# dryman/HashMergeJoin

Hardware: AMD Instinct MI355X
Metric: probe-side tuples/s + achieved HBM GB/s, |R|=|S|=2^28 u64 keys (higher is better)
Workload: dtype u64

## Files before the change

hashmergejoin_amd/__init__.py:

```python
from ._lib import (HMJ_BUILD_ANTI, HMJ_BUILD_OUTER, HMJ_BUILD_SEMI, HMJ_CHECKSUM, HMJ_COLS_HASHED, HMJ_COLS_NO_ROW, HMJ_COLS_PACKED, HMJ_FIRST_WINS, HMJ_FULL_OUTER, HMJ_GROUP_COUNT, HMJ_GROUP_MAX, HMJ_GROUP_MIN, HMJ_GROUP_ROW_MAP, HMJ_GROUP_SUM, HMJ_JOIN_ANTI, HMJ_JOIN_INNER, HMJ_JOIN_PROBE_OUTER, HMJ_JOIN_SEMI, HMJ_KIND_BUILD_SIDE, HMJ_KIND_PROBE_SIDE, HMJ_MATERIALIZE, HMJ_ORDERED, HMJ_PATH_CHUNKED_BUILD, HMJ_PATH_DENSE_BUILD,
                   HMJ_PATH_EXACT, HMJ_PATH_GLOBAL_TABLE, HMJ_PATH_HOST_PIPELINE, HMJ_PATH_HOT_KEY_HINT, HMJ_PATH_LOOKBACK_TIMEOUT, HMJ_PATH_ORDER_BY_KEY, HMJ_PATH_ORDER_BY_RANK_SORT, HMJ_PATH_ORDER_DEFERRED, HMJ_PATH_ORDERED_EXPANSION, HMJ_PATH_LDS_TABLE,
                   HMJ_PATH_KEY_RANGES, HMJ_PATH_PREPARED, HMJ_PATH_PRESORTED, HMJ_PATH_RANK_RUNS, HMJ_PATH_SORT_MSD, HMJ_PATH_SLAB, HMJ_PATH_SLAB_ONE_PASS, HMJ_PATH_SLAB_PROBE, HMJ_PATH_SORTED_FK, HMJ_PATH_SORTED_FK_HALF, HMJ_PATH_SORTED_FK_WIDE, HMJ_PATH_SORTED_WRITE, HMJ_PATH_SPLIT, HMJ_PATH_UNIQ_WRITE, HMJ_PATH_WINDOW,
                   HMJ_KEY_FIXED, HMJ_KEY_LARGE_STRING, HMJ_MAX_KEY_COLS, HMJ_MAX_TAKE_COLS, HMJ_NULL_EQUAL, HMJ_STR_NO_ROW, HMJ_SUM_PROBE, HMJ_TAKE_NO_ROW, BuildJoinOpts, ColsJoinOpts, ColsKindOpts, ColsRel, ColsResult, ExchangeKindOpts, GroupOpts, GroupResult, HmjError, JoinOpts, JoinResult, KeyCol, KindCounts, MixedCol, MixedOpts, MixedRel, StrJoinOpts, StrKindOpts, StrRel, StrResult, TakeDst, TakeOpts, TakeSrc, TakeStrDst, TakeStrOpts, TakeStrSrc, Timing, Validity,
                   lib_path, load_library)
from .join import Executor, HashMergeJoin, cols_key64, expected_groups, mixed_key64, pack_strings, pack_validity, plan, unpack_strings, unpack_validity

__all__ = ["Executor", "HashMergeJoin", "plan", "HmjError", "JoinResult", "Timing", "load_library",
           "lib_path", "HMJ_MATERIALIZE", "HMJ_ORDERED", "HMJ_FIRST_WINS", "HMJ_CHECKSUM",
           "HMJ_SUM_PROBE", "JoinOpts", "HMJ_JOIN_INNER", "HMJ_JOIN_SEMI", "HMJ_JOIN_ANTI", "HMJ_JOIN_PROBE_OUTER",
           "BuildJoinOpts", "HMJ_BUILD_SEMI", "HMJ_BUILD_ANTI", "HMJ_BUILD_OUTER", "HMJ_FULL_OUTER",
           "ExchangeKindOpts", "KindCounts", "HMJ_KIND_PROBE_SIDE", "HMJ_KIND_BUILD_SIDE",
           "pack_strings", "StrRel", "StrJoinOpts", "StrResult", "StrKindOpts", "HMJ_STR_NO_ROW",
           "KeyCol", "ColsRel", "ColsJoinOpts", "ColsResult", "HMJ_COLS_PACKED", "HMJ_COLS_HASHED", "HMJ_MAX_KEY_COLS",
           "cols_key64", "ColsKindOpts", "HMJ_COLS_NO_ROW", "Validity", "pack_validity",
           "TakeSrc", "TakeDst", "TakeOpts", "HMJ_TAKE_NO_ROW", "HMJ_MAX_TAKE_COLS", "unpack_validity",
           "TakeStrSrc", "TakeStrDst", "TakeStrOpts", "unpack_strings",
           "MixedCol", "MixedRel", "MixedOpts", "HMJ_KEY_FIXED", "HMJ_KEY_LARGE_STRING", "mixed_key64",
           "HMJ_NULL_EQUAL",
           "GroupOpts", "GroupResult", "HMJ_GROUP_COUNT", "HMJ_GROUP_SUM", "HMJ_GROUP_MIN", "HMJ_GROUP_MAX", "HMJ_GROUP_ROW_MAP",
           "expected_groups"]
```

hashmergejoin_amd/_lib.py:

```python
import ctypes as C
import os

HMJ_MATERIALIZE = 0x01
HMJ_ORDERED = 0x02
HMJ_FIRST_WINS = 0x04
HMJ_CHECKSUM = 0x08
HMJ_SUM_PROBE = 0x10
HMJ_NULL_EQUAL = 0x20
HMJ_E_RCCL, HMJ_E_PEER, HMJ_E_TIMEOUT = -6, -7, -8
HMJ_PATH_SLAB, HMJ_PATH_EXACT, HMJ_PATH_UNIQ_WRITE, HMJ_PATH_SPLIT, HMJ_PATH_WINDOW = 0x1, 0x2, 0x4, 0x8, 0x10
HMJ_PATH_ORDER_DEFERRED, HMJ_PATH_ORDER_BY_KEY, HMJ_PATH_PREPARED, HMJ_PATH_CHUNKED_BUILD = 0x20, 0x40, 0x80, 0x100
HMJ_PATH_HOT_KEY_HINT = 0x200
HMJ_PATH_SLAB_PROBE = 0x400
HMJ_PATH_SORTED_WRITE = 0x800
HMJ_PATH_SORTED_FK = 0x1000
HMJ_PATH_DENSE_BUILD = 0x2000
HMJ_PATH_GLOBAL_TABLE = 0x100000
HMJ_PATH_ORDER_BY_RANK_SORT = 0x200000
HMJ_PATH_ORDERED_EXPANSION = 0x400000
HMJ_PATH_LDS_TABLE = 0x800000
HMJ_PATH_RANK_RUNS = 0x1000000
HMJ_PATH_RANK_LOOKUP_IN_PASS = 0x2000000
HMJ_PATH_SORT_MSD = 0x4000000
HMJ_PATH_KEY_RANGES = 0x8000000
HMJ_PATH_SLAB_ONE_PASS = 0x80000
HMJ_PATH_HOST_PIPELINE = 0x4000
HMJ_PATH_SORTED_FK_HALF = 0x8000
HMJ_PATH_LOOKBACK_TIMEOUT = 0x10000
HMJ_PATH_SORTED_FK_WIDE = 0x20000
HMJ_PATH_PRESORTED = 0x40000

_HERE = os.path.dirname(os.path.abspath(__file__))
_U64P = C.POINTER(C.c_uint64)


class HmjError(RuntimeError):
    def __init__(self, code, msg):
        super().__init__("hmj error %d: %s" % (code, msg))
        self.code = code


class JoinResult(C.Structure):
    _fields_ = [("n_matches", C.c_uint64), ("sum_r", C.c_uint64), ("sum_s", C.c_uint64),
                ("xor_fold", C.c_uint64), ("mix_sum", C.c_uint64), ("sum_probe_all", C.c_uint64),
                ("key", C.c_void_p), ("rval", C.c_void_p), ("sval", C.c_void_p)]

    def checks(self):
        return {k: int(getattr(self, k)) for k in ("n_matches", "sum_r", "sum_s", "xor_fold", "mix_sum")}


HMJ_JOIN_INNER, HMJ_JOIN_SEMI, HMJ_JOIN_ANTI, HMJ_JOIN_PROBE_OUTER = 0, 1, 2, 3


class JoinOpts(C.Structure):
    _fields_ = [("struct_size", C.c_uint32), ("kind", C.c_uint32), ("outer_fill", C.c_uint64),
                ("n_probe_matched", C.c_uint64), ("n_probe_unmatched", C.c_uint64)]


HMJ_BUILD_SEMI, HMJ_BUILD_ANTI, HMJ_BUILD_OUTER, HMJ_FULL_OUTER = 1, 2, 3, 4


class BuildJoinOpts(C.Structure):
    _fields_ = [("struct_size", C.c_uint32), ("kind", C.c_uint32), ("build_fill", C.c_uint64), ("probe_fill", C.c_uint64),
# ... 165 lines not shown
                ("ms_out_scan", C.c_float), ("ms_probe_write", C.c_float), ("ms_order", C.c_float),
                ("radix_bits", C.c_int), ("radix_passes", C.c_int),
                ("n_scatter_launches", C.c_int), ("n_split_retries", C.c_int),
                ("bytes_scatter", C.c_uint64), ("bytes_hist", C.c_uint64),
                ("bytes_probe_count", C.c_uint64), ("bytes_probe_write", C.c_uint64),
                ("path", C.c_uint32), ("key_prefix_bits", C.c_int32), ("key_window_low", C.c_int32),
                ("n_probe_items", C.c_uint32), ("ms_scatter_pass0", C.c_float), ("ms_scatter_pass1", C.c_float)]

    def as_dict(self):
        return {n: getattr(self, n) for n, _ in self._fields_}


class PlanDesc(C.Structure):
    _fields_ = [("struct_size", C.c_uint32), ("path", C.c_uint32), ("radix_bits", C.c_int32), ("radix_passes", C.c_int32),
                ("pass_bits", C.c_int32 * 4), ("key_prefix_bits", C.c_int32), ("key_window_low", C.c_int32),
                ("n_partitions", C.c_uint32), ("probe_items", C.c_uint32), ("attempts", C.c_uint32), ("refused", C.c_uint32),
                ("cooling", C.c_uint32), ("workload", C.c_uint64)]

    def as_dict(self):
        d = {n: getattr(self, n) for n, _ in self._fields_}
        d["pass_bits"] = list(self.pass_bits)
        return d


HMJ_REFUSED_GTABLE_SHAPE, HMJ_REFUSED_GTABLE_COOLING, HMJ_REFUSED_GTABLE_GAVE_UP = 0x1, 0x2, 0x4
HMJ_REFUSED_RANK_SORT_MODEL, HMJ_REFUSED_RANK_SORT_COOLING, HMJ_REFUSED_RANK_SORT_GAVE_UP = 0x8, 0x10, 0x20
HMJ_REFUSED_SLAB_SHAPE, HMJ_REFUSED_SLAB_COOLING, HMJ_REFUSED_SLAB_SORTED_INPUT, HMJ_REFUSED_SLAB_OVERFLOW = 0x40, 0x80, 0x100, 0x200
HMJ_REFUSED_FAST_WRITE_COOLING, HMJ_REFUSED_FAST_WRITE_GAVE_UP = 0x400, 0x800
HMJ_REFUSED_SLAB_PROBE_COOLING, HMJ_REFUSED_SLAB_PROBE_OVERFLOW = 0x1000, 0x2000
HMJ_REFUSED_PREFIX_VIOLATED, HMJ_REFUSED_EXPANSION_GAVE_UP = 0x4000, 0x8000
HMJ_COOL_UNIQ_WRITE, HMJ_COOL_SORTED_WRITE, HMJ_COOL_GTABLE, HMJ_COOL_GTABLE_WRITE = 0x1, 0x2, 0x4, 0x8
HMJ_COOL_RANK_SORT, HMJ_COOL_RANK_SORT_SLAB, HMJ_COOL_EXPANSION, HMJ_COOL_SORT_SLAB = 0x10, 0x20, 0x40, 0x80
HMJ_COOL_SLAB, HMJ_COOL_SLAB_PROBE, HMJ_COOL_ONE_PASS_WRITE, HMJ_COOL_EXACT_PREFIX = 0x100, 0x200, 0x400, 0x800
HMJ_COOL_RANK_RUNS = 0x1000


class PlaceInfo(C.Structure):
    _fields_ = [("name", C.c_char * 16), ("bytes", C.c_uint64), ("fill_TBps", C.c_float), ("candidates", C.c_int),
                ("ms_search", C.c_float), ("searched", C.c_int), ("aborted", C.c_int), ("budget_ms", C.c_float),
                ("cand_ms_alloc", C.c_float * 4), ("cand_ms_fill", C.c_float * 4), ("cand_TBps", C.c_float * 4)]


def lib_path():
    return os.environ.get("HMJ_LIB") or os.path.join(_HERE, "libhmj_hip.so")


class ExchangeInfo(C.Structure):
    _fields_ = [("n_ranks", C.c_int), ("owner_mode", C.c_int), ("rounds_build", C.c_uint32), ("rounds_probe", C.c_uint32),
                ("recv_build", C.c_uint64), ("recv_probe", C.c_uint64), ("ms_split", C.c_float),
                ("ms_exchange_build", C.c_float), ("ms_exchange_probe", C.c_float), ("ms_local", C.c_float),
                ("ms_total", C.c_float), ("digit_bits", C.c_int32), ("digit_low", C.c_int32), ("n_subjoins", C.c_uint32),
                ("fallback", C.c_uint32), ("sample_max_share", C.c_float), ("ms_kernels", C.c_float),
                ("ms_exposed", C.c_float)]

    def as_dict(self):
        return {n: getattr(self, n) for n, _ in self._fields_}


HMJ_MAX_RANKS, HMJ_MAX_ROUNDS = 16, 16


class DigitPlan(C.Structure):
    _fields_ = [("usable", C.c_int32), ("digit_bits", C.c_int32), ("digit_low", C.c_int32), ("n_rounds", C.c_uint32),
                ("owner_first", C.c_uint32 * (HMJ_MAX_RANKS + 1)),
                ("round_first", (C.c_uint32 * (HMJ_MAX_ROUNDS + 1)) * HMJ_MAX_RANKS), ("max_share", C.c_float)]


# ... 151 lines not shown
```

hashmergejoin_amd/csrc/api.hip:

```cpp
#include <hip/hip_runtime.h>
#include <sys/mman.h>

#include <algorithm>
#include <cstdio>
#include <cstdlib>
#include <chrono>
#include <cmath>
#include <cstring>
#include <mutex>
#include <string>
#include <thread>
#include <vector>

#include "hmj_ctx.h"

using hmj::u32;
using hmj::u64;
using namespace hmj_host;

namespace hmj_host {

constexpr int kMaxEvents = 1024;

int fail(hmj_ctx* c, int code, const char* what, hipError_t e) {
// ... 29 lines not shown
  acc->ms_scatter_pass[0] += t.ms_scatter_pass[0];
  acc->ms_scatter_pass[1] += t.ms_scatter_pass[1];
  if (t.radix_passes) {
    acc->radix_bits = t.radix_bits;
    acc->radix_passes = t.radix_passes;
    acc->key_prefix_bits = t.key_prefix_bits;
    acc->key_window_low = t.key_window_low;
  }
  acc->n_probe_items += t.n_probe_items;
}

static int ilog2_u64(uint64_t v) { return v ? 63 - __builtin_clzll(v) : 0; }
uint64_t workload_signature(uint64_t n_build, uint64_t n_probe, uint32_t flags, int kind) {
  const uint32_t mode = ((flags & HMJ_ORDERED) ? 4u : 0u) | ((flags & (HMJ_MATERIALIZE | HMJ_ORDERED)) ? 2u : 0u) |
                        ((flags & HMJ_FIRST_WINS) ? 1u : 0u);
  return ((uint64_t)(kind & 31) << 20) | ((uint64_t)mode << 16) | ((uint64_t)ilog2_u64(n_build) << 8) | (uint64_t)ilog2_u64(n_probe);
}
WorkloadMemo* memo_for(hmj_ctx* c, uint64_t sig) {
  auto it = c->memos.find(sig);
  if (it == c->memos.end()) {
    if (c->memos.size() >= 1024) c->memos.clear();
    it = c->memos.emplace(sig, c->memo_init).first;
  }
  c->wm = &it->second;
  c->wm_sig = sig;
  return c->wm;
}
uint32_t WorkloadMemo::cooling() const {
  return (uniq_cooldown ? HMJ_COOL_UNIQ_WRITE : 0u) | (sorted_cooldown ? HMJ_COOL_SORTED_WRITE : 0u) | (gtable_cooldown ? HMJ_COOL_GTABLE : 0u) |
         (gtable_write_cooldown ? HMJ_COOL_GTABLE_WRITE : 0u) | (gtable_sort_cooldown ? HMJ_COOL_RANK_SORT : 0u) |
         (gtable_sort_slab_cooldown ? HMJ_COOL_RANK_SORT_SLAB : 0u) | (expand_cooldown ? HMJ_COOL_EXPANSION : 0u) |
         (sort_slab_cooldown ? HMJ_COOL_SORT_SLAB : 0u) | (slab_cooldown ? HMJ_COOL_SLAB : 0u) | (slab_probe_cooldown ? HMJ_COOL_SLAB_PROBE : 0u) |
         (one_pass_write_cooldown ? HMJ_COOL_ONE_PASS_WRITE : 0u) | (exact_prefix_joins ? HMJ_COOL_EXACT_PREFIX : 0u) |
         (rank_runs_cooldown ? HMJ_COOL_RANK_RUNS : 0u) | (sort_msd_cooldown ? HMJ_COOL_SORT_MSD : 0u);
}

int wait_arrival(hmj_ctx* c, hipEvent_t ev) {
  if (c->arrive_wait) return c->arrive_wait(c, ev);
  HIP_TRY(hipStreamWaitEvent(c->stream, ev, 0));
  return HMJ_OK;
}

int ensure_dev(hmj_ctx* c, DevBuf& b, size_t bytes) {
  if (bytes <= b.cap) return HMJ_OK;
  if (c && (&b == &c->rbuf[0] || &b == &c->rbuf[1] || &b == &c->r_off || &b == &c->slab_br || &b == &c->cnt_br))
    c->prep.valid = false;
  if (b.p) {
    hipError_t e = hipFree(b.p);
    b.p = nullptr;
    b.cap = 0;
    if (e != hipSuccess) return fail(c, HMJ_E_HIP, "hipFree", e);
  }
  size_t want = bytes + (bytes >> 4) + 256;
#ifdef HMJ_DEV
  if (const char* e = getenv("HMJ_ALLOC_PAD_KB")) want += (size_t)atoll(e) << 10;
  if (const char* e = getenv("HMJ_ALLOC_ROUND_MB")) {
    const size_t g = (size_t)atoll(e) << 20;
    if (g) want = (want + g - 1) / g * g;
  }
#endif
  const auto t_alloc0 = std::chrono::steady_clock::now();
  hipError_t e = hipMalloc(&b.p, want);
  if (e != hipSuccess) {
    b.p = nullptr;
    (void)hipGetLastError();
    return fail(c, HMJ_E_OOM, "hipMalloc", e);
  }
// ... 430 lines not shown
  a.r_off = (const u32*)c->r_off.p;
  a.S = Sp;
  a.s_off = (const u32*)c->s_off.p;
  a.P = P;
  a.Q = Q;
  a.accum = (u64*)c->accum.p;
  return a;
}
static hmj::ProbeArgs slab_probe_args(hmj_ctx* c, const hmj::SlabGeom* build_slabs, const void* Rp, const DevBuf& s_slab,
                                      const DevBuf& s_cnt, u32 s_cap, u32 P, u32 Q) {
  hmj::ProbeArgs a;
  std::memset(&a, 0, sizeof(a));
  if (build_slabs) {
    a.R = c->slab_br.p;
    a.r_cnt = (const u32*)c->cnt_br.p;
    a.r_cap = build_slabs->CB;
    a.r_cnt_n = c->cnt_br.cap / 4;
    a.r_rows = c->slab_br.cap / 16;
  } else {
    a.R = Rp;
    a.r_off = (const u32*)c->r_off.p;
  }
  a.S = s_slab.p;
  a.s_cnt = (const u32*)s_cnt.p;
  a.s_cap = s_cap;
  a.s_cnt_n = s_cnt.cap / 4;
  a.s_rows = s_slab.cap / 16;
  a.P = P;
  a.Q = Q;
  a.accum = (u64*)c->accum.p;
  return a;
}

static int slab_pass_a(hmj_ctx* c, const void* in, u32 n, int rel, int low, int bits, const hmj::SlabGeom& g, bool arriving) {
  u64* acc = (u64*)c->accum.p;
  const u64 a_rows = c->slab_a.cap / 16, a_cnt = c->cnt_a.cap / 4;
  const int sp = span_begin(c, K_SCATTER, rel, 0);
  if (arriving) {
    u32 w_done = 0;
    for (size_t i = 0; i < c->arrive_ev.size(); i++) {
      RC_TRY(wait_arrival(c, c->arrive_ev[i]));
      const bool last = i + 1 == c->arrive_ev.size();
      const u32 w_end = last ? g.WA : (u32)std::min<u64>(g.WA, c->arrive_rows[i] / g.rpw);
      if (w_end > w_done) {
        HIP_TRY(hmj::launch_slab_a(in, n, low, bits, g, c->slab_a.p, a_rows, (u32*)c->cnt_a.p, a_cnt, acc, c->stream, w_done, w_end));
        w_done = w_end;
      }
    }
  } else {
    HIP_TRY(hmj::launch_slab_a(in, n, low, bits, g, c->slab_a.p, a_rows, (u32*)c->cnt_a.p, a_cnt, acc, c->stream));
  }
  span_end(c, sp);
  c->timing.bytes_scatter += 32ull * n;
  return HMJ_OK;
}
static int slab_passes(hmj_ctx* c, const void* in, u32 n, int rel, int low, int ba, int bb, const hmj::SlabGeom& g, DevBuf& sb,
                       DevBuf& cb, bool arriving) {
  RC_TRY(slab_pass_a(c, in, n, rel, low, ba, g, arriving));
  const int sp = span_begin(c, K_SCATTER, rel, 1);
  HIP_TRY(hmj::launch_slab_b(c->slab_a.p, (const u32*)c->cnt_a.p, ba, low + ba, bb, g, sb.p, sb.cap / 16, (u32*)cb.p, cb.cap / 4,
                             (u64*)c->accum.p, c->stream));
  span_end(c, sp);
  c->timing.bytes_scatter += 32ull * n;
  return HMJ_OK;
}

static int clear_matched(hmj_ctx* c, size_t slots, u32** matched) {
  const size_t bytes = (slots / 32 + 1) * 4;
  RC_TRY(ensure_dev(c, c->matched, bytes));
  *matched = (u32*)c->matched.p;
  HIP_TRY(hipMemsetAsync(c->matched.p, 0, bytes, c->stream));
  return HMJ_OK;
}

int order_rows(hmj_ctx* c, const u32* vstart, const u32* in_base32, const u64* in_base64, u32 P, u32 Q, int low,
               u64 n, bool by_key_only, bool many_per_key, const u64** rk, const u64** rr, const u64** rs, int* retry_code) {
  const size_t bytes = (size_t)n * 8;
  RC_TRY(ensure_dev(c, c->ord_key, bytes));
  RC_TRY(ensure_dev(c, c->ord_rval, bytes));
  RC_TRY(ensure_dev(c, c->ord_sval, bytes));
  const bool can_sort = n <= 0xFFFFFFFFull;
  if (by_key_only && !can_sort) {
    *retry_code = kRetryNoWinOrdered;
    return HMJ_OK;
  }
  int sp = span_begin(c, K_ORDER, -1);
  HIP_TRY(hmj::launch_order((const u64*)c->part_out_off.p, vstart, in_base32, in_base64, P, Q, low,
                            (const u64*)c->out_key.p, (const u64*)c->out_rval.p, (const u64*)c->out_sval.p,
                            (u64*)c->ord_key.p, (u64*)c->ord_rval.p, (u64*)c->ord_sval.p, (u64*)c->accum.p,
                            can_sort ? 65536u : 0u, many_per_key, c->num_cus * 4, c->stream));
  span_end(c, sp);
  u64* h = (u64*)c->h_accum.p;
  HIP_TRY(hipMemcpyAsync(&h[hmj::ACC_ERR], (u64*)c->accum.p + hmj::ACC_ERR, 8, hipMemcpyDeviceToHost, c->stream));
  HIP_TRY(hipStreamSynchronize(c->stream));
  if (h[hmj::ACC_ERR] & hmj::ERR_ORDER_FAIL)
    return fail(c, HMJ_E_UNSUPPORTED, "HMJ_ORDERED: one partition's result exceeds 2^31-1 rows and the whole result 2^32-1 rows");
// ... 521 lines not shown
static int run_slab_join(hmj_ctx* c, const JoinCall& j, const JoinPlan& p) {
  const bool materialize = j.materialize(), first = j.first(), extra = j.extra();
  const u32 nb = j.nb, np = j.np, np_plan = p.np_plan, P = p.P;
  const int* pass_bits = p.pass_bits;
  hmj::SlabGeom gr, gs;
  if (p.allow_slab && c->slab_mode && c->wm->slab_cooldown == 0 && !c->prepare_only && !(c->timing.path & HMJ_PATH_SLAB) &&
      !((!materialize || p.fast_write) && p.Q == 1 && p.probe_fits && p.passes == 2 && pass_bits[0] <= hmj::SLAB_MAX_BITS &&
        pass_bits[1] <= hmj::SLAB_MAX_BITS && p.dense_scale <= 2.5))
    c->plan.refused |= HMJ_REFUSED_SLAB_SHAPE;
  if (!(p.allow_slab && c->slab_mode && c->wm->slab_cooldown == 0 && (!materialize || p.fast_write) && p.Q == 1 &&
        p.probe_fits &&
        p.passes == 2 && pass_bits[0] <= hmj::SLAB_MAX_BITS && pass_bits[1] <= hmj::SLAB_MAX_BITS &&
        slab_sizes_ok(c, nb, np_plan, materialize || np_plan < nb) &&
        p.dense_scale <= 2.5 &&
        hmj::slab_geometry(nb, pass_bits[0], pass_bits[1], &gr, 0, 1.0, p.dense_scale) &&
        hmj::slab_geometry(np_plan, pass_bits[0], pass_bits[1], &gs, 0,
                           (nb && np_plan > nb) ? (double)np_plan / (double)nb : 1.0, p.dense_scale)))
    return kPlanNotTaken;
  const bool reuse = c->prep.valid && c->prep.slab && c->prep.ptr == j.R && c->prep.n == nb &&
                     c->prep.low == p.low && c->prep.B == p.B;
  c->prep.valid = false;
  c->timing.path |= HMJ_PATH_SLAB | (reuse ? HMJ_PATH_PREPARED : 0u);
  c->timing.n_probe_items = P;
  const int ba = pass_bits[0], bb = pass_bits[1];
  const u64 rows_a = gr.rows_a > gs.rows_a ? gr.rows_a : gs.rows_a;
  const u32 wa = gr.WA > gs.WA ? gr.WA : gs.WA;
  RC_TRY(ensure_dev(c, c->slab_a, rows_a * 16));
  RC_TRY(ensure_dev(c, c->cnt_a, ((size_t)wa << ba) * 4));
  RC_TRY(ensure_dev(c, c->slab_br, gr.rows_b * 16));
  RC_TRY(ensure_dev(c, c->slab_bs, gs.rows_b * 16));
  RC_TRY(ensure_dev(c, c->cnt_br, (size_t)P * gr.KB * 4));
  RC_TRY(ensure_dev(c, c->cnt_bs, (size_t)P * gs.KB * 4));
  if (!reuse) RC_TRY(slab_passes(c, j.R, nb, 0, p.low, ba, bb, gr, c->slab_br, c->cnt_br, false));
  if (!c->prepare_only) RC_TRY(slab_passes(c, j.S, np, 1, p.low, ba, bb, gs, c->slab_bs, c->cnt_bs, !c->arrive_ev.empty()));
  u64* hh;
  if (c->prepare_only) {
    RC_TRY(read_accum(c, &hh));
    if (hh[hmj::ACC_ERR] & hmj::ERR_SLAB) {
      c->wm->slab_cooldown = 8;
      return kRetryNoSlab;
    }
    c->prep.valid = true;
    c->prep.slab = true;
    c->prep.ptr = j.R;
    c->prep.n = nb;
    c->prep.low = p.low;
    c->prep.B = p.B;
    return HMJ_OK;
  }
  hmj::ProbeArgs sa = slab_probe_args(c, &gr, nullptr, c->slab_bs, c->cnt_bs, gs.CB, P, 1);
  if (p.fast_write)
    return unique_key_write(c, sa, true, nb, np, p.low, extra, p.verify_pfx ? p.prefix : 0, p.pfx_ref, j.ordered(), j.to_host,
                            p.fk_wide_plan, p.dense_scale, j.out);
#ifdef HMJ_DEV
  sa.debug = c->dev_ablate;
#endif
  int sp = span_begin(c, K_PROBE_COUNT, -1);
  if (first || extra) {
    sa.extra = (extra ? 1u : 0u) | (first ? 2u : 0u);
    HIP_TRY(hmj::launch_probe_count_ext(sa, nullptr, nullptr, true, c->num_cus, c->stream));
  } else {
    HIP_TRY(hmj::launch_probe_count_slab(sa, c->num_cus, c->stream));
  }
  span_end(c, sp);
  c->timing.bytes_probe_count = 16ull * ((u64)nb + np);
  RC_TRY(read_accum(c, &hh));
  if (hh[hmj::ACC_ERR] & hmj::ERR_SLAB) {
    c->wm->slab_cooldown = 8;
    return kRetryNoSlab;
  }
  result_sums(j.out, hh);
  return HMJ_OK;
}

static int partition_build_exact(hmj_ctx* c, const JoinCall& j, const JoinPlan& p, const void** Rp) {
  const bool reuse_exact = c->prep.valid && !c->prep.slab && c->prep.ptr == j.R && c->prep.n == j.nb &&
                           c->prep.low == p.low && c->prep.B == p.B;
  c->prep.valid = false;
  c->timing.path |= HMJ_PATH_EXACT | (reuse_exact ? HMJ_PATH_PREPARED : 0u);
  if (reuse_exact) {
    *Rp = c->prep.Rp;
  } else {
    RC_TRY(partition_relation(c, j.R, j.nb, c->rbuf, p.low, p.passes, p.pass_bits, 0, Rp, p.asc_r));
    const int s = span_begin(c, K_OFFSETS, -1);
    HIP_TRY(hmj::launch_part_offsets(*Rp, j.nb, p.low, p.B, (u32*)c->r_off.p, c->stream));
    span_end(c, s);
  }
  if (c->prepare_only) {
    HIP_TRY(hipStreamSynchronize(c->stream));
// ... 316 lines not shown
  RC_TRY(ensure_dev(c, c->s_off, ((size_t)p.P + 1) * 4));
  RC_TRY(ensure_dev(c, c->accum, 8 * sizeof(u64)));
  RC_TRY(ensure_host(c, c->h_accum, 8 * sizeof(u64)));
  if (j.materialize()) {
    RC_TRY(ensure_dev(c, c->part_count, (size_t)p.items * 8));
    RC_TRY(ensure_dev(c, c->part_out_off, ((size_t)p.items + 1) * 8));
  }
  HIP_TRY(hipMemsetAsync(c->accum.p, 0, 8 * sizeof(u64), c->stream));
  int rc = run_slab_join(c, j, p);
  if (rc != kPlanNotTaken) return rc;
  const void* Rp;
  RC_TRY(partition_build_exact(c, j, p, &Rp));
  if (c->prepare_only) return HMJ_OK;
  for (hipEvent_t ev : c->arrive_ev) RC_TRY(wait_arrival(c, ev));
  rc = run_probe_slab_join(c, j, p, Rp);
  if (rc != kPlanNotTaken) return rc;
  rc = run_one_pass_slab_join(c, j, p, Rp);
  if (rc != kPlanNotTaken) return rc;
  return run_partitioned_join(c, j, p, Rp);
}

int join_device_impl(hmj_ctx* c, const void* R, uint64_t n_build, const void* S, uint64_t n_probe,
                     uint32_t flags, hmj_result* out, bool to_host, bool allow_auto_prefix,
                     bool allow_slab, bool allow_fast_write, bool allow_win_ordered, bool prefix_unsafe,
                     bool allow_slab_probe) {
  if (!out) return fail(c, HMJ_E_ARG, "out is NULL");
  std::memset(out, 0, sizeof(*out));
  RC_TRY(check_rel(c, R, n_build, "build_aos is NULL"));
  RC_TRY(check_rel(c, S, n_probe, "probe_aos is NULL"));
  if (flags & HMJ_ORDERED) flags |= HMJ_MATERIALIZE;
  if (!c->prepare_only && c->prep.valid && !c->prep.slab && c->prep.ptr == R && c->prep.n == (u32)n_build) allow_slab = false;
  const bool materialize = flags & HMJ_MATERIALIZE;
  if (c->wm->slab_cooldown > 0 && allow_slab) c->wm->slab_cooldown--;
  if (c->wm->slab_probe_cooldown > 0 && allow_slab_probe) c->wm->slab_probe_cooldown--;
  if (c->wm->one_pass_write_cooldown > 0 && materialize && allow_slab_probe) c->wm->one_pass_write_cooldown--;
  JoinPlan p;
  RC_TRY(plan_join(c, R, n_build, S, n_probe, flags, allow_auto_prefix, allow_slab, allow_fast_write, allow_win_ordered,
                   prefix_unsafe, allow_slab_probe, &p));
  const JoinCall j{R, S, (u32)n_build, (u32)n_probe, flags, out, to_host};
  return execute_join(c, j, p);
}

int try_global_table(hmj_ctx* c, const void* R, uint64_t n_build, const void* S, uint64_t n_probe, uint32_t flags,
                     hmj_result* out, bool to_host, bool* done) {
  *done = false;
  const bool materialize = (flags & HMJ_MATERIALIZE) != 0;
  c->plan.refused |= HMJ_REFUSED_GTABLE_SHAPE;
  if (!c->gtable_mode || (flags & HMJ_ORDERED) || c->prepare_only || c->force_bits >= 0 ||
      !c->arrive_ev.empty() || n_build == 0 || n_probe > 0xFFFFFFFFull || n_probe < c->gtable_min_probe ||
      (n_build > (materialize && !(c->one_pass_slab && c->slab_mode && n_probe >= (1ull << 22) && n_probe >= 8 * n_build) ? 2 : 1) * c->gtable_max_rows && !(n_build <= 8 * c->gtable_max_rows && n_build + n_probe <= 16 * c->gtable_max_rows)) ||
      n_probe < (uint64_t)c->gtable_min_fanout * n_build ||
      (c->prep.valid && c->prep.ptr == R && c->prep.n == (u32)n_build))
    return HMJ_OK;
  c->plan.refused &= ~HMJ_REFUSED_GTABLE_SHAPE;
  if (materialize && c->wm->gtable_write_cooldown > 0) {
    c->wm->gtable_write_cooldown--;
    c->plan.refused |= HMJ_REFUSED_GTABLE_COOLING;
    return HMJ_OK;
  }
  if (c->wm->gtable_cooldown > 0) {
    c->wm->gtable_cooldown--;
    c->plan.refused |= HMJ_REFUSED_GTABLE_COOLING;
    return HMJ_OK;
  }
  if (!out) return fail(c, HMJ_E_ARG, "out is NULL");
  RC_TRY(check_rel(c, R, n_build, "build_aos is NULL"));
// ... 875 lines not shown
    const u64 unmatched = k.kind == HMJ_JOIN_SEMI ? n_probe - out->n_matches : filled;
    counts->n_probe_matched = n_probe - unmatched;
    counts->n_probe_unmatched = unmatched;
  } else {
    const u64 b_unmatched = k.kind == HMJ_BUILD_SEMI ? n_build - swept : swept;
    counts->n_build_matched = n_build - b_unmatched;
    counts->n_build_unmatched = b_unmatched;
    if (k.kind == HMJ_FULL_OUTER) {
      counts->n_probe_matched = n_probe - filled;
      counts->n_probe_unmatched = filled;
    }
  }
  return HMJ_OK;
}

}

extern "C" {

int hmj_create(hmj_ctx** out, int device_id) {
  if (!out) return HMJ_E_ARG;
  *out = nullptr;
  int ndev = 0;
  if (hipGetDeviceCount(&ndev) != hipSuccess || ndev <= 0) {
    (void)hipGetLastError();
    return HMJ_E_NODEV;
  }
  if (device_id < 0 && hipGetDevice(&device_id) != hipSuccess) return HMJ_E_NODEV;
  if (device_id >= ndev) return HMJ_E_ARG;
  if (hipSetDevice(device_id) != hipSuccess) return HMJ_E_NODEV;
  hmj_ctx* c = new hmj_ctx();
  c->device = device_id;
  if (const char* e = getenv("HMJ_SLAB")) c->slab_mode = atoi(e);
  if (const char* e = getenv("HMJ_ONE_PASS_SLAB")) c->one_pass_slab = atoi(e) != 0;
  if (const char* e = getenv("HMJ_GTABLE")) c->gtable_mode = atoi(e) != 0;
  if (const char* e = getenv("HMJ_RANK_RUNS")) c->rank_runs_mode = atoi(e) != 0;
  if (const char* e = getenv("HMJ_RANK_RUNS_MAX_CUT")) c->rank_runs_max_cut = atoi(e) < 0 ? 0 : atoi(e) > 16 ? 16 : atoi(e);
  if (const char* e = getenv("HMJ_RANK_RUNS_MAX_GROUP")) c->rank_runs_max_group = atoi(e) < 0 ? 0 : atoi(e) > 4 ? 4 : atoi(e);
  if (const char* e = getenv("HMJ_PROMOTE_TO_ORDERED")) c->promote_to_ordered = atoi(e) != 0;
  if (const char* e = getenv("HMJ_KEY_RANGES")) c->key_ranges = atoi(e) != 0;
  if (const char* e = getenv("HMJ_KEY_RANGES_FORCE")) c->key_ranges_force = atoi(e) < 0 ? 0 : atoi(e) > 4 ? 4 : atoi(e);
  if (const char* e = getenv("HMJ_RANK_RUNS_WAVE")) c->rank_runs_wave = atoi(e) != 0;
  if (const char* e = getenv("HMJ_RANK_RUNS_MAX_LEVEL")) c->rank_runs_max_level = atoi(e) < 0 ? 0 : atoi(e) > 2 ? 2 : atoi(e);
  if (const char* e = getenv("HMJ_GTABLE_SORT")) c->gtable_sort_mode = atoi(e) != 0;
  if (const char* e = getenv("HMJ_EXPAND_FK_FANOUT")) c->expand_fk_fanout = atoi(e) > 0 ? (u32)atoi(e) : 0u;
  if (const char* e = getenv("HMJ_SORT_MSD")) c->sort_msd = atoi(e) != 0;
  if (const char* e = getenv("HMJ_SORT_MSD_MEAN")) c->sort_msd_mean = atof(e) >= 64.0 ? atof(e) : c->sort_msd_mean;
  if (const char* e = getenv("HMJ_SORT_MSD_MAX_BITS")) c->sort_msd_max_bits = atoi(e) < 2 ? 2 : atoi(e) > 18 ? 18 : atoi(e);
  if (const char* e = getenv("HMJ_SORT_MSD_MIN_LOG2")) {
    const int l = atoi(e);
    if (l >= 16 && l <= 32) c->sort_msd_min = 1ull << l;
  }
  if (const char* e = getenv("HMJ_SORT_SLAB_MIN_LOG2")) {
    const int l = atoi(e);
    if (l >= 12 && l <= 32) c->sort_slab_min = 1ull << l;
  }
  if (const char* e = getenv("HMJ_GTABLE_SORT_SLAB_MIN_LOG2")) {
    const int l = atoi(e);
    if (l >= 12 && l <= 32) c->gtable_sort_slab_min = 1ull << l;
  }
  if (const char* e = getenv("HMJ_GTABLE_SORT_FANOUT")) c->gtable_sort_fanout = atoi(e) > 0 ? (u32)atoi(e) : 1u;
  if (const char* e = getenv("HMJ_PLACE")) {
    c->place_tune = atoi(e) != 0;
    if (atoi(e) > 0) {
      c->place_tries = atoi(e);
      c->place_search_always = true;
// ... 862 lines not shown
```

hashmergejoin_amd/csrc/hmj_ctx.h:

```cpp
#pragma once
#include <hip/hip_runtime.h>

#include <string>
#include <unordered_map>
#include <vector>

#include "../../include/hmj.h"
#include "hmj_dev.h"
#include "hmj_launch.h"

struct hmj_comm;

namespace hmj_host {

struct DevBuf {
  void* p = nullptr;
  size_t cap = 0;
};
struct HostBuf {
  void* p = nullptr;
  size_t cap = 0;
  bool pinned = true;
};

// ... 31 lines not shown
  template <class F>
  void each_buf(F f) {
    for (DevBuf* b : {&rows, &sorted, &flags, &blk, &blk_off, &list, &runs, &acc, &start}) f(*b);
    each_result_buf(f);
  }
};

enum Kind {
  K_TOTAL = 0, K_H2D, K_D2H, K_HIST, K_SCAN, K_SCATTER, K_OFFSETS, K_PROBE_COUNT, K_OUT_SCAN,
  K_PROBE_WRITE, K_ORDER, K_NKINDS
};
struct Span {
  int kind, rel, e0, e1;
  int pass;
};

struct WorkloadMemo {
  int uniq_cooldown = 0;
  int sorted_cooldown = 0;
  bool sorted_chained = false;
  bool sorted_wide = true;
  bool sorted_fk = false;
  int sorted_fk_age = 0;
  int gtable_cooldown = 0;
  int gtable_write_cooldown = 0;
  int gtable_sort_cooldown = 0;
  int gtable_sort_slab_cooldown = 0;
  int rank_runs_cooldown = 0;
  int rank_lookup_cooldown = 0;
  int expand_cooldown = 0;
  int sort_slab_cooldown = 0;
  int sort_msd_cooldown = 0;
  int slab_cooldown = 0;
  int slab_probe_cooldown = 0;
  int one_pass_write_cooldown = 0;
  int exact_prefix_joins = 0;
  uint32_t cooling() const;
};

}

namespace hmj_host {
struct OrderedCostModel {
  double part_fixed_ms = 0.15;
  double part_ns = 0.030, part_ns_per_f = 0.00023;
  double part_bucket_ns = 0.043, part_bucket_ns_per_f = 0.0001;
  double part_epilogue_ns = 0.25;
  double comp_fixed_ms = 0.65;
  double comp_ns_chain = 0.060, comp_ns_exact = 0.072;
  double comp_ns_wide = 0.145;
  double comp_ns_beyond_l2 = 0.02;
  double runs_fixed_ms = 0.25, runs_ns = 0.0215, runs_ns_per_run = 7.5;
  double runs_ns_per_log2_build = 0.0023;
  double runs_wave_ns_per_run = 1.2, runs_wave_ns = 0.007;
  double runs_range_ns = 0.0;
};
}

struct hmj_ctx {
  using DevBuf = hmj_host::DevBuf;
  using HostBuf = hmj_host::HostBuf;
  using Span = hmj_host::Span;
  using WorkloadMemo = hmj_host::WorkloadMemo;
  using u32 = hmj::u32;
  using u64 = hmj::u64;
  int device = 0, num_cus = 256;
// ... 56 lines not shown
  bool gtable_mode = true;
  uint64_t gtable_max_rows = 1ull << 17;
  u32 gtable_min_fanout = 0;
  uint64_t gtable_min_probe = 1;
  int gtable_wg_per_cu = 8;
  u32 gtable_slots_per_row = 16;
  int gtable_max_log_cap = 18;
  bool ltable_mode = true;
  bool gtable_sort_mode = true;
  u32 gtable_sort_fanout = 128;
  bool rank_runs_mode = true;
  int rank_runs_max_cut = 10;
  int rank_runs_max_group = 3;
  int rank_runs_max_level = 2;
  uint64_t big_join_rows = 1ull << 29;
  bool promote_to_ordered = true;
  bool key_ranges = true;
  int key_ranges_force = 0;
  bool rank_runs_wave = true;
  bool build_sort_msd = true;
  bool gtable_sort_slab = true;
  u64 gtable_sort_slab_min = 1ull << 25;
  bool expand_mode = true;
  u32 fk_payload_buckets = 24;
  u32 expand_fk_fanout = 0;
  bool expand_allow_rebits = true;
  int expand_rebits = 0;
  bool sort_msd = true;
  double sort_msd_mean = 1200.0;
  int sort_msd_max_bits = 18;
  u64 sort_msd_min = 1ull << 22;
  bool sort_slab = true;
  u64 sort_slab_min = 1ull << 25;
  int slab_mode = 1;
  bool staged_upload = false;
  bool host_pipeline = true;
  hipStream_t copy_stream = nullptr;
  std::vector<hipEvent_t> copy_ev;
  bool split_mode = true;
  bool window_mode = true;
  u32 slab_min_rows = 1u << 21;
  u32 slab_probe_kb = 0;
  bool one_pass_slab = true;
  int scatter_variant = 1;
  bool profiling = false;
  bool trace = false;
#ifdef HMJ_DEV
  u32 dev_ablate = 0;
#endif
  std::vector<hipEvent_t> events;
  std::vector<Span> spans;
  int ev_used = 0;
  hmj_timing timing;
  std::string last_error;
  hmj_comm* comm = nullptr;
  std::vector<u64> arrive_rows;
  std::vector<hipEvent_t> arrive_ev;
  bool sample_build_only = false;
  int (*arrive_wait)(hmj_ctx*, hipEvent_t) = nullptr;
};


namespace hmj_host {
int fail(hmj_ctx* c, int code, const char* what, hipError_t e = hipSuccess);
#define HIP_TRY(expr)                                                        \
  do {                                                                       \
// ... 39 lines not shown
```

hashmergejoin_amd/csrc/hmj_dev.h:

```cpp
#pragma once
#include <hip/hip_runtime.h>
#include <stdint.h>

namespace hmj {

typedef unsigned long long u64;
typedef unsigned int u32;
typedef unsigned short u16;

struct __attribute__((aligned(16))) Tup {
  u64 key;
  u64 val;
};

constexpr int kWave = 64;
#ifndef HMJ_SCAN_DPP
#define HMJ_SCAN_DPP 1
#endif

#ifndef HMJ_STREAM_POLICY
#define HMJ_STREAM_POLICY 2
#endif
typedef u64 u64x2_t __attribute__((ext_vector_type(2)));
__device__ __forceinline__ void store_stream(Tup* p, const Tup& v) {
#if HMJ_STREAM_POLICY >= 1
  u64x2_t x = {v.key, v.val};
  __builtin_nontemporal_store(x, reinterpret_cast<u64x2_t*>(p));
#else
  *p = v;
#endif
}
__device__ __forceinline__ Tup load_stream(const Tup* p) {
#if HMJ_STREAM_POLICY >= 2
  const u64x2_t x = __builtin_nontemporal_load(reinterpret_cast<const u64x2_t*>(p));
  Tup t;
  t.key = x.x;
  t.val = x.y;
  return t;
#else
  return *p;
#endif
}

constexpr u64 GT_EMPTY = ~0ull;
constexpr int GT_MAXWALK = 64;
__device__ __forceinline__ u32 gt_hash(u64 key, int shift) {
  u64 h = key * 0x9E3779B97F4A7C15ull;
  h ^= h >> 32;
  h *= 0xD6E8FEB86659FD93ull;
  return (u32)(h >> shift);
}

#ifndef HMJ_RANK_PASS_CHUNK_ROWS
#define HMJ_RANK_PASS_CHUNK_ROWS 64
#endif
constexpr int RANK_PASS_CHUNK_ROWS = HMJ_RANK_PASS_CHUNK_ROWS;
__device__ __forceinline__ u64 rank_run_bucket(u64 off, int pre, u64 mult) { return ((off >> pre) * mult) >> 32; }

template <int ROWS, typename Table, typename OnSlot>
__device__ __forceinline__ void gt_walk(Table tab, u32 mask, u32 (&slot)[ROWS], bool (&live)[ROWS], OnSlot on_slot) {
  bool any_live = false;
#pragma unroll
  for (int r = 0; r < ROWS; r++) any_live |= live[r];
  while (any_live) {
    Tup e[ROWS];
#pragma unroll
    for (int r = 0; r < ROWS; r++)
      if (live[r]) e[r] = tab[slot[r]];
    any_live = false;
#pragma unroll
    for (int r = 0; r < ROWS; r++) {
// ... 3 lines not shown
        } else {
          slot[r] = (slot[r] + 1) & mask;
          any_live = true;
        }
      }
    }
  }
}

constexpr int RP_THREADS = 512;
constexpr int RP_WAVES = RP_THREADS / kWave;
constexpr int RP_ITEMS = 8;
constexpr int RP_TILE = RP_THREADS * RP_ITEMS;
constexpr int RP_MAX_BITS = 9;
constexpr int RP_MAXD = 1 << RP_MAX_BITS;
constexpr int RP_MAX_BLOCKS = 2048;

constexpr int PB_THREADS = 1024;
constexpr int PB_CAP = 5120;
constexpr int PB_LOG_NB = 12;
constexpr int PB_TARGET_AVG = 4096;
constexpr int PB_PLAN_SLACK = 256;

constexpr int SLAB_KB = 4;
constexpr int SLAB_MAX_BITS = 9;

enum { ACC_N = 0, ACC_SUM_R, ACC_SUM_S, ACC_XOR, ACC_MIX, ACC_SUM_P, ACC_ERR, ACC_PAD };
constexpr u64 ERR_SLAB = 2;
constexpr u64 ERR_ORDER_DEFER = 16;
constexpr u64 ERR_ORDER_FAIL = 32;
constexpr u64 ERR_SORTED = 64;
constexpr u64 ERR_FASTPATH = 8;
constexpr u64 ERR_GTABLE = 128;
constexpr u64 ERR_PREFIX = 4;

__device__ __forceinline__ u64 mix64(u64 x) {
  x ^= x >> 30;
  x *= 0xBF58476D1CE4E5B9ull;
  x ^= x >> 27;
  x *= 0x94D049BB133111EBull;
  x ^= x >> 31;
  return x;
}

__device__ __forceinline__ u64 tmix(u64 key, u64 rval, u64 sval) {
  u64 t = mix64(key);
  t = mix64(t ^ rval);
  t = mix64(t + sval);
  return t;
}

__device__ __forceinline__ int lane_id() {
  return __builtin_amdgcn_mbcnt_hi(~0u, __builtin_amdgcn_mbcnt_lo(~0u, 0u));
}

__device__ __forceinline__ u32 popc_below(u64 m) {
  return __builtin_amdgcn_mbcnt_hi((u32)(m >> 32), __builtin_amdgcn_mbcnt_lo((u32)m, 0u));
}

__device__ __forceinline__ u32 wave_incl_scan_u32(u32 v, int ) {
#if HMJ_SCAN_DPP
  v += (u32)__builtin_amdgcn_update_dpp(0, (int)v, 0x111, 0xF, 0xF, false);
  v += (u32)__builtin_amdgcn_update_dpp(0, (int)v, 0x112, 0xF, 0xF, false);
  v += (u32)__builtin_amdgcn_update_dpp(0, (int)v, 0x114, 0xF, 0xF, false);
  v += (u32)__builtin_amdgcn_update_dpp(0, (int)v, 0x118, 0xF, 0xF, false);
  v += (u32)__builtin_amdgcn_update_dpp(0, (int)v, 0x142, 0xA, 0xF, false);
// ... 73 lines not shown
```

hashmergejoin_amd/csrc/hmj_launch.h:

```cpp
#pragma once
#include <hip/hip_runtime.h>
#include <stddef.h>
#include <stdint.h>

#include <atomic>

namespace hmj {
typedef unsigned long long u64;
typedef unsigned int u32;

struct SmemAttrOnce {
  std::atomic<unsigned long long> devices{0};
};
inline hipError_t ensure_max_smem(SmemAttrOnce& once, const void* kernel, size_t bytes) {
  int dev = 0;
  hipError_t e = hipGetDevice(&dev);
  if (e != hipSuccess) return e;
  const unsigned long long bit = 1ull << (dev & 63);
  if (dev < 64 && (once.devices.load(std::memory_order_acquire) & bit)) return hipSuccess;
  e = hipFuncSetAttribute(kernel, hipFuncAttributeMaxDynamicSharedMemorySize, (int)bytes);
  if (e != hipSuccess) return e;
  if (dev < 64) once.devices.fetch_or(bit, std::memory_order_release);
  return hipSuccess;
}

constexpr int kMaxRanks = 16;
struct OwnerFn {
  u32 mode;
  u32 G;
  u64 spl[kMaxRanks - 1];
};
int radix_tile_rows(int bits, int variant);
void radix_pass_geometry(u32 n, int tile, u32* nblk, u32* rows_per_block);
size_t radix_scatter_smem_bytes();
hipError_t launch_radix_hist(const void* in, u32 n, int tile, int shift, int bits, u32* hist,
                             u32 nblk, u32 rows_per_block, hipStream_t st, const OwnerFn* own = nullptr);
hipError_t launch_owner_scatter(const void* in, void* out, u32 n, int bits, const OwnerFn& own,
                                const u32* hist_scanned, const u32* totals, u32 nblk, u32 rows_per_block,
                                u64* offsets_out, hipStream_t st);
hipError_t launch_radix_rowscan(u32* hist, u32 nblk, int bits, u32* totals, hipStream_t st);
hipError_t launch_radix_scatter(const void* in, void* out, u32 n, int variant, int shift, int bits,
                                const u32* hist_scanned, const u32* totals, u32 nblk,
                                u32 rows_per_block, u64* offsets_out, hipStream_t st);
struct SlabGeom {
  u32 WA, rpw, CA, CB, KB;
  u64 rows_a, rows_b;
};
bool slab_geometry(u32 n, int bits_a, int bits_b, SlabGeom* g, u32 kb = 0, double fan = 1.0, double density = 1.0);
bool slab_geometry_one_pass(u32 n, int bits, double keys_per_digit, u32 max_workers, SlabGeom* g, double density = 1.0);
u32 slab_capacity(double mean, double fan);
hipError_t launch_slab_a(const void* in, u32 n, int shift, int bits, const SlabGeom& g, void* slab_a, u64 slab_a_rows,
                         u32* cnt_a, u64 cnt_a_n, u64* accum, hipStream_t st, u32 w_begin = 0, u32 w_end = 0xFFFFFFFFu);
hipError_t launch_slab_b(const void* slab_a, const u32* cnt_a, int bits_a, int shift, int bits,
                         const SlabGeom& g, void* slab_b, u64 slab_b_rows, u32* cnt_b, u64 cnt_b_n, u64* accum, hipStream_t st);
hipError_t launch_key_sample(const void* R, u32 nb, const void* S, u32 np, u64* out, hipStream_t st);
hipError_t launch_key_exact(const void* R, u32 nb, const void* S, u32 np, u64 ref, u64* out, int num_cus, hipStream_t st,
                            bool ref_is_first_key = false);
hipError_t launch_check_partitioned(const void* a, u32 n, int low, int bits, u32* flag, int num_cus, hipStream_t st);
hipError_t launch_part_offsets(const void* a, u32 n, int low, int bits, u32* off, hipStream_t st);

struct ProbeArgs {
  const void* R;
  const u32* r_off;
  const void* S;
  const u32* s_off;
  u32 P;
  u32 Q;
  u64* part_count;
  const u64* part_out_off;
  u64* out_key;
  u64* out_rval;
  u64* out_sval;
  u64 out_cap;
  u64* accum;
  const u32* item_list;
  const u32* n_item_list;
  const u32* r_cnt;
  const u32* s_cnt;
  u32 r_cap, s_cap;
  u32 s_wa, s_ppi;
  u64 r_cnt_n, s_cnt_n;
  u64 r_rows, s_rows;
  const u64* item_base;
  const u32* r_end;
  const u32* s_end;
  u32 extra;
  u32 pfx_shift;
  u64 pfx_val;
  u32* matched;
  u32 debug;
};
hipError_t launch_probe(const ProbeArgs& a, int mode, bool first_wins, bool extra, int grid,
                        hipStream_t st);
int probe_default_grid(int num_cus);
hipError_t launch_probe_kind(const ProbeArgs& a, int mode, int kind, bool first_wins, u64 fill, int grid, hipStream_t st);
hipError_t launch_probe_build_kind(const ProbeArgs& a, int mode, int kind, u64 fill, u32* bmark, int grid, hipStream_t st);
hipError_t launch_build_sweep(const ProbeArgs& a, const u32* r_off, u32 P, const u32* vstart, u64* sweep_n, int mode,
                              bool set, u64 fill, int num_cus, hipStream_t st);
hipError_t launch_probe_count_ext(const ProbeArgs& a, u32* irregular, u32* n_irregular, bool slab,
                                  int num_cus, hipStream_t st);
hipError_t launch_probe_count_slab(const ProbeArgs& a, int num_cus, hipStream_t st);
hipError_t launch_probe_write_sorted(const ProbeArgs& a, bool slab, bool fk, int shape, u64* lookback, bool chained, int key_low,
                                     int num_cus, hipStream_t st);
hipError_t launch_probe_write_uniq(const ProbeArgs& a, bool slab, int num_cus, hipStream_t st);
hipError_t launch_slab_np(const u32* cnt, u32 P, u64* out, hipStream_t st);
hipError_t launch_probe_count_fast(const ProbeArgs& a, u32* irregular, u32* n_irregular, bool big,
                                   bool per_partition_counts, int num_cus, hipStream_t st);
hipError_t launch_scan_u64(const u64* in, u64* out_excl, u32 n, hipStream_t st);
hipError_t launch_probe_expand_ordered(const ProbeArgs& a, int key_low, int num_cus, hipStream_t st);
hipError_t launch_order(const u64* part_out_off, const u32* vstart, const u32* in_base32, const u64* in_base64, u32 P, u32 Q,
                        int low, const u64* akey, const u64* arval, const u64* asval, u64* bkey, u64* brval,
                        u64* bsval, u64* accum, u32 defer_rows, bool many_per_key, int grid, hipStream_t st);
hipError_t launch_compact(const u64* part_out_off, const u32* in_base32, const u64* in_base64, u32 P, const u64* akey,
                          const u64* arval, const u64* asval, u64* bkey, u64* brval, u64* bsval, int grid, hipStream_t st);
hipError_t launch_rekey(void* pairs, u64 n, const u64* col, hipStream_t st);

hipError_t launch_gtable_build(const void* R, u32 nb, void* tab, int log_cap, u64* accum, bool first, int num_cus,
                               hipStream_t st);
hipError_t launch_gtable_probe(const void* S, u32 np, const void* tab, int log_cap, const void* R, u64* accum, bool first,
                               bool extra, int num_cus, int wg_per_cu, hipStream_t st);
hipError_t launch_gtable_write(const void* S, u32 np, const void* tab, int log_cap, const void* R, u64* accum, u64* out_key,
                               u64* out_rval, u64* out_sval, bool first, bool extra, int num_cus, int wg_per_cu, hipStream_t st);

hipError_t launch_ltable_probe(const void* R, u32 nb, const void* S, u32 np, u64* accum, bool first, bool extra, int num_cus, hipStream_t st);
int ltable_max_rows();
hipError_t launch_sval_range(const void* S, u32 np, u64* out2 , int num_cus, hipStream_t st,
                             u32 every = 1 );
hipError_t launch_gtable_emit(const void* S, u32 np, const void* tab, int log_cap, u64 svmin, int range_bits, u64* accum,
                              void* pairs, bool extra, bool wide, int num_cus, int wg_per_cu, hipStream_t st);
hipError_t launch_gtable_swap(const void* in, void* out, u64 n, int num_cus, hipStream_t st);
hipError_t launch_gtable_emit_ranks(const void* S, u32 np, const void* tab, int log_cap, u64* accum, void* pairs, bool extra, int num_cus,
                                    int wg_per_cu, hipStream_t st);
int rank_sort_max_run(int level = 0);
hipError_t launch_sort_runs_write(const void* slabs, const u32* cnt, u32 cap, u32 P, const u64* out_off, void* out, u64* accum, int level,
// ... 36 lines not shown
```

hashmergejoin_amd/csrc/probe.hip:

```cpp
#include "hmj_dev.h"
#include "hmj_launch.h"
#include <type_traits>

namespace hmj {

constexpr u32 PB_NB = 1u << PB_LOG_NB;
constexpr u32 NIL = 0xFFFFu;
static_assert(PB_CAP < 0xFFFF, "chain links are 16-bit");

struct ProbeSmem {
  u64 key[PB_CAP];
  u64 val[PB_CAP];
  u32 head[PB_NB];
  u32 aux[PB_CAP];
  u16 next[PB_CAP];
  u32 scratch[PB_THREADS / kWave + 1];
  u64 pcount;
  u64 red[8];
  u64 obase;
  u32 wtot[PB_THREADS / kWave];
  u32 nslot;
};
constexpr u32 PB_BATCH = 2 * PB_THREADS;
static_assert(PB_BATCH <= PB_CAP, "a batch must fit an empty table");
// ... 860 lines not shown
};

template <int LOG_NB>
__device__ __forceinline__ u32 fast_hash(u64 k) {
  u32 x = (u32)k ^ ((u32)(k >> 32) * 0x85EBCA6Bu);
  x *= 0x9E3779B1u;
  return x >> (32 - LOG_NB);
}

template <int THREADS, int ROWS = FP_ROWS>
__device__ __forceinline__ void fp_load(Tup (&t)[ROWS], const Tup* __restrict__ base, u32 n,
                                        int tid) {
#pragma unroll
  for (int k = 0; k < ROWS; k++) {
    u32 i = k * THREADS + tid;
    t[k] = base[i < n ? i : n - 1];
  }
}

static_assert(SLAB_KB == 4, "fp_load_slab / fp_load_pieces / slab_np_kernel unroll exactly four pieces per partition");
template <int THREADS, int ROWS = FP_ROWS>
__device__ __forceinline__ void fp_load_slab(Tup (&t)[ROWS], const Tup* __restrict__ base, u32 cap,
                                             u32 p1, u32 p2, u32 p3, u32 n, int tid) {
#pragma unroll
  for (int k = 0; k < ROWS; k++) {
    u32 i = k * THREADS + tid;
    i = i < n ? i : n - 1;
    const u32 j = (i >= p1) + (i >= p2) + (i >= p3);
    const u32 pre = j == 0 ? 0u : (j == 1 ? p1 : (j == 2 ? p2 : p3));
    t[k] = base[(u64)j * cap + (i - pre)];
  }
}

template <int THREADS>
__device__ __forceinline__ void fp_load_pieces(Tup (&t)[FP_ROWS], const Tup* __restrict__ base, u32 cap, u32 cnt_mine, int tid) {
  constexpr int QT = THREADS / 4;
  const u32 g = (u32)tid / QT, l = (u32)tid % QT;
  const Tup* __restrict__ piece = base + (u64)g * cap;
  const u32 last = cnt_mine ? cnt_mine - 1 : 0;
#pragma unroll
  for (int k = 0; k < FP_ROWS; k++) {
    const u32 r = l + (u32)k * QT;
    t[k] = piece[r < last ? r : last];
  }
}

template <int THREADS, int LOG_NB, bool PCOUNT, bool SLAB, int OUT>
__global__ __launch_bounds__(THREADS, 4) void probe_count_fast_kernel(
    ProbeArgs a, u32* __restrict__ irregular, u32* __restrict__ n_irregular) {
  typedef FastSmem<THREADS, LOG_NB> Smem;
  constexpr u32 CAP = Smem::CAP, NB = 1u << LOG_NB;
  constexpr bool PIECES = SLAB && OUT == 0 && !PCOUNT && HMJ_PROBE_PIECES;
  constexpr u32 QT = THREADS / 4, PIECE_CAP = FP_ROWS * QT;
  extern __shared__ __attribute__((aligned(16))) unsigned char smem_raw[];
  Smem& sm = *reinterpret_cast<Smem*>(smem_raw);
  const Tup* __restrict__ R = static_cast<const Tup*>(a.R);
  const Tup* __restrict__ S = static_cast<const Tup*>(a.S);
  const u32* __restrict__ r_off = a.r_off;
  const u32* __restrict__ s_off = a.s_off;
  const u32* __restrict__ r_end = (SLAB || a.r_end == nullptr) ? a.r_off + 1 : a.r_end;
  const u32* __restrict__ s_end = (SLAB || a.s_end == nullptr) ? a.s_off + 1 : a.s_end;
  const u32 P = a.P;
  const int tid = threadIdx.x;
  u64 acc_n = 0, acc_r = 0, acc_s = 0, acc_x = 0, acc_m = 0, acc_p = 0;
  bool pfx_bad = false, giveup = false;
  for (u32 i = tid; i < NB; i += THREADS) sm.head[i] = 0;
  if (tid < 2) sm.itemcnt[tid] = 0;
  u32 epoch = 0;
  u32 prev_p = 0xFFFFFFFFu, parity = 0;

  u32 p = blockIdx.x;
  u32 rb = 0, nb = 0, sb = 0, np = 0;
  bool regular = false;
  Tup br[FP_ROWS], pr[FP_ROWS], pq[FP_ROWS];
  u32 r1 = 0, r2 = 0, r3 = 0, s1 = 0, s2 = 0, s3 = 0, r1n = 0, r2n = 0, r3n = 0, s1n = 0, s2n = 0, s3n = 0;
  u32 rm = 0, sm_ = 0, rmn = 0, smn = 0;
  const u32 my_piece = (u32)tid / QT;
  bool slab_bad = false;
  if (p < P) {
    if (SLAB) {
      const u32* rc = a.r_cnt + (u64)p * SLAB_KB;
      const u32* sc = a.s_cnt + (u64)p * SLAB_KB;
      r1 = rc[0]; r2 = r1 + rc[1]; r3 = r2 + rc[2]; nb = r3 + rc[3];
      s1 = sc[0]; s2 = s1 + sc[1]; s3 = s2 + sc[2]; np = s3 + sc[3];
      if (nb > CAP || np > CAP) slab_bad = true;
      if (PIECES) {
        rm = my_piece == 0 ? rc[0] : my_piece == 1 ? rc[1] : my_piece == 2 ? rc[2] : rc[3];
        sm_ = my_piece == 0 ? sc[0] : my_piece == 1 ? sc[1] : my_piece == 2 ? sc[2] : sc[3];
        if (rc[0] > PIECE_CAP || rc[1] > PIECE_CAP || rc[2] > PIECE_CAP || rc[3] > PIECE_CAP || sc[0] > PIECE_CAP ||
            sc[1] > PIECE_CAP || sc[2] > PIECE_CAP || sc[3] > PIECE_CAP) {
          slab_bad = true;
          nb = CAP + 1;
        }
      }
    } else {
      rb = r_off[p]; nb = r_end[p] - rb;
      sb = s_off[p]; np = s_end[p] - sb;
    }
    regular = nb && np && nb <= CAP && np <= CAP;
    if (regular) {
      if (PIECES) {
        fp_load_pieces<THREADS>(br, R + (u64)p * SLAB_KB * a.r_cap, a.r_cap, rm, tid);
        fp_load_pieces<THREADS>(pr, S + (u64)p * SLAB_KB * a.s_cap, a.s_cap, sm_, tid);
      } else if (SLAB) {
        fp_load_slab<THREADS>(br, R + (u64)p * SLAB_KB * a.r_cap, a.r_cap, r1, r2, r3, nb, tid);
        if (OUT == 0) fp_load_slab<THREADS>(pr, S + (u64)p * SLAB_KB * a.s_cap, a.s_cap, s1, s2, s3, np, tid);
      } else {
        fp_load<THREADS>(br, R + rb, nb, tid);
        if (OUT == 0) fp_load<THREADS>(pr, S + sb, np, tid);
      }
    }
  }
  const Tup* __restrict__ dummy = reinterpret_cast<const Tup*>(a.accum);
  auto load_build = [&](Tup (&t)[FP_ROWS], bool ok, u32 pp, u32 rb_, u32 nb_, u32 q1, u32 q2, u32 q3, u32 mine) {
    if (PIECES)
      fp_load_pieces<THREADS>(t, ok ? R + (u64)pp * SLAB_KB * a.r_cap : dummy, ok ? a.r_cap : 0u, ok ? mine : 1u, tid);
    else if (SLAB)
      fp_load_slab<THREADS>(t, ok ? R + (u64)pp * SLAB_KB * a.r_cap : dummy, ok ? a.r_cap : 0u, ok ? q1 : 1u, ok ? q2 : 1u,
                            ok ? q3 : 1u, ok ? nb_ : 1u, tid);
    else
      fp_load<THREADS>(t, ok ? R + rb_ : dummy, ok ? nb_ : 1u, tid);
  };
  auto load_probe = [&](Tup (&t)[FP_ROWS], bool ok, u32 pp, u32 sb_, u32 np_, u32 q1, u32 q2, u32 q3, u32 mine) {
    if (PIECES)
      fp_load_pieces<THREADS>(t, ok ? S + (u64)pp * SLAB_KB * a.s_cap : dummy, ok ? a.s_cap : 0u, ok ? mine : 1u, tid);
    else if (SLAB)
      fp_load_slab<THREADS>(t, ok ? S + (u64)pp * SLAB_KB * a.s_cap : dummy, ok ? a.s_cap : 0u, ok ? q1 : 1u, ok ? q2 : 1u,
                            ok ? q3 : 1u, ok ? np_ : 1u, tid);
    else
      fp_load<THREADS>(t, ok ? S + sb_ : dummy, ok ? np_ : 1u, tid);
  };
  const int tid_outer = tid;
  while (p < P) {
    int tid = tid_outer;
    if constexpr (OUT != 0) asm volatile("" : "+v"(tid));
    u64 out_base = (u64)sb;
    if constexpr (OUT == 1 && SLAB) {
      const u64* ibp = a.item_base + p;
      asm volatile("s_load_dwordx2 %0, %1, 0x0\n\ts_waitcnt lgkmcnt(0)" : "=s"(out_base) : "s"(ibp) : "memory");
    }
    const u32 pn = __builtin_amdgcn_readfirstlane(p + gridDim.x);
    u32 rb2 = 0, nb2 = 0, sb2 = 0, np2 = 0;
    bool regular2 = false;
    if (pn < P) {
      if (SLAB) {
        const u32* rc = a.r_cnt + (u64)pn * SLAB_KB;
        const u32* sc = a.s_cnt + (u64)pn * SLAB_KB;
        r1n = rc[0]; r2n = r1n + rc[1]; r3n = r2n + rc[2]; nb2 = r3n + rc[3];
        s1n = sc[0]; s2n = s1n + sc[1]; s3n = s2n + sc[2]; np2 = s3n + sc[3];
        if (nb2 > CAP || np2 > CAP) slab_bad = true;
        if (PIECES) {
          rmn = my_piece == 0 ? rc[0] : my_piece == 1 ? rc[1] : my_piece == 2 ? rc[2] : rc[3];
          smn = my_piece == 0 ? sc[0] : my_piece == 1 ? sc[1] : my_piece == 2 ? sc[2] : sc[3];
          if (rc[0] > PIECE_CAP || rc[1] > PIECE_CAP || rc[2] > PIECE_CAP || rc[3] > PIECE_CAP || sc[0] > PIECE_CAP ||
              sc[1] > PIECE_CAP || sc[2] > PIECE_CAP || sc[3] > PIECE_CAP) {
            slab_bad = true;
            nb2 = CAP + 1;
          }
        }
      } else {
        rb2 = r_off[pn]; nb2 = r_end[pn] - rb2;
        sb2 = s_off[pn]; np2 = s_end[pn] - sb2;
      }
      regular2 = nb2 && np2 && nb2 <= CAP && np2 <= CAP;
    }
    if (OUT == 0) {
      load_probe(pq, regular2, pn, sb2, np2, s1n, s2n, s3n, smn);
    } else if (regular) {
      if (SLAB)
        fp_load_slab<THREADS>(pr, S + (u64)p * SLAB_KB * a.s_cap, a.s_cap, s1, s2, s3, np, tid);
      else
        fp_load<THREADS>(pr, S + sb, np, tid);
    }
    if (regular) {
      lds_barrier();
      if (PCOUNT && prev_p != 0xFFFFFFFFu && tid == 0) {
        a.part_count[prev_p] = sm.itemcnt[parity ^ 1];
        sm.itemcnt[parity ^ 1] = 0;
      }
      if (PCOUNT) prev_p = 0xFFFFFFFFu;
      epoch++;
      if (epoch == 0x10000u) {
        for (u32 i = tid; i < NB; i += THREADS) sm.head[i] = 0;
        epoch = 1;
        lds_barrier();
      }
      const u32 tag = epoch << 16;
      if (!HMJ_ABLATE(1u)) {
        u32 old[FP_ROWS];
#pragma unroll
        for (int k = 0; k < FP_ROWS; k++) {
          const u32 i = k * THREADS + tid;
          old[k] = tag | NIL;
          if (PIECES ? ((u32)tid % QT + (u32)k * QT < rm) : (i < nb)) {
            if (a.pfx_shift && (br[k].key >> a.pfx_shift) != a.pfx_val) pfx_bad = true;
            sm.key[i] = br[k].key;
            sm.val[i] = br[k].val;
            old[k] = atomicExch(&sm.head[fast_hash<LOG_NB>(br[k].key)], tag | i);
          }
        }
#pragma unroll
        for (int k = 0; k < FP_ROWS; k++) {
          const u32 i = k * THREADS + tid;
          if (PIECES ? ((u32)tid % QT + (u32)k * QT < rm) : (i < nb)) sm.next[i] = ((old[k] >> 16) == epoch) ? (u16)old[k] : (u16)NIL;
        }
      } else {
#pragma unroll
        for (int k = 0; k < FP_ROWS; k++) acc_r += br[k].key;
      }
      load_build(br, regular2, pn, rb2, nb2, r1n, r2n, r3n, rmn);
      lds_barrier();
      const u64 n_before = acc_n;
      if (!HMJ_ABLATE(1u)) {
        u32 cur[FP_ROWS];
        u32 cnt[FP_ROWS], first[FP_ROWS];
#pragma unroll
        for (int k = 0; k < FP_ROWS; k++) {
          const u32 j = k * THREADS + tid;
          cur[k] = NIL;
          cnt[k] = 0;
          first[k] = OUT == 2 ? NIL : 0;
          if (PIECES ? ((u32)tid % QT + (u32)k * QT < sm_) : (j < np)) {
            if (a.pfx_shift && (pr[k].key >> a.pfx_shift) != a.pfx_val) pfx_bad = true;
            if (OUT >= 1 && (a.extra & 1u)) acc_p += pr[k].val;
            const u32 hv = sm.head[fast_hash<LOG_NB>(pr[k].key)];
            cur[k] = ((hv >> 16) == epoch) ? (hv & 0xFFFFu) : NIL;
          }
        }
        for (; !HMJ_ABLATE(2u);) {
          bool any = false;
#pragma unroll
          for (int k = 0; k < FP_ROWS; k++) any |= (cur[k] != NIL);
          if (!__any(any)) break;
#pragma unroll
          for (int k = 0; k < FP_ROWS; k++) {
            if (cur[k] != NIL) {
              const u32 i = cur[k];
              const u64 kk = sm.key[i], vv = sm.val[i];
              cur[k] = sm.next[i];
              if (kk == pr[k].key) {
                if (OUT == 2 && (a.extra & 2u)) {
                  first[k] = i < first[k] ? i : first[k];
                } else {
                  acc_n++;
                  acc_r += vv;
                  acc_s += pr[k].val;
                  if (OUT == 1) {
                    if (cnt[k] == 0) first[k] = i;
                    cnt[k]++;
                  }
                  if (OUT >= 1 && (a.extra & 1u)) {
                    const u64 m = tmix(kk, vv, pr[k].val);
                    acc_x ^= m;
                    acc_m += m;
                  }
                }
              }
            }
          }
        }
        if (OUT == 2 && (a.extra & 2u)) {
#pragma unroll
          for (int k = 0; k < FP_ROWS; k++) {
            if (first[k] != NIL) {
              const u64 vv = sm.val[first[k]];
              acc_n++;
              acc_r += vv;
              acc_s += pr[k].val;
              if (a.extra & 1u) {
                const u64 m = tmix(pr[k].key, vv, pr[k].val);
                acc_x ^= m;
                acc_m += m;
              }
            }
          }
        }
        if (OUT == 1) {
          u64 packed = 0;
          bool cx = false;
#pragma unroll
          for (int k = 0; k < FP_ROWS; k++) {
            cx |= cnt[k] > 1;
            packed |= (u64)(cnt[k] ? 1u : 0u) << (12 * k);
          }
          const int lane = tid & 63, wv = tid >> 6;
          const bool wave_dup = __any(cx);
          u64 incl = packed;
#pragma unroll
          for (int o = 1; o < kWave; o <<= 1) {
            u64 t = __shfl_up(incl, o, kWave);
            if (lane >= o) incl += t;
          }
          if (lane == 63) {
            sm.wscan[wv] = incl;
            sm.wdup[wv] = wave_dup ? 1u : 0u;
          }
          lds_barrier();
          u64 pre = 0, tot = 0;
          u32 dup = 0;
#pragma unroll
          for (int q = 0; q < THREADS / kWave; q++) {
            const u64 ws = sm.wscan[q];
            dup |= sm.wdup[q];
            if (q < wv) pre += ws;
            tot += ws;
          }
          const u64 ex = pre + incl - packed;
          if (dup) {
            giveup = true;
          } else {
            u64 o = out_base;
            u32 total = 0;
#pragma unroll
            for (int k = 0; k < FP_ROWS; k++) {
              if (cnt[k]) {
                const u64 d = o + ((ex >> (12 * k)) & 0xFFFu);
                a.out_key[d] = pr[k].key;
                a.out_rval[d] = sm.val[first[k]];
                a.out_sval[d] = pr[k].val;
              }
              const u32 tk = (u32)((tot >> (12 * k)) & 0xFFFu);
              o += tk;
              total += tk;
            }
            if (tid == 0) a.part_count[p] = total;
          }
        }
      } else {
#pragma unroll
        for (int k = 0; k < FP_ROWS; k++) acc_r += pr[k].key;
      }
      if (PCOUNT) {
        const u32 mine = (u32)(acc_n - n_before);
        const u32 ws = (u32)wave_sum_u64(mine);
        if ((tid & 63) == 0 && ws) atomicAdd(&sm.itemcnt[parity], ws);
        prev_p = p;
        parity ^= 1;
      }
    } else {
      if ((PCOUNT || OUT == 1) && tid == 0 && !(nb && np)) a.part_count[p] = 0;
      if (OUT == 1 && nb && np) giveup = true;
      if (OUT >= 1 && (a.extra & 1u) && !nb) {
        if (SLAB) {
          const Tup* base = S + (u64)p * SLAB_KB * a.s_cap;
          for (u32 j = tid; j < np; j += THREADS) {
            const u32 pc = (j >= s1) + (j >= s2) + (j >= s3);
            const u32 pre = pc == 0 ? 0 : pc == 1 ? s1 : pc == 2 ? s2 : s3;
            acc_p += base[(u64)pc * a.s_cap + (j - pre)].val;
          }
        } else {
          for (u32 j = tid; j < np; j += THREADS) acc_p += S[sb + j].val;
        }
      }
      if (OUT != 1 && !SLAB && tid == 0 && nb && np) irregular[atomicAdd(n_irregular, 1u)] = p;
      load_build(br, regular2, pn, rb2, nb2, r1n, r2n, r3n, rmn);
    }
    if (OUT == 0) {
#pragma unroll
      for (int k = 0; k < FP_ROWS; k++) pr[k] = pq[k];
    }
    p = pn; rb = rb2; nb = nb2; sb = sb2; np = np2; regular = regular2;
    r1 = r1n; r2 = r2n; r3 = r3n; s1 = s1n; s2 = s2n; s3 = s3n;
    rm = rmn; sm_ = smn;
  }
  if (SLAB && slab_bad && tid == 0) atomicOr(&a.accum[ACC_ERR], ERR_SLAB);
  if (OUT == 1 && __any(giveup) && (tid & 63) == 0) atomicOr(&a.accum[ACC_ERR], ERR_FASTPATH);
  if (__any(pfx_bad) && (tid & 63) == 0) atomicOr(&a.accum[ACC_ERR], ERR_PREFIX);
  lds_barrier();
  if (PCOUNT && prev_p != 0xFFFFFFFFu && tid == 0) a.part_count[prev_p] = sm.itemcnt[parity ^ 1];
  if (tid < 8) sm.red[tid] = 0;
  lds_barrier();
  const u64 v[6] = {acc_n, acc_r, acc_s, acc_x, acc_m, acc_p};
  block_accumulate(sm.red, a.accum, v, 1u << ACC_XOR);
}

constexpr int SW_LOGB = 12, SW_NB = 1 << SW_LOGB, SW_MAXBUCKET = 32;
constexpr u64 LB_AGG = 1ull << 62, LB_PFX = 2ull << 62, LB_MASK = (1ull << 62) - 1;
constexpr u32 LB_SPIN_LIMIT = 1u << 22;

template <int THREADS>
struct SortedSmem {
  static constexpr int CAP = THREADS * FP_ROWS, CAPB = CAP, LOGB = SW_LOGB;
  u64 key[CAP];
  u64 val[CAP];
  u64 sval[CAP];
  u32 cnt[SW_NB];
  u16 bstart[SW_NB + 2];
  u16 perm[CAP];
  u32 mbits[2][CAP / 32];
  u32 scratch[THREADS / kWave + 1];
  u32 tick[2];
  u32 flag;
  u64 obase;
  u64 red[8];
};

constexpr int SWF_LOGB = 11, SWF_CAPB = 4608, SWF_MAXDUP = 1024;
constexpr int SWF_HALF_THREADS = 512, SWF_HALF_ROWS = 6, SWF_HALF_CAPB = 2048, SWF_HALF_LOGB = 10;
constexpr int SWF_WIDE_ROWS = 6, SWF_WIDE_CAPB = 2560;
template <int THREADS, int ROWS = FP_ROWS, int CAPB_ = SWF_CAPB, int LOGB_ = SWF_LOGB>
// ... 1094 lines not shown
      vr_beg[v] = rb + b;
      vr_end[v] = rb + e;
    }
    if (ns == 1) {
      vs_beg[v] = sb;
      vs_end[v] = sb + np;
    } else {
      const u32 step = (np + ns - 1) / ns;
      const u32 b = qs * step, e = (b + step < np) ? b + step : np;
      vs_beg[v] = sb + (b < np ? b : np);
      vs_end[v] = sb + e;
    }
  }
}
hipError_t launch_split_parts(const u32* r_off, const u32* s_off, u32 P, u32 thr_rows, u32 slice_rows, u32 build_thr,
                              u32 build_slice, u32 cap_v, u32* vstart, u32* vr_beg, u32* vr_end, u32* vs_beg,
                              u32* vs_end, u32* nv_out, hipStream_t st) {
  hipLaunchKernelGGL(split_count_kernel, dim3(1), dim3(1024), 0, st, r_off, s_off, P, thr_rows, slice_rows, build_thr,
                     build_slice, cap_v, vstart, nv_out);
  hipLaunchKernelGGL(split_fill_kernel, dim3((cap_v + 255) / 256), dim3(256), 0, st, r_off, s_off, P, thr_rows,
                     slice_rows, build_thr, build_slice, cap_v, vstart, vr_beg, vr_end, vs_beg, vs_end);
  return hipGetLastError();
}

template <int MODE, bool FIRST, bool EXTRA>
static hipError_t launch_probe_t(const ProbeArgs& a, int grid, hipStream_t st) {
  static SmemAttrOnce attr_once;
  if (hipError_t e = ensure_max_smem(attr_once, reinterpret_cast<const void*>(probe_kernel<MODE, FIRST, EXTRA>), (size_t)sizeof(ProbeSmem)); e != hipSuccess) return e;
  hipLaunchKernelGGL((probe_kernel<MODE, FIRST, EXTRA>), dim3(grid), dim3(PB_THREADS),
                     sizeof(ProbeSmem), st, a);
  return hipGetLastError();
}

template <int THREADS, int LOG_NB, bool PCOUNT, bool SLAB = false, int OUT = 0>
static hipError_t launch_fast_t(const ProbeArgs& a, u32* irregular, u32* n_irregular, int grid,
                                hipStream_t st) {
  typedef FastSmem<THREADS, LOG_NB> Smem;
  static SmemAttrOnce attr_once;
  if (hipError_t e = ensure_max_smem(attr_once, reinterpret_cast<const void*>(probe_count_fast_kernel<THREADS, LOG_NB, PCOUNT, SLAB, OUT>), (size_t)sizeof(Smem)); e != hipSuccess) return e;
  if ((u32)grid > a.P) grid = (int)a.P;
  if (grid < 1) grid = 1;
  hipLaunchKernelGGL((probe_count_fast_kernel<THREADS, LOG_NB, PCOUNT, SLAB, OUT>), dim3(grid), dim3(THREADS),
                     sizeof(Smem), st, a, irregular, n_irregular);
  return hipGetLastError();
}

hipError_t launch_probe_count_fast(const ProbeArgs& a, u32* irregular, u32* n_irregular, bool big,
                                   bool per_partition_counts, int num_cus, hipStream_t st) {
  if (per_partition_counts) {
    if (big) return launch_fast_t<1024, BIG_LOG_NB, true>(a, irregular, n_irregular, num_cus * 4, st);
    return launch_fast_t<512, 11, true>(a, irregular, n_irregular, num_cus * 3 * 4, st);
  }
  if (big) return launch_fast_t<1024, BIG_LOG_NB, false>(a, irregular, n_irregular, num_cus * 4, st);
  return launch_fast_t<512, 11, false>(a, irregular, n_irregular, num_cus * 3 * 4, st);
}

static bool slab_operands_ok(const ProbeArgs& a) {
  const u64 pieces = (u64)a.P * SLAB_KB;
  return a.r_cnt && a.s_cnt && a.r_cnt_n >= pieces && a.s_cnt_n >= pieces && a.r_rows >= pieces * a.r_cap &&
         a.s_rows >= pieces * a.s_cap;
}

hipError_t launch_probe_write_uniq(const ProbeArgs& a, bool slab, int num_cus, hipStream_t st) {
  if (slab && !slab_operands_ok(a)) return hipErrorInvalidValue;
  if (slab) return launch_fast_t<1024, BIG_LOG_NB, false, true, 1>(a, nullptr, nullptr, num_cus * 4, st);
  return launch_fast_t<1024, BIG_LOG_NB, false, false, 1>(a, nullptr, nullptr, num_cus * 4, st);
}

template <bool SLAB, bool FK, bool EXTRA, bool PB = false>
static hipError_t launch_sorted_t(const ProbeArgs& a, u64* lookback, bool chained, int key_low, int grid, hipStream_t st) {
  typedef typename std::conditional<FK, SortedFkSmem<1024>, SortedSmem<1024>>::type Smem;
  static_assert(sizeof(Smem) <= 160 * 1024, "one workgroup's LDS");
  if constexpr (FK && !PB) {
    if (a.extra & 4u) return launch_sorted_t<SLAB, FK, EXTRA, true>(a, lookback, chained, key_low, grid, st);
  }
// ... 35 lines not shown
  if (slab && !slab_operands_ok(a)) return hipErrorInvalidValue;
  int grid = (fk && shape == 1) ? 2 * num_cus : num_cus;
  if ((u32)grid > a.P) grid = (int)a.P;
  if (grid < 1) grid = 1;
  if (fk && shape == 1)
    return launch_sorted_shape<SWF_HALF_THREADS, SWF_HALF_ROWS, SWF_HALF_CAPB, SWF_HALF_LOGB>(a, slab, lookback, chained, key_low, grid, st);
  if (fk && shape == 2)
    return launch_sorted_shape<1024, SWF_WIDE_ROWS, SWF_WIDE_CAPB, SWF_LOGB>(a, slab, lookback, chained, key_low, grid, st);
  if (slab) return fk ? launch_sorted_x<true, true>(a, lookback, chained, key_low, grid, st)
                      : launch_sorted_x<true, false>(a, lookback, chained, key_low, grid, st);
  return fk ? launch_sorted_x<false, true>(a, lookback, chained, key_low, grid, st)
            : launch_sorted_x<false, false>(a, lookback, chained, key_low, grid, st);
}

__global__ void slab_np_kernel(const u32* __restrict__ cnt, u32 P, u64* __restrict__ out) {
  u32 p = blockIdx.x * blockDim.x + threadIdx.x;
  if (p < P) {
    const u32* q = cnt + (u64)p * SLAB_KB;
    out[p] = (u64)q[0] + q[1] + q[2] + q[3];
  }
}
hipError_t launch_slab_np(const u32* cnt, u32 P, u64* out, hipStream_t st) {
  hipLaunchKernelGGL(slab_np_kernel, dim3((P + 255) / 256), dim3(256), 0, st, cnt, P, out);
  return hipGetLastError();
}

hipError_t launch_probe_count_ext(const ProbeArgs& a, u32* irregular, u32* n_irregular, bool slab,
                                  int num_cus, hipStream_t st) {
  if (slab && !slab_operands_ok(a)) return hipErrorInvalidValue;
  if (slab) return launch_fast_t<1024, BIG_LOG_NB, false, true, 2>(a, nullptr, nullptr, num_cus * 4, st);
  return launch_fast_t<1024, BIG_LOG_NB, false, false, 2>(a, irregular, n_irregular, num_cus * 4, st);
}

hipError_t launch_probe_count_slab(const ProbeArgs& a, int num_cus, hipStream_t st) {
  if (!slab_operands_ok(a)) return hipErrorInvalidValue;
  return launch_fast_t<1024, BIG_LOG_NB, false, true>(a, nullptr, nullptr, num_cus * 4, st);
}

hipError_t launch_probe(const ProbeArgs& a, int mode, bool first_wins, bool extra, int grid,
                        hipStream_t st) {
  if (!a.item_list && (u64)grid > (u64)a.P * a.Q) grid = (int)((u64)a.P * a.Q);
  if (grid < 1) grid = 1;
  if (a.s_ppi) {
    if (!a.s_cnt || (mode != 0 && mode != 3) || (mode == 3 && (!a.out_key || !a.out_rval || !a.out_sval || a.out_cap == 0)) || (first_wins && !a.matched) || a.s_wa == 0 || (u64)a.P * a.s_wa * a.s_cap > 0xFFFFFFFFull || (u64)a.Q * a.s_ppi < a.s_wa || (u64)(a.Q - 1) * a.s_ppi >= a.s_wa ||
        a.s_cnt_n < (u64)a.P * a.s_wa || a.s_rows < (u64)a.P * a.s_wa * a.s_cap)
      return hipErrorInvalidValue;
  } else if (a.s_cnt && (a.s_cnt_n < (u64)a.P * a.Q || a.s_rows < (u64)a.P * a.Q * a.s_cap || (u64)a.P * a.Q * a.s_cap > 0xFFFFFFFFull))
    return hipErrorInvalidValue;
#define HMJ_DISPATCH(M)                                                          \
  if (first_wins)                                                                \
    return extra ? launch_probe_t<M, true, true>(a, grid, st)                    \
                 : launch_probe_t<M, true, false>(a, grid, st);                  \
  else                                                                           \
    return extra ? launch_probe_t<M, false, true>(a, grid, st)                   \
                 : launch_probe_t<M, false, false>(a, grid, st);
  if (mode == 3 && !a.s_ppi) return hipErrorInvalidValue;
  if (mode == 0) {
    HMJ_DISPATCH(0)
  } else if (mode == 3) {
    HMJ_DISPATCH(3)
  } else if (mode == 1) {
    HMJ_DISPATCH(1)
  } else {
    if (first_wins) return launch_probe_t<2, true, false>(a, grid, st);
    return launch_probe_t<2, false, false>(a, grid, st);
  }
#undef HMJ_DISPATCH
}
// ... 427 lines not shown
```

hashmergejoin_amd/csrc/radix.hip:

```cpp
#include <cstdlib>
#include <cstring>

#include <type_traits>

#include "hmj_dev.h"
#include "hmj_launch.h"

namespace hmj {

template <int OWN>
__device__ __forceinline__ u32 owner_digit(u64 key, int shift, u32 mask, const OwnerFn& f) {
  if (OWN == 1) return (u32)__umul64hi(mix64(key), (u64)f.G);
  if (OWN == 2) {
    u32 d = 0;
#pragma unroll
    for (int i = 0; i < kMaxRanks - 1; i++) d += ((u32)i + 1 < f.G && key >= f.spl[i]) ? 1u : 0u;
    return d;
  }
  return (u32)(key >> shift) & mask;
}

template <int OWN>
__global__ __launch_bounds__(RP_THREADS) void radix_hist_kernel(const Tup* __restrict__ in, u32 n,
                                                                int shift, u32 mask,
// ... 177 lines not shown
    for (int h = 0; h < 2; h++) {
      Tup v[RP_ITEMS / 2];
#pragma unroll
      for (int r = 0; r < RP_ITEMS / 2; r++) {
        const u32 i = (h * (RP_ITEMS / 2) + r) * RP_THREADS + tid;
        if (FULL || i < tile_n) v[r] = sm.stage[i];
      }
      if (h == 0) {
#pragma unroll
        for (int r = 0; r < RP_ITEMS / 2; r++) {
          Tup z;
          z.key = 0;
          z.val = 0;
          sm.stage[r * RP_THREADS + tid] = z;
        }
      }
#pragma unroll
      for (int r = 0; r < RP_ITEMS / 2; r++) {
        const u32 i = (h * (RP_ITEMS / 2) + r) * RP_THREADS + tid;
        if (FULL || i < tile_n) {
          const u32 d = OWN ? owner_digit<OWN>(v[r].key, shift, mask, own) : digit_of<HI>(v[r].key, shift, mask);
          store_stream(&out[sm.delta[d] + i], v[r]);
        }
      }
    }
    for (int i = tid; i < RP_WAVES * RP_MAXD / 2; i += RP_THREADS)
      reinterpret_cast<u32*>(&sm.wcnt[0][0])[i] = 0;
    lds_barrier();
  }
}

constexpr int WC_ITEMS = 4;
constexpr int WC_LINE = 8;

#ifndef HMJ_WC_PLAN1
#define HMJ_WC_PLAN1 0
#endif
#ifndef HMJ_WC_FULLTILE
#define HMJ_WC_FULLTILE 1
#endif
#ifndef HMJ_WC_NOBAR5
#define HMJ_WC_NOBAR5 1
#endif
#ifdef HMJ_STAMPS
__device__ unsigned long long g_wc_stamps[32];
struct WcStamps {
  u32 acc[14];
  u64 last;
  int base;
  __device__ __forceinline__ void begin() {
    asm volatile("s_waitcnt vmcnt(0)" ::: "memory");
    last = __builtin_amdgcn_s_memtime();
  }
  __device__ __forceinline__ void mark(int i) {
    const u64 now = __builtin_amdgcn_s_memtime();
    acc[i] += (u32)(now - last);
    last = now;
  }
  __device__ __forceinline__ void flush() {
    if ((threadIdx.x & 63) == 0)
      for (int i = 0; i < 14; i++) atomicAdd(&g_wc_stamps[base + i], (unsigned long long)acc[i]);
  }
};
#define WC_STAMP_ARG , WcStamps& stamps
#define WC_STAMP_PASS , stamps
#define WC_MARK(i) stamps.mark(i)
#define WC_VMWAIT() asm volatile("s_waitcnt vmcnt(0)" ::: "memory")
#else
#define WC_STAMP_ARG
#define WC_STAMP_PASS
#define WC_MARK(i)
#define WC_VMWAIT()
#endif

template <int THREADS, int MAXD>
struct WcSmem {
  static constexpr int TILE = THREADS * WC_ITEMS;
  static constexpr int WAVES = THREADS / kWave;
  static constexpr int ZROWS = WAVES * MAXD * 8 / 16;
  static constexpr int MAXLINES = TILE / WC_LINE + 2 * MAXD;
  static_assert(ZROWS <= TILE && ZROWS % THREADS == 0, "lane masks must alias whole row slabs");
  static_assert(MAXD <= THREADS && MAXD * WC_LINE == TILE, "one digit per thread; carry == tile slots");
  union {
    Tup stage[TILE];
    u64 lanemask[WAVES][MAXD];
  };
  Tup carry[MAXD][WC_LINE];
  u16 wcnt[WAVES][MAXD];
  u32 tile_off[MAXD];
  u32 cflush[MAXD];
  static constexpr bool HAS_CF_TILE = MAXD <= 256;
  u32 cf_tile[HAS_CF_TILE ? MAXD : 1];
  u32 plan[MAXD];
  u32 pend[MAXD];
  u32 line_off[MAXD];
  u16 line_tab[MAXLINES];
  u32 total_lines;
  u32 scratch[WAVES + 1];
};

struct NoLimit {
  __device__ __forceinline__ u32 operator()(u32) const { return 0xFFFFFFFFu; }
};
template <int THREADS, int MAXD, bool HI, bool ALLVALID, bool LIMIT, typename Prefetch, typename Limit>
__device__ __forceinline__ void wc_tile(WcSmem<THREADS, MAXD>& sm, Tup (&t)[WC_ITEMS], u32 tile_n,
                                        Tup* __restrict__ out, int shift, u32 mask, u32 D,
                                        Prefetch&& prefetch, const Limit& limit, bool* ovf WC_STAMP_ARG) {
  typedef WcSmem<THREADS, MAXD> Smem;
  constexpr int WAVES = Smem::WAVES;
  const int tid = threadIdx.x, lane = tid & 63, w = tid >> 6;
  u16* wc = &sm.wcnt[w][0];
  u64* lm = &sm.lanemask[w][0];
  const u64 lanebit = 1ull << lane;
  const u32 wbase = (u32)w * (WC_ITEMS * 64) + lane;

  u32 dr[WC_ITEMS];
#ifdef HMJ_STAMPS
  stamps.last = __builtin_amdgcn_s_memtime();
  WC_VMWAIT();
  WC_MARK(0);
  stamps.acc[11]++;
#endif
#pragma unroll
  for (int r = 0; r < WC_ITEMS; r++) {
    u32 d = 0, rank = 0;
    if (ALLVALID || wbase + r * 64 < tile_n) {
      d = digit_of<HI>(t[r].key, shift, mask);
      __hip_atomic_fetch_or(&lm[d], lanebit, __ATOMIC_RELAXED, __HIP_MEMORY_SCOPE_WORKGROUP);
      const u64 m = __hip_atomic_load(&lm[d], __ATOMIC_RELAXED, __HIP_MEMORY_SCOPE_WORKGROUP);
      const u32 old = __hip_atomic_load(&wc[d], __ATOMIC_RELAXED, __HIP_MEMORY_SCOPE_WORKGROUP);
      const u32 below = popc_below(m);
      if (below == 0) {
        __hip_atomic_store(&lm[d], 0ull, __ATOMIC_RELAXED, __HIP_MEMORY_SCOPE_WORKGROUP);
        __hip_atomic_store(&wc[d], (u16)(old + (u32)__popcll(m)), __ATOMIC_RELAXED,
                           __HIP_MEMORY_SCOPE_WORKGROUP);
      }
      rank = old + below;
    }
    dr[r] = (d << 16) | rank;
  }
  WC_MARK(1);
  lds_barrier();
  WC_MARK(2);

#if HMJ_WC_PLAN1
  if (w == 0) {
    constexpr int DPL = MAXD / kWave;
    u32 cnt[DPL], nl[DPL], pd[DPL], cf[DPL], fl[DPL];
#pragma unroll
    for (int j = 0; j < DPL; j++) {
      const u32 d = (u32)j * kWave + lane;
      cnt[j] = nl[j] = pd[j] = cf[j] = fl[j] = 0;
      if (d < D) {
        u32 c[WAVES];
#pragma unroll
        for (int k = 0; k < WAVES; k++) c[k] = sm.wcnt[k][d];
        u32 run = 0;
#pragma unroll
        for (int k = 0; k < WAVES; k++) {
          sm.wcnt[k][d] = (u16)run;
          run += c[k];
        }
        cnt[j] = run;
        pd[j] = sm.pend[d];
        cf[j] = sm.cflush[d];
        u32 avail = pd[j] + run;
        if (LIMIT && cf[j] + avail > limit(d)) {
          *ovf = true;
          avail = 0;
          pd[j] = 0;
        }
        const u32 tail = (cf[j] + avail) & (WC_LINE - 1);
        fl[j] = (tail >= avail) ? 0u : avail - tail;
        nl[j] = fl[j] ? (((cf[j] & (WC_LINE - 1)) + fl[j] + WC_LINE - 1) >> 3) : 0u;
        sm.pend[d] = avail - fl[j];
        sm.cflush[d] = cf[j] + fl[j];
      }
    }
    u32 running = 0;
#pragma unroll
    for (int j = 0; j < DPL; j++) {
      const u32 d = (u32)j * kWave + lane;
      const u32 v = (nl[j] << 16) | cnt[j];
      const u32 incl = wave_incl_scan_u32(v, lane);
      const u32 sc = running + incl - v;
      running += (u32)__builtin_amdgcn_readlane((int)incl, 63);
      if (d < D) {
        const u32 loff = sc >> 16;
        sm.tile_off[d] = sc & 0xFFFFu;
        if constexpr (Smem::HAS_CF_TILE) sm.cf_tile[d] = cf[j];
        sm.plan[d] = (fl[j] << 8) | pd[j];
        sm.line_off[d] = loff;
        for (u32 l = 0; l < nl[j]; l++) sm.line_tab[loff + l] = (u16)d;
      }
    }
    if (lane == 0) sm.total_lines = running >> 16;
  }
#else
  {
    u32 cnt = 0, nl = 0, pd = 0, cf = 0, fl = 0;
    if ((u32)tid < D) {
#pragma unroll
      for (int k = 0; k < WAVES; k++) {
        u32 c = sm.wcnt[k][tid];
        sm.wcnt[k][tid] = (u16)cnt;
        cnt += c;
      }
      pd = sm.pend[tid];
      cf = sm.cflush[tid];
      u32 avail = pd + cnt;
      if (LIMIT && cf + avail > limit((u32)tid)) {
        *ovf = true;
        avail = 0;
        pd = 0;
      }
      const u32 tail = (cf + avail) & (WC_LINE - 1);
      fl = (tail >= avail) ? 0u : avail - tail;
      nl = fl ? (((cf & (WC_LINE - 1)) + fl + WC_LINE - 1) >> 3) : 0u;
      sm.pend[tid] = avail - fl;
      sm.cflush[tid] = cf + fl;
    }
    u32 tot;
    const u32 sc = block_excl_scan_u32<THREADS, false>((nl << 16) | cnt, sm.scratch, &tot);
    if ((u32)tid < D) {
      const u32 loff = sc >> 16;
      sm.tile_off[tid] = sc & 0xFFFFu;
      if constexpr (Smem::HAS_CF_TILE) sm.cf_tile[tid] = cf;
      sm.plan[tid] = (fl << 8) | pd;
      sm.line_off[tid] = loff;
      for (u32 l = 0; l < nl; l++) sm.line_tab[loff + l] = (u16)tid;
    }
    if (tid == 0) sm.total_lines = tot >> 16;
  }
#endif
  WC_MARK(3);
  lds_barrier();
  WC_MARK(4);

#pragma unroll
  for (int r = 0; r < WC_ITEMS; r++) {
    if (ALLVALID || wbase + r * 64 < tile_n) {
      const u32 d = dr[r] >> 16;
      sm.stage[sm.tile_off[d] + sm.wcnt[w][d] + (dr[r] & 0xFFFFu)] = t[r];
    }
  }
  WC_MARK(5);
  prefetch();
  WC_MARK(12);
  lds_barrier();
  WC_MARK(6);

  {
    const u32 TL = sm.total_lines, k = (u32)tid & (WC_LINE - 1);
    for (u32 L = (u32)tid >> 3; L < TL; L += THREADS / WC_LINE) {
      const u32 d = sm.line_tab[L];
      const u32 pl = sm.plan[d], fl = pl >> 8, pd = pl & 0xFFu;
      u32 cfd;
      if constexpr (Smem::HAS_CF_TILE) cfd = sm.cf_tile[d];
      else cfd = sm.cflush[d] - fl;
      const u32 grow = (cfd & ~(u32)(WC_LINE - 1)) + (L - sm.line_off[d]) * WC_LINE + k;
      const u32 j = grow - cfd;
      if (j < fl) store_stream(&out[grow], (j < pd) ? sm.carry[d][j] : sm.stage[sm.tile_off[d] + j - pd]);
    }
  }
  u64 keep_k[WC_ITEMS], keep_v[WC_ITEMS];
  u32 has = 0;
#pragma unroll
  for (int q = 0; q < WC_ITEMS; q++) {
    const u32 s = q * THREADS + tid, d = s >> 3, k = s & (WC_LINE - 1);
    u32 idx = 0;
    if (d < D && k < sm.pend[d]) {
      const u32 pl = sm.plan[d], fl = pl >> 8, pd = pl & 0xFFu;
      if (fl != 0 || k >= pd) {
        idx = sm.tile_off[d] + (fl ? fl - pd + k : k - pd);
        has |= 1u << q;
      }
    }
    const Tup kv = sm.stage[idx];
    keep_k[q] = kv.key;
    keep_v[q] = kv.val;
  }
  WC_MARK(7);
  lds_barrier();
  WC_MARK(8);
#pragma unroll
  for (int q = 0; q < WC_ITEMS; q++) {
    const u32 s = q * THREADS + tid;
    if (has & (1u << q)) {
      Tup kv;
      kv.key = keep_k[q];
      kv.val = keep_v[q];
      sm.carry[s >> 3][s & (WC_LINE - 1)] = kv;
    }
  }
#if HMJ_WC_NOBAR5
  {
    constexpr int ZR = MAXD * 8 / 16;
    Tup z;
    z.key = 0;
    z.val = 0;
#pragma unroll
    for (int r = 0; r < ZR / kWave; r++) sm.stage[w * ZR + r * kWave + lane] = z;
    u32* wz = reinterpret_cast<u32*>(&sm.wcnt[w][0]);
#pragma unroll
    for (int r = 0; r < MAXD / 2 / kWave; r++) wz[r * kWave + lane] = 0;
  }
  WC_MARK(9);
  WC_MARK(10);
#else
#pragma unroll
  for (int r = 0; r < WC_ITEMS; r++) {
    if (r * THREADS < Smem::ZROWS) {
      Tup z;
      z.key = 0;
      z.val = 0;
      sm.stage[r * THREADS + tid] = z;
    }
  }
  for (int i = tid; i < WAVES * MAXD / 2; i += THREADS) reinterpret_cast<u32*>(&sm.wcnt[0][0])[i] = 0;
  WC_MARK(9);
  lds_barrier();
  WC_MARK(10);
#endif
}

template <int THREADS, int MAXD>
__device__ __forceinline__ void wc_flush_carry(WcSmem<THREADS, MAXD>& sm, Tup* __restrict__ out, u32 D) {
  const int tid = threadIdx.x;
  lds_barrier();
#pragma unroll
  for (int q = 0; q < WC_ITEMS; q++) {
    const u32 s = q * THREADS + tid, d = s >> 3, k = s & (WC_LINE - 1);
    if (d < D && k < sm.pend[d]) store_stream(&out[sm.cflush[d] + k], sm.carry[d][k]);
  }
}

template <int THREADS, int MAXD>
__device__ __forceinline__ void wc_clear(WcSmem<THREADS, MAXD>& sm) {
  constexpr int WAVES = WcSmem<THREADS, MAXD>::WAVES;
  const int tid = threadIdx.x;
  for (int i = tid; i < WAVES * MAXD / 2; i += THREADS) reinterpret_cast<u32*>(&sm.wcnt[0][0])[i] = 0;
  for (int i = tid; i < WAVES * MAXD; i += THREADS) (&sm.lanemask[0][0])[i] = 0;
}

template <int THREADS, int MAXD, bool HI, bool FULL>
__global__ __launch_bounds__(THREADS, (THREADS * (MAXD <= 256 ? 2 : 1)) / 256) void radix_scatter_wc_kernel(
    const Tup* __restrict__ in, Tup* __restrict__ out, u32 n, u32 n_full, int shift, int bits,
    u32 rows_per_block, u32 worker_base, const u32* __restrict__ hist_scanned,
    const u32* __restrict__ totals, u32 nblk, u64* __restrict__ offsets_out) {
  typedef WcSmem<THREADS, MAXD> Smem;
  constexpr int TILE = Smem::TILE;
  extern __shared__ __attribute__((aligned(16))) unsigned char smem_raw[];
  Smem& sm = *reinterpret_cast<Smem*>(smem_raw);
  const u32 D = 1u << bits, mask = D - 1;
  const int tid = threadIdx.x, lane = tid & 63, w = tid >> 6;
  const u32 worker = worker_base + blockIdx.x;

  {
    u32 t = ((u32)tid < D) ? totals[tid] : 0, tot;
    u32 base = block_excl_scan_u32<THREADS>(t, sm.scratch, &tot);
    if ((u32)tid < D) {
      sm.cflush[tid] = base + hist_scanned[(u64)tid * nblk + worker];
      sm.pend[tid] = 0;
      if (offsets_out && worker == 0) {
        offsets_out[tid] = base;
        if ((u32)tid == D - 1) offsets_out[D] = n;
      }
    }
    wc_clear(sm);
  }
  __syncthreads();

// ... 10 lines not shown
  const u32 wbase = (u32)w * (WC_ITEMS * 64) + lane;

  Tup t[WC_ITEMS];
#pragma unroll
  for (int r = 0; r < WC_ITEMS; r++)
    if (FULL || begin + wbase + r * 64 < end) t[r] = load_stream(&in[begin + wbase + r * 64]);

  bool ovf = false;
#ifdef HMJ_STAMPS
  WcStamps stamps = {};
#endif
  for (u64 tile = begin; tile < end; tile += TILE) {
    const u32 tile_n = FULL ? (u32)TILE : (u32)(end - tile);
    wc_tile<THREADS, MAXD, HI, FULL, false>(
        sm, t, tile_n, out, shift, mask, D,
        [&]() {
          if (FULL && tile + TILE < end) {
            const Tup* src = in + tile + TILE;
#pragma unroll
            for (int r = 0; r < WC_ITEMS; r++) t[r] = load_stream(&src[wbase + r * 64]);
          }
        },
        NoLimit(), &ovf WC_STAMP_PASS);
  }
  wc_flush_carry(sm, out, D);
#ifdef HMJ_STAMPS
  stamps.flush();
#endif
}

struct NoXform {
  static constexpr bool kStrided = false;
};
template <int THREADS, int MAXD, bool HI, typename Xform>
__device__ __forceinline__ void slab_a_body(const Tup* __restrict__ in, u32 n, int shift, int bits, u32 rows_per_worker,
                                            Tup* __restrict__ slab, u32 CA, u32 WA, u32* __restrict__ cnt_out,
                                            u64* __restrict__ accum, u32 worker_base, Xform& xf) {
  typedef WcSmem<THREADS, MAXD> Smem;
  constexpr int TILE = Smem::TILE;
  extern __shared__ __attribute__((aligned(16))) unsigned char smem_raw[];
  Smem& sm = *reinterpret_cast<Smem*>(smem_raw);
  const u32 D = 1u << bits, mask = D - 1;
  const int tid = threadIdx.x, lane = tid & 63, w = tid >> 6;
  const u32 worker = worker_base + blockIdx.x;
  const auto limit = [=](u32 d) { return (d * WA + worker) * CA + CA; };
  if ((u32)tid < D) {
    sm.cflush[tid] = ((u32)tid * WA + worker) * CA;
    sm.pend[tid] = 0;
  }
  wc_clear(sm);
  __syncthreads();
  const u64 begin = (u64)worker * rows_per_worker;
  u64 end = begin + rows_per_worker;
  if (end > n) end = n;
  const u32 wbase = (u32)w * (WC_ITEMS * 64) + lane;
  bool ovf = false;
#ifdef HMJ_STAMPS
  WcStamps stamps = {};
#endif
  if constexpr (Xform::kStrided) {
    constexpr u32 CH = RANK_PASS_CHUNK_ROWS, IPC = CH / 64, CPT = TILE / CH;
    static_assert(WC_ITEMS % IPC == 0 && IPC >= 1, "a wave's rows of a tile are whole chunks");
    const u64 n_chunks = ((u64)n + CH - 1) / CH, whole_chunks = n / CH;
    const u32 tail = n % CH;
    const u32 slot = (u32)(((u64)worker * xf.slot_mult) % WA);
    const u64 my_whole = whole_chunks > slot ? (whole_chunks - slot + WA - 1) / WA : 0;
    auto chunk_of = [&](u64 k, u32 c) { return (k * CPT + c) * WA + slot; };
    auto rows_of = [&](u64 k) {
      const u64 first = k * CPT;
      const u32 nv = my_whole > first ? (u32)((my_whole - first < CPT) ? my_whole - first : CPT) : 0u;
      return nv * CH + ((nv < CPT && tail && chunk_of(k, nv) == whole_chunks) ? tail : 0u);
    };
    if (chunk_of(0, 0) < n_chunks) {
      Tup t[WC_ITEMS];
      auto load_tile = [&](u64 k) {
#pragma unroll
        for (int r = 0; r < WC_ITEMS; r++) {
          const u64 q = chunk_of(k, (u32)w * (WC_ITEMS / IPC) + r / IPC) * CH + (r % IPC) * 64 + lane;
          t[r] = load_stream(&in[q < n ? q : n - 1]);
        }
      };
      load_tile(0);
      for (u64 k = 0; chunk_of(k, 0) < n_chunks; k++) {
        const u32 tile_n = rows_of(k);
        auto prefetch = [&]() {
          if (chunk_of(k + 1, 0) < n_chunks) load_tile(k + 1);
        };
        xf(t, tile_n, wbase);
        if (HMJ_WC_FULLTILE && tile_n == (u32)TILE)
          wc_tile<THREADS, MAXD, HI, true, true>(sm, t, tile_n, slab, shift, mask, D, prefetch, limit, &ovf WC_STAMP_PASS);
        else
          wc_tile<THREADS, MAXD, HI, false, true>(sm, t, tile_n, slab, shift, mask, D, prefetch, limit, &ovf WC_STAMP_PASS);
      }
      wc_flush_carry(sm, slab, D);
    }
  } else if (begin < end) {
    Tup t[WC_ITEMS];
    {
      const u32 tn = (u32)((end - begin < TILE) ? end - begin : TILE);
#pragma unroll
      for (int r = 0; r < WC_ITEMS; r++) {
        const u32 q = wbase + r * 64;
        t[r] = load_stream(&in[begin + (q < tn ? q : tn - 1)]);
      }
    }
    for (u64 tile = begin; tile < end; tile += TILE) {
      const u32 tile_n = (u32)((end - tile < TILE) ? end - tile : TILE);
      auto prefetch = [&]() {
        if (tile + TILE < end) {
          const u64 nt = tile + TILE;
          const u32 tn = (u32)((end - nt < TILE) ? end - nt : TILE);
          const Tup* src = in + nt;
#pragma unroll
          for (int r = 0; r < WC_ITEMS; r++) {
            const u32 q = wbase + r * 64;
            t[r] = load_stream(&src[q < tn ? q : tn - 1]);
          }
        }
      };
      if constexpr (!std::is_same<Xform, NoXform>::value) xf(t, tile_n, wbase);
      if (HMJ_WC_FULLTILE && tile_n == (u32)TILE)
        wc_tile<THREADS, MAXD, HI, true, true>(sm, t, tile_n, slab, shift, mask, D, prefetch, limit, &ovf WC_STAMP_PASS);
      else
        wc_tile<THREADS, MAXD, HI, false, true>(sm, t, tile_n, slab, shift, mask, D, prefetch, limit, &ovf WC_STAMP_PASS);
    }
    wc_flush_carry(sm, slab, D);
  }
  if ((u32)tid < D) cnt_out[(u32)tid * WA + worker] = sm.cflush[tid] + sm.pend[tid] - ((u32)tid * WA + worker) * CA;
  if (ovf) atomicOr(&accum[ACC_ERR], ERR_SLAB);
#ifdef HMJ_STAMPS
  stamps.flush();
#endif
}

#ifndef HMJ_B_ADDR
#define HMJ_B_ADDR 2
#endif
#ifndef HMJ_B_NT
#define HMJ_B_NT 0
#endif
#ifdef HMJ_DEV
__device__ u32 g_b_ablate;
static bool g_b_addr_alt = false;
#endif
constexpr int SLAB_MAXSEG = 512;

template <int THREADS, int MAXD, bool HI, int ADDR>
__global__ __launch_bounds__(THREADS, (THREADS * (MAXD <= 256 ? 2 : 1)) / 256) void radix_slab_b_kernel(
    const Tup* __restrict__ slab_a, const u32* __restrict__ cnt_a, u32 CA, u32 WA, int bits_a, int shift,
    int bits, Tup* __restrict__ slab_b, u32 CB, u32* __restrict__ cnt_b, u64* __restrict__ accum, u32 KB) {
  typedef WcSmem<THREADS, MAXD> Smem;
  constexpr int TILE = Smem::TILE;
  static_assert(SLAB_MAXSEG <= THREADS, "one A-slab count per thread in the prologue scan");
  extern __shared__ __attribute__((aligned(16))) unsigned char smem_raw[];
  Smem& sm = *reinterpret_cast<Smem*>(smem_raw);
  u32* pre = reinterpret_cast<u32*>(smem_raw + sizeof(Smem));
  const u32 D = 1u << bits, mask = D - 1;
  const int tid = threadIdx.x, lane = tid & 63, w = tid >> 6;
  const u32 dA = blockIdx.x / KB, k = blockIdx.x % KB;
  const auto limit = [=](u32 d) { return (((d << bits_a) | dA) * KB + k) * CB + CB; };
  const u32 w0 = (u32)((u64)k * WA / KB), w1 = (u32)((u64)(k + 1) * WA / KB), ns = w1 - w0;
  {
    const u32 c = ((u32)tid < ns) ? cnt_a[dA * WA + w0 + tid] : 0;
    u32 tot;
    const u32 ex = block_excl_scan_u32<THREADS>(c, sm.scratch, &tot);
    if ((u32)tid < ns) pre[tid] = ex;
    if (tid == 0) pre[ns] = tot;
    if ((u32)tid < D) {
      sm.cflush[tid] = ((((u32)tid << bits_a) | dA) * KB + k) * CB;
      sm.pend[tid] = 0;
    }
    wc_clear(sm);
  }
  __syncthreads();
  const u32 total = pre[ns];
#ifdef HMJ_DEV
  const u32 abl = g_b_ablate;
#else
  constexpr u32 abl = 0;
#endif
  const u32 wbase = (u32)w * (WC_ITEMS * 64) + lane;
  (void)wbase;
  const Tup* __restrict__ bucket = slab_a + (u64)(dA * WA + w0) * CA;
  bool ovf = false;
#ifdef HMJ_STAMPS
  WcStamps stamps = {};
  stamps.base = 16;
#endif
  if (total) {
    Tup t[WC_ITEMS];
    if constexpr (ADDR != 0) {
    u32 d_s0 = 0, d_b0 = 0, d_b1 = 0, d_b2 = 0, d_b3 = 0;
    const float slabs_per_row = (float)ns / (float)total;
    auto plan1 = [&](u32 tile_begin) {
      u32 q0 = tile_begin + (u32)w * (WC_ITEMS * 64) + (u32)(lane & 3) * 64;
      q0 = q0 < total ? q0 : total - 1;
      u32 g = (u32)((float)q0 * slabs_per_row);
      g = g < ns ? g : ns - 1;
      u32 lo = g >= 3 ? g - 3 : 0;
      u32 pw[8];
#pragma unroll
      for (int i = 0; i < 8; i++) pw[i] = pre[lo + i < ns ? lo + i : ns];
      u32 j = 0;
#pragma unroll
      for (int i = 1; i < 8; i++) j += pw[i] <= q0 ? 1u : 0u;
      const bool bracketed = pw[0] <= q0 && pw[7] > q0;
      lo += j;
      if (__any(!bracketed)) {
        u32 hi = ns;
        lo = 0;
#pragma unroll
        for (int it = 0; it < 9; it++) {
          const u32 mid = (lo + hi) >> 1;
          const bool le = pre[mid] <= q0, act = hi - lo > 1;
          lo = (act && le) ? mid : lo;
          hi = (act && !le) ? mid : hi;
        }
      }
      d_s0 = lo;
      d_b0 = pre[lo];
      d_b1 = pre[lo + 1 < ns ? lo + 1 : ns];
      d_b2 = pre[lo + 2 < ns ? lo + 2 : ns];
      d_b3 = pre[lo + 3 < ns ? lo + 3 : ns];
// ... 114 lines not shown
#pragma unroll
        for (int r = 0; r < WC_ITEMS; r++) {
          u32 q = wq0 + lane + r * 64;
          q = q < total ? q : total - 1;
          u32 sx = u_s0;
          while (sx + 1 < ns && pre[sx + 1] <= q) sx++;
          off[r] = (u64)sx * CA + (q - pre[sx]);
        }
      }
#pragma unroll
      for (int r = 0; r < WC_ITEMS; r++) t[r] = HMJ_B_NT ? load_stream(&bucket[off[r]]) : bucket[off[r]];
    };
    auto plan = [&](u32 tb) {
      if constexpr (ADDR == 2) plan2(tb); else plan1(tb);
    };
    auto issue = [&](u32 tb) {
      if constexpr (ADDR == 2) issue2(tb); else issue1(tb);
    };
    if (abl != 4) plan(0);
    issue(0);
    if ((u32)TILE < total && abl != 4) plan(TILE);
    for (u32 tile = 0; tile < total; tile += TILE) {
      const u32 tile_n = (total - tile < (u32)TILE) ? total - tile : (u32)TILE;
      auto prefetch = [&]() {
        if (tile + TILE < total) {
          issue(tile + TILE);
#ifdef HMJ_STAMPS
          stamps.mark(13);
#endif
          if (tile + 2 * TILE < total && abl != 4) plan(tile + 2 * TILE);
        }
      };
#ifdef HMJ_DEV
      if (abl == 1 || abl == 4) {
#pragma unroll
        for (int r = 0; r < WC_ITEMS; r++)
          if (t[r].key == 0) t[r].key = (u64)(tile + (u32)tid + r * THREADS + blockIdx.x * 7919u + 1) * 0x9E3779B97F4A7C15ull;
      }
#endif
      if (HMJ_WC_FULLTILE && tile_n == (u32)TILE)
        wc_tile<THREADS, MAXD, HI, true, true>(sm, t, tile_n, slab_b, shift, mask, D, prefetch, limit, &ovf WC_STAMP_PASS);
      else
        wc_tile<THREADS, MAXD, HI, false, true>(sm, t, tile_n, slab_b, shift, mask, D, prefetch, limit, &ovf WC_STAMP_PASS);
    }
    } else {
    u32 seg = 0;
    auto load = [&](u32 tile_begin) {
      const u32 tn = (total - tile_begin < (u32)TILE) ? total - tile_begin : (u32)TILE;
      while (seg + 1 < ns && pre[seg + 1] <= tile_begin) seg++;
      u32 s = seg;
      u64 off[WC_ITEMS];
#pragma unroll
      for (int r = 0; r < WC_ITEMS; r++) {
        u32 q = wbase + r * 64;
        q = tile_begin + (q < tn ? q : tn - 1);
        while (s + 1 < ns && pre[s + 1] <= q) s++;
        off[r] = (u64)s * CA + (q - pre[s]);
      }
#pragma unroll
      for (int r = 0; r < WC_ITEMS; r++) t[r] = HMJ_B_NT ? load_stream(&bucket[off[r]]) : bucket[off[r]];
    };
    load(0);
    for (u32 tile = 0; tile < total; tile += TILE) {
      const u32 tile_n = (total - tile < (u32)TILE) ? total - tile : (u32)TILE;
      wc_tile<THREADS, MAXD, HI, false, true>(
          sm, t, tile_n, slab_b, shift, mask, D,
          [&]() {
            if (tile + TILE < total) load(tile + TILE);
          },
          limit, &ovf WC_STAMP_PASS);
// ... 98 lines not shown
    atomicMax(&rng[1], (unsigned long long)mx);
  }
  if (eq_r) atomicAdd(&same[0], eq_r);
  if (eq_s) atomicAdd(&same[1], eq_s);
  if (up_r) atomicAdd(&order[0], up_r);
  if (dn_r) atomicAdd(&order[1], dn_r);
  if (up_s) atomicAdd(&order[2], up_s);
  if (dn_s) atomicAdd(&order[3], dn_s);
  __syncthreads();
  {
    const u64 lo = rng[0], span = rng[1] - rng[0];
#pragma unroll
    for (int k = 0; k < 2; k++)
      if (myvalid[k] && span) atomicAdd(&bins[(u32)((mykey[k] - lo) / ((span >> 6) + 1)) & 63u], 1u);
  }
  __syncthreads();
  if (tid == 0) {
    out[0] = acc;
    out[1] = ref;
    out[2] = (u64)same[0] | ((u64)order[0] << 16) | ((u64)order[1] << 32);
    out[3] = (u64)same[1] | ((u64)order[2] << 16) | ((u64)order[3] << 32);
    out[4] = rng[0];
    out[5] = rng[1];
    u32 nonempty = 0, big = 0;
    for (int i = 0; i < 64; i++) {
      nonempty += bins[i] ? 1u : 0u;
      big = bins[i] > big ? bins[i] : big;
    }
    out[6] = nonempty;
    out[7] = big;
  }
}

template <int THREADS, int MAXD, bool HI>
__global__ __launch_bounds__(THREADS, (THREADS * (MAXD <= 256 ? 2 : 1)) / 256) void radix_slab_a_kernel(
    const Tup* __restrict__ in, u32 n, int shift, int bits, u32 rows_per_worker, Tup* __restrict__ slab,
    u32 CA, u32 WA, u32* __restrict__ cnt_out, u64* __restrict__ accum, u32 worker_base) {
  NoXform xf;
  slab_a_body<THREADS, MAXD, HI, NoXform>(in, n, shift, bits, rows_per_worker, slab, CA, WA, cnt_out, accum, worker_base, xf);
}

template <bool CUT>
struct RankXform {
  static constexpr bool kStrided = CUT;
  u32 slot_mult;
  const Tup* __restrict__ tab;
  u32 mask;
  int hshift;
  int tb, pre;
  u64 svmin, svrange, mult;
  u64 acc_s;
  u64 n_rows;
  bool miss;
  __device__ __forceinline__ void operator()(Tup (&t)[WC_ITEMS], u32 tile_n, u32 wbase) {
    u32 slot[WC_ITEMS];
    bool live[WC_ITEMS], want[WC_ITEMS];
    u32 found = 0;
#pragma unroll
    for (int r = 0; r < WC_ITEMS; r++) {
      want[r] = wbase + (u32)r * 64 < tile_n;
      slot[r] = gt_hash(t[r].key, hshift);
      if (want[r]) acc_s += t[r].val;
      if (want[r]) n_rows++;
      live[r] = want[r] && t[r].key != GT_EMPTY;
    }
    u64 rank[WC_ITEMS] = {};
    gt_walk<WC_ITEMS>(tab, mask, slot, live, [&](int r, const Tup& e) {
      const bool eq = e.key == t[r].key;
      if (eq) {
        rank[r] = e.val;
        found |= 1u << r;
      }
// ... 10 lines not shown
        t[r].key = rank[r];
      }
    }
  }
};
template <int THREADS, int MAXD, bool CUT>
__global__ __launch_bounds__(THREADS, (THREADS * (MAXD <= 256 ? 2 : 1)) / 256) void radix_slab_a_rank_kernel(
    const Tup* __restrict__ in, u32 n, int shift, int bits, u32 rows_per_worker, Tup* __restrict__ slab, u32 CA, u32 WA,
    u32* __restrict__ cnt_out, u64* __restrict__ accum, const Tup* __restrict__ tab, int log_cap, bool extra, int tb, u64 svmin, u64 svrange,
    int pre, u64 mult, u32 slot_mult) {
  RankXform<CUT> xf{slot_mult, tab, (1u << log_cap) - 1, 64 - log_cap, tb, pre, svmin, svrange, mult, 0ull, 0ull, false};
  slab_a_body<THREADS, MAXD, false, RankXform<CUT>>(in, n, shift, bits, rows_per_worker, slab, CA, WA, cnt_out, accum, 0u, xf);
  __shared__ u64 wsum[THREADS / kWave], wrows[THREADS / kWave];
  const int lane = threadIdx.x & 63, wv = threadIdx.x >> 6;
  const u64 ws = wave_sum_u64(xf.acc_s), wr = wave_sum_u64(xf.n_rows);
  const bool any_miss = __any(xf.miss);
  if (lane == 0) {
    wsum[wv] = ws;
    wrows[wv] = wr;
  }
  if (any_miss && lane == 0) atomicOr(reinterpret_cast<unsigned long long*>(&accum[ACC_ERR]), (unsigned long long)ERR_FASTPATH);
  __syncthreads();
  if (threadIdx.x == 0) {
    u64 tot = 0, rows = 0;
    for (int w = 0; w < THREADS / kWave; w++) {
      tot += wsum[w];
      rows += wrows[w];
    }
    if (tot) atomicAdd(reinterpret_cast<unsigned long long*>(&accum[ACC_SUM_S]), (unsigned long long)tot);
    if (extra && tot) atomicAdd(reinterpret_cast<unsigned long long*>(&accum[ACC_SUM_P]), (unsigned long long)tot);
    if (rows) atomicAdd(reinterpret_cast<unsigned long long*>(&accum[ACC_N]), (unsigned long long)rows);
  }
}
template <int THREADS, int MAXD, bool HI>
static hipError_t launch_slab_a_t(const void* in, u32 n, int shift, int bits, u32 rpw, void* slab, u32 CA,
                                  u32 WA, u32* cnt, u64* accum, hipStream_t st, u32 w_begin, u32 w_end) {
  typedef WcSmem<THREADS, MAXD> Smem;
  const size_t smem = sizeof(Smem);
  static_assert(sizeof(Smem) <= 160 * 1024, "slab pass A: LDS");
  static SmemAttrOnce attr_once;
  if (hipError_t e = ensure_max_smem(attr_once, reinterpret_cast<const void*>(radix_slab_a_kernel<THREADS, MAXD, HI>), (size_t)smem); e != hipSuccess) return e;
  if (w_end > WA) w_end = WA;
  if (w_begin >= w_end) return hipSuccess;
  hipLaunchKernelGGL((radix_slab_a_kernel<THREADS, MAXD, HI>), dim3(w_end - w_begin), dim3(THREADS), smem, st,
                     static_cast<const Tup*>(in), n, shift, bits, rpw, static_cast<Tup*>(slab), CA, WA, cnt,
                     accum, w_begin);
  return hipGetLastError();
}

template <int THREADS, int MAXD, bool HI>
static hipError_t launch_slab_b_t(const void* slab_a, const u32* cnt_a, u32 CA, u32 WA, int bits_a, int shift,
                                  int bits, void* slab_b, u32 CB, u32* cnt_b, u64* accum, hipStream_t st, u32 KB) {
  typedef WcSmem<THREADS, MAXD> Smem;
  const size_t smem = sizeof(Smem) + (SLAB_MAXSEG + 1) * sizeof(u32);
  static_assert(sizeof(Smem) + (SLAB_MAXSEG + 1) * sizeof(u32) <= 160 * 1024, "slab pass B: LDS");
#ifdef HMJ_DEV
  if (g_b_addr_alt) {
    constexpr int ALT = HMJ_B_ADDR == 2 ? 1 : 2;
    static SmemAttrOnce attr_alt;
    if (hipError_t e = ensure_max_smem(attr_alt, reinterpret_cast<const void*>(radix_slab_b_kernel<THREADS, MAXD, HI, ALT>), (size_t)smem); e != hipSuccess) return e;
    hipLaunchKernelGGL((radix_slab_b_kernel<THREADS, MAXD, HI, ALT>), dim3((1u << bits_a) * KB), dim3(THREADS), smem, st,
                       static_cast<const Tup*>(slab_a), cnt_a, CA, WA, bits_a, shift, bits,
                       static_cast<Tup*>(slab_b), CB, cnt_b, accum, KB);
    return hipGetLastError();
  }
#endif
  static SmemAttrOnce attr_once;
  if (hipError_t e = ensure_max_smem(attr_once, reinterpret_cast<const void*>(radix_slab_b_kernel<THREADS, MAXD, HI, HMJ_B_ADDR>), (size_t)smem); e != hipSuccess) return e;
  hipLaunchKernelGGL((radix_slab_b_kernel<THREADS, MAXD, HI, HMJ_B_ADDR>), dim3((1u << bits_a) * KB), dim3(THREADS), smem, st,
                     static_cast<const Tup*>(slab_a), cnt_a, CA, WA, bits_a, shift, bits,
                     static_cast<Tup*>(slab_b), CB, cnt_b, accum, KB);
  return hipGetLastError();
}

static u32 slab_cap(double mean, double fan) {
  double c = mean + 8.0 * __builtin_sqrt(fan * mean) + 24.0;
  return ((u32)c + 8) & ~7u;
}
u32 slab_capacity(double mean, double fan) { return slab_cap(mean, fan < 1.0 ? 1.0 : fan); }
bool slab_geometry(u32 n, int bits_a, int bits_b, SlabGeom* g, u32 kb, double fan, double density) {
  if (bits_a < 1 || bits_a > SLAB_MAX_BITS || bits_b < 1 || bits_b > SLAB_MAX_BITS) return false;
  const u32 tile = bits_a > 8 ? 4096 : 2048;
  u64 tiles = ((u64)n + tile - 1) / tile;
  u64 max_workers = 2048;
#ifdef HMJ_DEV
  if (const char* e = getenv("HMJ_SLAB_WORKERS")) max_workers = (u64)atoi(e) > 0 ? (u64)atoi(e) : max_workers;
#endif
  u64 tpw = (tiles + max_workers - 1) / max_workers;
  if (tpw == 0) tpw = 1;
  g->WA = (u32)((tiles + tpw - 1) / tpw);
  g->rpw = (u32)(tpw * tile);
  if (kb == 0) kb = SLAB_KB;
  g->KB = kb;
  if (g->WA < kb || (g->WA + kb - 1) / kb > (u32)SLAB_MAXSEG) return false;
  if (fan < 1.0) fan = 1.0;
  if (density < 1.0) density = 1.0;
  const double fan_a = 1.0 + 4.0 * (double)g->rpw * fan / (double)(n ? n : 1);
  g->CA = slab_cap(density * (double)g->rpw / (double)(1u << bits_a), fan_a < fan ? fan_a : fan);
  g->CB = slab_cap(density * (double)n / (double)(1u << bits_a) / (double)kb / (double)(1u << bits_b), fan);
  const u64 rows_a = (u64)(1u << bits_a) * g->WA * g->CA;
  const u64 rows_b = (u64)(1u << (bits_a + bits_b)) * kb * g->CB;
  g->rows_a = rows_a;
  g->rows_b = rows_b;
  return rows_a < 0xFFFFFFF0ull && rows_b < 0xFFFFFFF0ull;
}

bool slab_geometry_one_pass(u32 n, int bits, double keys_per_digit, u32 max_workers, SlabGeom* g, double density) {
  if (bits < 1 || bits > SLAB_MAX_BITS || max_workers == 0) return false;
  const u32 tile = bits > 8 ? 4096 : 2048;
  const u64 tiles = ((u64)n + tile - 1) / tile;
  u64 tpw = (tiles + max_workers - 1) / max_workers;
  if (tpw == 0) tpw = 1;
  g->WA = (u32)((tiles + tpw - 1) / tpw);
  g->rpw = (u32)(tpw * tile);
  g->KB = 0;
  g->CB = 0;
  g->rows_b = 0;
  if (density < 1.0) density = 1.0;
  const double mean = density * (double)g->rpw / (double)(1u << bits);
  if (keys_per_digit < 1.0) keys_per_digit = 1.0;
  g->CA = slab_cap(mean, 1.0 + mean / keys_per_digit);
  g->rows_a = (u64)(1u << bits) * g->WA * g->CA;
  return g->WA >= 1 && g->rows_a < 0xFFFFFFF0ull;
}

hipError_t launch_slab_a(const void* in, u32 n, int shift, int bits, const SlabGeom& g, void* slab_a, u64 slab_a_rows,
                         u32* cnt_a, u64 cnt_a_n, u64* accum, hipStream_t st, u32 w_begin, u32 w_end) {
  if (bits < 1 || bits > SLAB_MAX_BITS || g.WA == 0 || g.CA == 0 || (u64)g.WA * g.rpw < n) return hipErrorInvalidValue;
  if (slab_a_rows < ((u64)g.WA << bits) * g.CA || cnt_a_n < ((u64)g.WA << bits)) return hipErrorInvalidValue;
  if (((u64)g.WA << bits) * g.CA >= 0xFFFFFFF0ull) return hipErrorInvalidValue;
  const bool hi = shift >= 32;
#define HMJ_SLAB_A(T, M, H) launch_slab_a_t<T, M, H>(in, n, shift, bits, g.rpw, slab_a, g.CA, g.WA, cnt_a, accum, st, w_begin, w_end)
  if (bits > 8) return hi ? HMJ_SLAB_A(1024, 512, true) : HMJ_SLAB_A(1024, 512, false);
  return hi ? HMJ_SLAB_A(512, 256, true) : HMJ_SLAB_A(512, 256, false);
#undef HMJ_SLAB_A
}

hipError_t launch_slab_a_ranks(const void* in, u32 n, int shift, int bits, const SlabGeom& g, void* slab_a, u64 slab_a_rows, u32* cnt_a,
                               u64 cnt_a_n, u64* accum, const void* tab, int log_cap, bool extra, int tb, u64 svmin, u64 svrange, int pre,
                               u64 mult, hipStream_t st) {
  if (bits < 1 || bits > SLAB_MAX_BITS || g.WA == 0 || g.CA == 0 || (u64)g.WA * g.rpw < n || !tab || log_cap < 4 || log_cap > 30 || tb < 0 ||
      tb > 16 || pre < 0 || pre > 32 || shift < 0 || shift > 4 || (shift && tb))
    return hipErrorInvalidValue;
  if (slab_a_rows < ((u64)g.WA << bits) * g.CA || cnt_a_n < ((u64)g.WA << bits)) return hipErrorInvalidValue;
  if (((u64)g.WA << bits) * g.CA >= 0xFFFFFFF0ull) return hipErrorInvalidValue;
  u32 slot_mult = 1;
  if (tb > 0 && g.WA > 2) {
    auto gcd = [](u32 a, u32 b) {
      while (b) {
        const u32 t = a % b;
        a = b;
        b = t;
      }
      return a;
    };
    slot_mult = (u32)((double)g.WA * 0.6180339887498949);
    if (slot_mult < 1) slot_mult = 1;
    while (gcd(slot_mult, g.WA) != 1) slot_mult++;
  }
#define HMJ_SLAB_AR(T, M, C)                                                                                                          \
  {                                                                                                                                   \
    typedef WcSmem<T, M> Smem;                                                                                                        \
    static SmemAttrOnce once;                                                                                                         \
    if (hipError_t e = ensure_max_smem(once, reinterpret_cast<const void*>(radix_slab_a_rank_kernel<T, M, C>), sizeof(Smem)); e != hipSuccess) \
      return e;                                                                                                                       \
    hipLaunchKernelGGL((radix_slab_a_rank_kernel<T, M, C>), dim3(g.WA), dim3(T), sizeof(Smem), st, static_cast<const Tup*>(in), n, shift, bits, g.rpw, \
                       static_cast<Tup*>(slab_a), g.CA, g.WA, cnt_a, accum, static_cast<const Tup*>(tab), log_cap, extra, tb, svmin, svrange, pre, mult, \
                       slot_mult);                                                                                                    \
  }
  if (tb > 0) {
    if (bits > 8) HMJ_SLAB_AR(1024, 512, true) else HMJ_SLAB_AR(512, 256, true)
  } else {
    if (bits > 8) HMJ_SLAB_AR(1024, 512, false) else HMJ_SLAB_AR(512, 256, false)
  }
#undef HMJ_SLAB_AR
  return hipGetLastError();
}

hipError_t launch_slab_b(const void* slab_a, const u32* cnt_a, int bits_a, int shift, int bits,
                         const SlabGeom& g, void* slab_b, u64 slab_b_rows, u32* cnt_b, u64 cnt_b_n, u64* accum, hipStream_t st) {
  if (bits < 1 || bits > SLAB_MAX_BITS || bits_a < 1 || bits_a > SLAB_MAX_BITS || g.KB == 0 || g.WA < g.KB ||
      (g.WA + g.KB - 1) / g.KB > (u32)SLAB_MAXSEG)
    return hipErrorInvalidValue;
  const u64 pieces = ((u64)g.KB << (bits_a + bits));
  if (slab_b_rows < pieces * g.CB || cnt_b_n < pieces || pieces * g.CB >= 0xFFFFFFF0ull) return hipErrorInvalidValue;
  const bool hi = shift >= 32;
#define HMJ_SLAB_B(T, M, H) launch_slab_b_t<T, M, H>(slab_a, cnt_a, g.CA, g.WA, bits_a, shift, bits, slab_b, g.CB, cnt_b, accum, st, g.KB)
  if (bits > 8) return hi ? HMJ_SLAB_B(1024, 512, true) : HMJ_SLAB_B(1024, 512, false);
  return hi ? HMJ_SLAB_B(512, 256, true) : HMJ_SLAB_B(512, 256, false);
#undef HMJ_SLAB_B
}

__global__ __launch_bounds__(256) void key_exact_kernel(const Tup* __restrict__ R, u32 nb, const Tup* __restrict__ S, u32 np,
                                                        u64 ref, bool ref_is_first_key, u64* __restrict__ out) {
  if (ref_is_first_key) ref = nb ? R[0].key : (np ? S[0].key : 0);
  u64 x = 0, mn = ~0ull, mx = 0;
  const u64 stride = (u64)gridDim.x * blockDim.x;
  for (u64 i = (u64)blockIdx.x * blockDim.x + threadIdx.x; i < nb; i += stride) {
    const u64 k = R[i].key;
    x |= k ^ ref;
    mn = k < mn ? k : mn;
    mx = k > mx ? k : mx;
  }
  for (u64 i = (u64)blockIdx.x * blockDim.x + threadIdx.x; i < np; i += stride) x |= S[i].key ^ ref;
#pragma unroll
  for (int o = kWave / 2; o > 0; o >>= 1) {
    x |= __shfl_xor(x, o, kWave);
    const u64 a2 = __shfl_xor(mn, o, kWave), b2 = __shfl_xor(mx, o, kWave);
    mn = a2 < mn ? a2 : mn;
    mx = b2 > mx ? b2 : mx;
  }
  __shared__ u64 wx[4], wmn[4], wmx[4];
  if ((threadIdx.x & 63) == 0) {
    wx[threadIdx.x >> 6] = x;
    wmn[threadIdx.x >> 6] = mn;
    wmx[threadIdx.x >> 6] = mx;
  }
  __syncthreads();
  if (threadIdx.x == 0) {
// ... 231 lines not shown
```

include/hmj.h:

```cpp
#ifndef HMJ_H
#define HMJ_H

#include <stddef.h>
#include <stdint.h>

#ifdef __cplusplus
extern "C" {
#endif

typedef struct hmj_ctx hmj_ctx;

#define HMJ_OK 0
#define HMJ_E_ARG (-1)
#define HMJ_E_NODEV (-2)
#define HMJ_E_OOM (-3)
#define HMJ_E_HIP (-4)
#define HMJ_E_UNSUPPORTED (-5)

#define HMJ_E_RCCL (-6)
#define HMJ_E_PEER (-7)
#define HMJ_E_TIMEOUT (-8)

#define HMJ_MATERIALIZE 0x01u
#define HMJ_ORDERED 0x02u
// ... 36 lines not shown
  uint32_t path;
  int32_t key_prefix_bits;
  int32_t key_window_low;
  uint32_t n_probe_items;
  float ms_scatter_pass[2];
} hmj_timing;
#define HMJ_PATH_SLAB 0x001u
#define HMJ_PATH_EXACT 0x002u
#define HMJ_PATH_UNIQ_WRITE 0x004u
#define HMJ_PATH_SPLIT 0x008u
#define HMJ_PATH_WINDOW 0x010u
#define HMJ_PATH_ORDER_DEFERRED 0x020u
#define HMJ_PATH_ORDER_BY_KEY 0x040u
#define HMJ_PATH_PREPARED 0x080u
#define HMJ_PATH_CHUNKED_BUILD 0x100u
#define HMJ_PATH_HOT_KEY_HINT 0x200u
#define HMJ_PATH_SLAB_PROBE 0x400u
#define HMJ_PATH_SORTED_WRITE 0x800u
#define HMJ_PATH_SORTED_FK 0x1000u
#define HMJ_PATH_DENSE_BUILD 0x2000u
#define HMJ_PATH_SORTED_FK_HALF 0x8000u
#define HMJ_PATH_SORTED_FK_WIDE 0x20000u
#define HMJ_PATH_LOOKBACK_TIMEOUT 0x10000u
#define HMJ_PATH_PRESORTED 0x40000u
#define HMJ_PATH_SLAB_ONE_PASS 0x80000u
#define HMJ_PATH_ORDER_BY_RANK_SORT 0x200000u
#define HMJ_PATH_RANK_RUNS 0x1000000u
#define HMJ_PATH_RANK_LOOKUP_IN_PASS 0x2000000u
#define HMJ_PATH_SORT_MSD 0x4000000u
#define HMJ_PATH_KEY_RANGES 0x8000000u
#define HMJ_PATH_ORDERED_EXPANSION 0x400000u
#define HMJ_PATH_LDS_TABLE 0x800000u
#define HMJ_PATH_GLOBAL_TABLE 0x100000u
#define HMJ_PATH_HOST_PIPELINE 0x4000u

typedef struct {
  uint32_t struct_size;
  uint32_t path;
  int32_t radix_bits, radix_passes, pass_bits[4];
  int32_t key_prefix_bits, key_window_low;
  uint32_t n_partitions;
  uint32_t probe_items;
  uint32_t attempts;
  uint32_t refused;
  uint32_t cooling;
  uint64_t workload;
} hmj_plan_desc;
#define HMJ_REFUSED_GTABLE_SHAPE 0x0001u
#define HMJ_REFUSED_GTABLE_COOLING 0x0002u
#define HMJ_REFUSED_GTABLE_GAVE_UP 0x0004u
#define HMJ_REFUSED_RANK_SORT_MODEL 0x0008u
#define HMJ_REFUSED_RANK_SORT_COOLING 0x0010u
#define HMJ_REFUSED_RANK_SORT_GAVE_UP 0x0020u
#define HMJ_REFUSED_SLAB_SHAPE 0x0040u
#define HMJ_REFUSED_SLAB_COOLING 0x0080u
#define HMJ_REFUSED_SLAB_SORTED_INPUT 0x0100u
#define HMJ_REFUSED_SLAB_OVERFLOW 0x0200u
#define HMJ_REFUSED_FAST_WRITE_COOLING 0x0400u
#define HMJ_REFUSED_FAST_WRITE_GAVE_UP 0x0800u
#define HMJ_REFUSED_SLAB_PROBE_COOLING 0x1000u
#define HMJ_REFUSED_SLAB_PROBE_OVERFLOW 0x2000u
#define HMJ_REFUSED_PREFIX_VIOLATED 0x4000u
#define HMJ_REFUSED_EXPANSION_GAVE_UP 0x8000u
#define HMJ_COOL_UNIQ_WRITE 0x001u
#define HMJ_COOL_SORTED_WRITE 0x002u
#define HMJ_COOL_GTABLE 0x004u
#define HMJ_COOL_GTABLE_WRITE 0x008u
#define HMJ_COOL_RANK_SORT 0x010u
#define HMJ_COOL_RANK_SORT_SLAB 0x020u
#define HMJ_COOL_EXPANSION 0x040u
#define HMJ_COOL_SORT_SLAB 0x080u
#define HMJ_COOL_SLAB 0x100u
#define HMJ_COOL_SLAB_PROBE 0x200u
#define HMJ_COOL_ONE_PASS_WRITE 0x400u
#define HMJ_COOL_EXACT_PREFIX 0x800u
#define HMJ_COOL_RANK_RUNS 0x1000u
#define HMJ_COOL_SORT_MSD 0x2000u

int hmj_create(hmj_ctx** out, int device_id);
void hmj_destroy(hmj_ctx* ctx);
#define HMJ_STREAM_OWN ((void*)(intptr_t)-1)
int hmj_set_stream(hmj_ctx* ctx, void* hip_stream);
int hmj_reserve(hmj_ctx* ctx, uint64_t n_build, uint64_t n_probe, uint64_t max_matches,
                uint32_t flags);
int hmj_set_radix_bits(hmj_ctx* ctx, int total_bits);
int hmj_autotune_radix_bits(hmj_ctx* ctx, uint64_t n_build, uint64_t n_probe, int apply, int* best_bits,
                            double ms[3]);
int hmj_set_key_prefix_bits(hmj_ctx* ctx, int bits);
int hmj_plan(uint64_t n_build, int* total_bits, int* n_passes, int pass_bits[4]);
#define HMJ_ABI_VERSION 5
int hmj_abi_version(void);
#define HMJ_PLACE_MAX_CAND 4
typedef struct {
  char name[16];
  uint64_t bytes;
  float fill_TBps;
  int candidates;
  float ms_search;
  int searched;
  int aborted;
  float budget_ms;
  float cand_ms_alloc[HMJ_PLACE_MAX_CAND];
  float cand_ms_fill[HMJ_PLACE_MAX_CAND];
  float cand_TBps[HMJ_PLACE_MAX_CAND];
} hmj_place_info;
int hmj_placement_info(hmj_ctx* ctx, hmj_place_info* out, int max_entries);
int hmj_last_plan(hmj_ctx* ctx, hmj_plan_desc* out);
int hmj_forget_workloads(hmj_ctx* ctx);
int hmj_set_profiling(hmj_ctx* ctx, int enabled);
int hmj_last_timing(hmj_ctx* ctx, hmj_timing* out);
// ... 347 lines not shown
```

Measured before the change: 34.30 billion.

## Scatter bare probe keys through slab passes for count-only joins

```diff
diff --git a/hashmergejoin_amd/__init__.py b/hashmergejoin_amd/__init__.py
--- a/hashmergejoin_amd/__init__.py
+++ b/hashmergejoin_amd/__init__.py
@@ -1,6 +1,6 @@
-from ._lib import (HMJ_BUILD_ANTI, HMJ_BUILD_OUTER, HMJ_BUILD_SEMI, HMJ_CHECKSUM, HMJ_COLS_HASHED, HMJ_COLS_NO_ROW, HMJ_COLS_PACKED, HMJ_FIRST_WINS, HMJ_FULL_OUTER, HMJ_GROUP_COUNT, HMJ_GROUP_MAX, HMJ_GROUP_MIN, HMJ_GROUP_ROW_MAP, HMJ_GROUP_SUM, HMJ_JOIN_ANTI, HMJ_JOIN_INNER, HMJ_JOIN_PROBE_OUTER, HMJ_JOIN_SEMI, HMJ_KIND_BUILD_SIDE, HMJ_KIND_PROBE_SIDE, HMJ_MATERIALIZE, HMJ_ORDERED, HMJ_PATH_CHUNKED_BUILD, HMJ_PATH_DENSE_BUILD,
+from ._lib import (HMJ_BUILD_ANTI, HMJ_BUILD_OUTER, HMJ_BUILD_SEMI, HMJ_CHECKSUM, HMJ_COOL_PROBE_KEYS, HMJ_COLS_HASHED, HMJ_COLS_NO_ROW, HMJ_COLS_PACKED, HMJ_FIRST_WINS, HMJ_FULL_OUTER, HMJ_GROUP_COUNT, HMJ_GROUP_MAX, HMJ_GROUP_MIN, HMJ_GROUP_ROW_MAP, HMJ_GROUP_SUM, HMJ_JOIN_ANTI, HMJ_JOIN_INNER, HMJ_JOIN_PROBE_OUTER, HMJ_JOIN_SEMI, HMJ_KIND_BUILD_SIDE, HMJ_KIND_PROBE_SIDE, HMJ_MATERIALIZE, HMJ_ORDERED, HMJ_PATH_CHUNKED_BUILD, HMJ_PATH_DENSE_BUILD,
                    HMJ_PATH_EXACT, HMJ_PATH_GLOBAL_TABLE, HMJ_PATH_HOST_PIPELINE, HMJ_PATH_HOT_KEY_HINT, HMJ_PATH_LOOKBACK_TIMEOUT, HMJ_PATH_ORDER_BY_KEY, HMJ_PATH_ORDER_BY_RANK_SORT, HMJ_PATH_ORDER_DEFERRED, HMJ_PATH_ORDERED_EXPANSION, HMJ_PATH_LDS_TABLE,
-                   HMJ_PATH_KEY_RANGES, HMJ_PATH_PREPARED, HMJ_PATH_PRESORTED, HMJ_PATH_RANK_RUNS, HMJ_PATH_SORT_MSD, HMJ_PATH_SLAB, HMJ_PATH_SLAB_ONE_PASS, HMJ_PATH_SLAB_PROBE, HMJ_PATH_SORTED_FK, HMJ_PATH_SORTED_FK_HALF, HMJ_PATH_SORTED_FK_WIDE, HMJ_PATH_SORTED_WRITE, HMJ_PATH_SPLIT, HMJ_PATH_UNIQ_WRITE, HMJ_PATH_WINDOW,
+                   HMJ_PATH_KEY_RANGES, HMJ_PATH_PREPARED, HMJ_PATH_PRESORTED, HMJ_PATH_PROBE_KEYS, HMJ_PATH_RANK_LOOKUP_IN_PASS, HMJ_PATH_RANK_RUNS, HMJ_PATH_SORT_MSD, HMJ_PATH_SLAB, HMJ_PATH_SLAB_ONE_PASS, HMJ_PATH_SLAB_PROBE, HMJ_PATH_SORTED_FK, HMJ_PATH_SORTED_FK_HALF, HMJ_PATH_SORTED_FK_WIDE, HMJ_PATH_SORTED_WRITE, HMJ_PATH_SPLIT, HMJ_PATH_UNIQ_WRITE, HMJ_PATH_WINDOW,
                    HMJ_KEY_FIXED, HMJ_KEY_LARGE_STRING, HMJ_MAX_KEY_COLS, HMJ_MAX_TAKE_COLS, HMJ_NULL_EQUAL, HMJ_STR_NO_ROW, HMJ_SUM_PROBE, HMJ_TAKE_NO_ROW, BuildJoinOpts, ColsJoinOpts, ColsKindOpts, ColsRel, ColsResult, ExchangeKindOpts, GroupOpts, GroupResult, HmjError, JoinOpts, JoinResult, KeyCol, KindCounts, MixedCol, MixedOpts, MixedRel, StrJoinOpts, StrKindOpts, StrRel, StrResult, TakeDst, TakeOpts, TakeSrc, TakeStrDst, TakeStrOpts, TakeStrSrc, Timing, Validity,
                    lib_path, load_library)
 from .join import Executor, HashMergeJoin, cols_key64, expected_groups, mixed_key64, pack_strings, pack_validity, plan, unpack_strings, unpack_validity
@@ -18,4 +18,4 @@
            "MixedCol", "MixedRel", "MixedOpts", "HMJ_KEY_FIXED", "HMJ_KEY_LARGE_STRING", "mixed_key64",
            "HMJ_NULL_EQUAL",
            "GroupOpts", "GroupResult", "HMJ_GROUP_COUNT", "HMJ_GROUP_SUM", "HMJ_GROUP_MIN", "HMJ_GROUP_MAX", "HMJ_GROUP_ROW_MAP",
-           "expected_groups"]
+           "expected_groups", "HMJ_PATH_PROBE_KEYS", "HMJ_COOL_PROBE_KEYS", "HMJ_PATH_RANK_LOOKUP_IN_PASS"]
diff --git a/hashmergejoin_amd/_lib.py b/hashmergejoin_amd/_lib.py
--- a/hashmergejoin_amd/_lib.py
+++ b/hashmergejoin_amd/_lib.py
@@ -29,6 +29,7 @@
 HMJ_PATH_LOOKBACK_TIMEOUT = 0x10000
 HMJ_PATH_SORTED_FK_WIDE = 0x20000
 HMJ_PATH_PRESORTED = 0x40000
+HMJ_PATH_PROBE_KEYS = 0x10000000
 
 _HERE = os.path.dirname(os.path.abspath(__file__))
 _U64P = C.POINTER(C.c_uint64)
@@ -260,7 +261,7 @@
 HMJ_COOL_UNIQ_WRITE, HMJ_COOL_SORTED_WRITE, HMJ_COOL_GTABLE, HMJ_COOL_GTABLE_WRITE = 0x1, 0x2, 0x4, 0x8
 HMJ_COOL_RANK_SORT, HMJ_COOL_RANK_SORT_SLAB, HMJ_COOL_EXPANSION, HMJ_COOL_SORT_SLAB = 0x10, 0x20, 0x40, 0x80
 HMJ_COOL_SLAB, HMJ_COOL_SLAB_PROBE, HMJ_COOL_ONE_PASS_WRITE, HMJ_COOL_EXACT_PREFIX = 0x100, 0x200, 0x400, 0x800
-HMJ_COOL_RANK_RUNS = 0x1000
+HMJ_COOL_RANK_RUNS, HMJ_COOL_SORT_MSD, HMJ_COOL_PROBE_KEYS = 0x1000, 0x2000, 0x4000
 
 
 class PlaceInfo(C.Structure):
diff --git a/hashmergejoin_amd/csrc/api.hip b/hashmergejoin_amd/csrc/api.hip
--- a/hashmergejoin_amd/csrc/api.hip
+++ b/hashmergejoin_amd/csrc/api.hip
@@ -85,7 +85,8 @@
          (gtable_sort_slab_cooldown ? HMJ_COOL_RANK_SORT_SLAB : 0u) | (expand_cooldown ? HMJ_COOL_EXPANSION : 0u) |
          (sort_slab_cooldown ? HMJ_COOL_SORT_SLAB : 0u) | (slab_cooldown ? HMJ_COOL_SLAB : 0u) | (slab_probe_cooldown ? HMJ_COOL_SLAB_PROBE : 0u) |
          (one_pass_write_cooldown ? HMJ_COOL_ONE_PASS_WRITE : 0u) | (exact_prefix_joins ? HMJ_COOL_EXACT_PREFIX : 0u) |
-         (rank_runs_cooldown ? HMJ_COOL_RANK_RUNS : 0u) | (sort_msd_cooldown ? HMJ_COOL_SORT_MSD : 0u);
+         (rank_runs_cooldown ? HMJ_COOL_RANK_RUNS : 0u) | (sort_msd_cooldown ? HMJ_COOL_SORT_MSD : 0u) |
+         (probe_keys_cooldown ? HMJ_COOL_PROBE_KEYS : 0u);
 }
 
 int wait_arrival(hmj_ctx* c, hipEvent_t ev) {
@@ -582,9 +583,10 @@
   return a;
 }
 
-static int slab_pass_a(hmj_ctx* c, const void* in, u32 n, int rel, int low, int bits, const hmj::SlabGeom& g, bool arriving) {
+static int slab_pass_a(hmj_ctx* c, const void* in, u32 n, int rel, int low, int bits, const hmj::SlabGeom& g, bool arriving,
+                       u32 row_bytes = 16) {
   u64* acc = (u64*)c->accum.p;
-  const u64 a_rows = c->slab_a.cap / 16, a_cnt = c->cnt_a.cap / 4;
+  const u64 a_rows = c->slab_a.cap / row_bytes, a_cnt = c->cnt_a.cap / 4;
   const int sp = span_begin(c, K_SCATTER, rel, 0);
   if (arriving) {
     u32 w_done = 0;
@@ -593,25 +595,25 @@
       const bool last = i + 1 == c->arrive_ev.size();
       const u32 w_end = last ? g.WA : (u32)std::min<u64>(g.WA, c->arrive_rows[i] / g.rpw);
       if (w_end > w_done) {
-        HIP_TRY(hmj::launch_slab_a(in, n, low, bits, g, c->slab_a.p, a_rows, (u32*)c->cnt_a.p, a_cnt, acc, c->stream, w_done, w_end));
+        HIP_TRY(hmj::launch_slab_a(in, n, low, bits, g, c->slab_a.p, a_rows, (u32*)c->cnt_a.p, a_cnt, acc, c->stream, w_done, w_end, row_bytes));
         w_done = w_end;
       }
     }
   } else {
-    HIP_TRY(hmj::launch_slab_a(in, n, low, bits, g, c->slab_a.p, a_rows, (u32*)c->cnt_a.p, a_cnt, acc, c->stream));
+    HIP_TRY(hmj::launch_slab_a(in, n, low, bits, g, c->slab_a.p, a_rows, (u32*)c->cnt_a.p, a_cnt, acc, c->stream, 0, 0xFFFFFFFFu, row_bytes));
   }
   span_end(c, sp);
-  c->timing.bytes_scatter += 32ull * n;
+  c->timing.bytes_scatter += (16ull + row_bytes) * n;
   return HMJ_OK;
 }
 static int slab_passes(hmj_ctx* c, const void* in, u32 n, int rel, int low, int ba, int bb, const hmj::SlabGeom& g, DevBuf& sb,
-                       DevBuf& cb, bool arriving) {
-  RC_TRY(slab_pass_a(c, in, n, rel, low, ba, g, arriving));
+                       DevBuf& cb, bool arriving, u32 row_bytes = 16) {
+  RC_TRY(slab_pass_a(c, in, n, rel, low, ba, g, arriving, row_bytes));
   const int sp = span_begin(c, K_SCATTER, rel, 1);
-  HIP_TRY(hmj::launch_slab_b(c->slab_a.p, (const u32*)c->cnt_a.p, ba, low + ba, bb, g, sb.p, sb.cap / 16, (u32*)cb.p, cb.cap / 4,
-                             (u64*)c->accum.p, c->stream));
+  HIP_TRY(hmj::launch_slab_b(c->slab_a.p, (const u32*)c->cnt_a.p, ba, low + ba, bb, g, sb.p, sb.cap / row_bytes, (u32*)cb.p, cb.cap / 4,
+                             (u64*)c->accum.p, c->stream, row_bytes));
   span_end(c, sp);
-  c->timing.bytes_scatter += 32ull * n;
+  c->timing.bytes_scatter += 2ull * row_bytes * n;
   return HMJ_OK;
 }
 
@@ -1199,7 +1201,17 @@
   RC_TRY(ensure_dev(c, c->cnt_br, (size_t)P * gr.KB * 4));
   RC_TRY(ensure_dev(c, c->cnt_bs, (size_t)P * gs.KB * 4));
   if (!reuse) RC_TRY(slab_passes(c, j.R, nb, 0, p.low, ba, bb, gr, c->slab_br, c->cnt_br, false));
-  if (!c->prepare_only) RC_TRY(slab_passes(c, j.S, np, 1, p.low, ba, bb, gs, c->slab_bs, c->cnt_bs, !c->arrive_ev.empty()));
+  hmj::SlabGeom gk;
+  const bool keys = j.flags == 0 && c->join_kind == 0 && !c->prepare_only && !p.fast_write && c->probe_keys &&
+                    c->wm->probe_keys_cooldown == 0 &&
+                    hmj::slab_geometry(np_plan, ba, bb, &gk, 0, (nb && np_plan > nb) ? (double)np_plan / (double)nb : 1.0, p.dense_scale, 8) &&
+                    gk.KB == gs.KB && gk.rows_a * 8 <= c->slab_a.cap && ((u64)gk.WA << ba) * 4 <= c->cnt_a.cap &&
+                    gk.rows_b * 8 <= c->slab_bs.cap && (u64)gk.WA * gk.rpw >= np;
+  const bool arriving = !c->arrive_ev.empty();
+  const size_t spans_before = c->spans.size();
+  const u64 bytes_before = c->timing.bytes_scatter;
+  if (!c->prepare_only)
+    RC_TRY(slab_passes(c, j.S, np, 1, p.low, ba, bb, keys ? gk : gs, c->slab_bs, c->cnt_bs, arriving, keys ? 8 : 16));
   u64* hh;
   if (c->prepare_only) {
     RC_TRY(read_accum(c, &hh));
@@ -1222,6 +1234,31 @@
 #ifdef HMJ_DEV
   sa.debug = c->dev_ablate;
 #endif
+  if (keys) {
+    hmj::ProbeArgs ka = sa;
+    ka.s_cap = gk.CB;
+    ka.s_rows = c->slab_bs.cap / 8;
+    const int spk = span_begin(c, K_PROBE_COUNT, -1);
+    HIP_TRY(hmj::launch_probe_count_slab(ka, c->num_cus, c->stream, true));
+    span_end(c, spk);
+    RC_TRY(read_accum(c, &hh));
+    if (hh[hmj::ACC_ERR] & hmj::ERR_SLAB) {
+      c->wm->slab_cooldown = 8;
+      return kRetryNoSlab;
+    }
+    if (!(hh[hmj::ACC_ERR] & hmj::ERR_PROBE_KEYS)) {
+      c->timing.path |= HMJ_PATH_PROBE_KEYS;
+      c->timing.bytes_probe_count = 16ull * nb + 8ull * np;
+      result_sums(j.out, hh);
+      j.out->sum_s = hh[hmj::ACC_PAD];
+      return HMJ_OK;
+    }
+    c->wm->probe_keys_cooldown = 64;
+    c->spans.resize(spans_before);
+    c->timing.bytes_scatter = bytes_before;
+    HIP_TRY(hipMemsetAsync(c->accum.p, 0, 8 * sizeof(u64), c->stream));
+    RC_TRY(slab_passes(c, j.S, np, 1, p.low, ba, bb, gs, c->slab_bs, c->cnt_bs, arriving));
+  }
   int sp = span_begin(c, K_PROBE_COUNT, -1);
   if (first || extra) {
     sa.extra = (extra ? 1u : 0u) | (first ? 2u : 0u);
@@ -1604,6 +1641,7 @@
   if (!c->prepare_only && c->prep.valid && !c->prep.slab && c->prep.ptr == R && c->prep.n == (u32)n_build) allow_slab = false;
   const bool materialize = flags & HMJ_MATERIALIZE;
   if (c->wm->slab_cooldown > 0 && allow_slab) c->wm->slab_cooldown--;
+  if (c->wm->probe_keys_cooldown > 0 && allow_slab && flags == 0 && !c->prepare_only) c->wm->probe_keys_cooldown--;
   if (c->wm->slab_probe_cooldown > 0 && allow_slab_probe) c->wm->slab_probe_cooldown--;
   if (c->wm->one_pass_write_cooldown > 0 && materialize && allow_slab_probe) c->wm->one_pass_write_cooldown--;
   JoinPlan p;
@@ -2545,6 +2583,7 @@
   hmj_ctx* c = new hmj_ctx();
   c->device = device_id;
   if (const char* e = getenv("HMJ_SLAB")) c->slab_mode = atoi(e);
+  if (const char* e = getenv("HMJ_PROBE_KEYS")) c->probe_keys = atoi(e) != 0;
   if (const char* e = getenv("HMJ_ONE_PASS_SLAB")) c->one_pass_slab = atoi(e) != 0;
   if (const char* e = getenv("HMJ_GTABLE")) c->gtable_mode = atoi(e) != 0;
   if (const char* e = getenv("HMJ_RANK_RUNS")) c->rank_runs_mode = atoi(e) != 0;
diff --git a/hashmergejoin_amd/csrc/hmj_ctx.h b/hashmergejoin_amd/csrc/hmj_ctx.h
--- a/hashmergejoin_amd/csrc/hmj_ctx.h
+++ b/hashmergejoin_amd/csrc/hmj_ctx.h
@@ -87,6 +87,7 @@
   int sort_slab_cooldown = 0;
   int sort_msd_cooldown = 0;
   int slab_cooldown = 0;
+  int probe_keys_cooldown = 0;
   int slab_probe_cooldown = 0;
   int one_pass_write_cooldown = 0;
   int exact_prefix_joins = 0;
@@ -209,6 +210,7 @@
   u64 sort_msd_min = 1ull << 22;
   bool sort_slab = true;
   u64 sort_slab_min = 1ull << 25;
+  bool probe_keys = true;
   int slab_mode = 1;
   bool staged_upload = false;
   bool host_pipeline = true;
diff --git a/hashmergejoin_amd/csrc/hmj_dev.h b/hashmergejoin_amd/csrc/hmj_dev.h
--- a/hashmergejoin_amd/csrc/hmj_dev.h
+++ b/hashmergejoin_amd/csrc/hmj_dev.h
@@ -37,6 +37,20 @@
   t.key = x.x;
   t.val = x.y;
   return t;
+#else
+  return *p;
+#endif
+}
+__device__ __forceinline__ void store_stream(u64* p, u64 v) {
+#if HMJ_STREAM_POLICY >= 1
+  __builtin_nontemporal_store(v, p);
+#else
+  *p = v;
+#endif
+}
+__device__ __forceinline__ u64 load_stream(const u64* p) {
+#if HMJ_STREAM_POLICY >= 2
+  return __builtin_nontemporal_load(p);
 #else
   return *p;
 #endif
@@ -106,6 +120,7 @@
 constexpr u64 ERR_SORTED = 64;
 constexpr u64 ERR_FASTPATH = 8;
 constexpr u64 ERR_GTABLE = 128;
+constexpr u64 ERR_PROBE_KEYS = 256;
 constexpr u64 ERR_PREFIX = 4;
 
 __device__ __forceinline__ u64 mix64(u64 x) {
diff --git a/hashmergejoin_amd/csrc/hmj_launch.h b/hashmergejoin_amd/csrc/hmj_launch.h
--- a/hashmergejoin_amd/csrc/hmj_launch.h
+++ b/hashmergejoin_amd/csrc/hmj_launch.h
@@ -46,13 +46,16 @@
   u32 WA, rpw, CA, CB, KB;
   u64 rows_a, rows_b;
 };
-bool slab_geometry(u32 n, int bits_a, int bits_b, SlabGeom* g, u32 kb = 0, double fan = 1.0, double density = 1.0);
+bool slab_geometry(u32 n, int bits_a, int bits_b, SlabGeom* g, u32 kb = 0, double fan = 1.0, double density = 1.0,
+                   u32 row_bytes = 16);
 bool slab_geometry_one_pass(u32 n, int bits, double keys_per_digit, u32 max_workers, SlabGeom* g, double density = 1.0);
 u32 slab_capacity(double mean, double fan);
 hipError_t launch_slab_a(const void* in, u32 n, int shift, int bits, const SlabGeom& g, void* slab_a, u64 slab_a_rows,
-                         u32* cnt_a, u64 cnt_a_n, u64* accum, hipStream_t st, u32 w_begin = 0, u32 w_end = 0xFFFFFFFFu);
+                         u32* cnt_a, u64 cnt_a_n, u64* accum, hipStream_t st, u32 w_begin = 0, u32 w_end = 0xFFFFFFFFu,
+                         u32 row_bytes = 16);
 hipError_t launch_slab_b(const void* slab_a, const u32* cnt_a, int bits_a, int shift, int bits,
-                         const SlabGeom& g, void* slab_b, u64 slab_b_rows, u32* cnt_b, u64 cnt_b_n, u64* accum, hipStream_t st);
+                         const SlabGeom& g, void* slab_b, u64 slab_b_rows, u32* cnt_b, u64 cnt_b_n, u64* accum, hipStream_t st,
+                         u32 row_bytes = 16);
 hipError_t launch_key_sample(const void* R, u32 nb, const void* S, u32 np, u64* out, hipStream_t st);
 hipError_t launch_key_exact(const void* R, u32 nb, const void* S, u32 np, u64 ref, u64* out, int num_cus, hipStream_t st,
                             bool ref_is_first_key = false);
@@ -99,7 +102,7 @@
                               bool set, u64 fill, int num_cus, hipStream_t st);
 hipError_t launch_probe_count_ext(const ProbeArgs& a, u32* irregular, u32* n_irregular, bool slab,
                                   int num_cus, hipStream_t st);
-hipError_t launch_probe_count_slab(const ProbeArgs& a, int num_cus, hipStream_t st);
+hipError_t launch_probe_count_slab(const ProbeArgs& a, int num_cus, hipStream_t st, bool probe_keys = false);
 hipError_t launch_probe_write_sorted(const ProbeArgs& a, bool slab, bool fk, int shape, u64* lookback, bool chained, int key_low,
                                      int num_cus, hipStream_t st);
 hipError_t launch_probe_write_uniq(const ProbeArgs& a, bool slab, int num_cus, hipStream_t st);
diff --git a/hashmergejoin_amd/csrc/probe.hip b/hashmergejoin_amd/csrc/probe.hip
--- a/hashmergejoin_amd/csrc/probe.hip
+++ b/hashmergejoin_amd/csrc/probe.hip
@@ -916,11 +916,11 @@
   }
 }
 
-template <int THREADS>
-__device__ __forceinline__ void fp_load_pieces(Tup (&t)[FP_ROWS], const Tup* __restrict__ base, u32 cap, u32 cnt_mine, int tid) {
+template <int THREADS, typename Row>
+__device__ __forceinline__ void fp_load_pieces(Row (&t)[FP_ROWS], const Row* __restrict__ base, u32 cap, u32 cnt_mine, int tid) {
   constexpr int QT = THREADS / 4;
   const u32 g = (u32)tid / QT, l = (u32)tid % QT;
-  const Tup* __restrict__ piece = base + (u64)g * cap;
+  const Row* __restrict__ piece = base + (u64)g * cap;
   const u32 last = cnt_mine ? cnt_mine - 1 : 0;
 #pragma unroll
   for (int k = 0; k < FP_ROWS; k++) {
@@ -929,17 +929,24 @@
   }
 }
 
-template <int THREADS, int LOG_NB, bool PCOUNT, bool SLAB, int OUT>
+__device__ __forceinline__ u64 fp_key(const Tup& r) { return r.key; }
+__device__ __forceinline__ u64 fp_val(const Tup& r) { return r.val; }
+__device__ __forceinline__ u64 fp_key(u64 r) { return r; }
+__device__ __forceinline__ u64 fp_val(u64) { return 0ull; }
+
+template <int THREADS, int LOG_NB, bool PCOUNT, bool SLAB, int OUT, bool KEYS = false>
 __global__ __launch_bounds__(THREADS, 4) void probe_count_fast_kernel(
     ProbeArgs a, u32* __restrict__ irregular, u32* __restrict__ n_irregular) {
   typedef FastSmem<THREADS, LOG_NB> Smem;
+  typedef typename std::conditional<KEYS, u64, Tup>::type PRow;
   constexpr u32 CAP = Smem::CAP, NB = 1u << LOG_NB;
   constexpr bool PIECES = SLAB && OUT == 0 && !PCOUNT && HMJ_PROBE_PIECES;
+  static_assert(!KEYS || PIECES, "bare probe keys: the piece-wise count form only");
   constexpr u32 QT = THREADS / 4, PIECE_CAP = FP_ROWS * QT;
   extern __shared__ __attribute__((aligned(16))) unsigned char smem_raw[];
   Smem& sm = *reinterpret_cast<Smem*>(smem_raw);
   const Tup* __restrict__ R = static_cast<const Tup*>(a.R);
-  const Tup* __restrict__ S = static_cast<const Tup*>(a.S);
+  const PRow* __restrict__ S = static_cast<const PRow*>(a.S);
   const u32* __restrict__ r_off = a.r_off;
   const u32* __restrict__ s_off = a.s_off;
   const u32* __restrict__ r_end = (SLAB || a.r_end == nullptr) ? a.r_off + 1 : a.r_end;
@@ -947,7 +954,7 @@
   const u32 P = a.P;
   const int tid = threadIdx.x;
   u64 acc_n = 0, acc_r = 0, acc_s = 0, acc_x = 0, acc_m = 0, acc_p = 0;
-  bool pfx_bad = false, giveup = false;
+  bool pfx_bad = false, giveup = false, keys_bad = false;
   for (u32 i = tid; i < NB; i += THREADS) sm.head[i] = 0;
   if (tid < 2) sm.itemcnt[tid] = 0;
   u32 epoch = 0;
@@ -956,7 +963,8 @@
   u32 p = blockIdx.x;
   u32 rb = 0, nb = 0, sb = 0, np = 0;
   bool regular = false;
-  Tup br[FP_ROWS], pr[FP_ROWS], pq[FP_ROWS];
+  Tup br[FP_ROWS];
+  PRow pr[FP_ROWS], pq[FP_ROWS];
   u32 r1 = 0, r2 = 0, r3 = 0, s1 = 0, s2 = 0, s3 = 0, r1n = 0, r2n = 0, r3n = 0, s1n = 0, s2n = 0, s3n = 0;
   u32 rm = 0, sm_ = 0, rmn = 0, smn = 0;
   const u32 my_piece = (u32)tid / QT;
@@ -986,16 +994,19 @@
       if (PIECES) {
         fp_load_pieces<THREADS>(br, R + (u64)p * SLAB_KB * a.r_cap, a.r_cap, rm, tid);
         fp_load_pieces<THREADS>(pr, S + (u64)p * SLAB_KB * a.s_cap, a.s_cap, sm_, tid);
-      } else if (SLAB) {
-        fp_load_slab<THREADS>(br, R + (u64)p * SLAB_KB * a.r_cap, a.r_cap, r1, r2, r3, nb, tid);
-        if (OUT == 0) fp_load_slab<THREADS>(pr, S + (u64)p * SLAB_KB * a.s_cap, a.s_cap, s1, s2, s3, np, tid);
-      } else {
-        fp_load<THREADS>(br, R + rb, nb, tid);
-        if (OUT == 0) fp_load<THREADS>(pr, S + sb, np, tid);
+      } else if constexpr (!KEYS) {
+        if (SLAB) {
+          fp_load_slab<THREADS>(br, R + (u64)p * SLAB_KB * a.r_cap, a.r_cap, r1, r2, r3, nb, tid);
+          if (OUT == 0) fp_load_slab<THREADS>(pr, S + (u64)p * SLAB_KB * a.s_cap, a.s_cap, s1, s2, s3, np, tid);
+        } else {
+          fp_load<THREADS>(br, R + rb, nb, tid);
+          if (OUT == 0) fp_load<THREADS>(pr, S + sb, np, tid);
+        }
       }
     }
   }
   const Tup* __restrict__ dummy = reinterpret_cast<const Tup*>(a.accum);
+  const PRow* __restrict__ dummy_p = reinterpret_cast<const PRow*>(a.accum);
   auto load_build = [&](Tup (&t)[FP_ROWS], bool ok, u32 pp, u32 rb_, u32 nb_, u32 q1, u32 q2, u32 q3, u32 mine) {
     if (PIECES)
       fp_load_pieces<THREADS>(t, ok ? R + (u64)pp * SLAB_KB * a.r_cap : dummy, ok ? a.r_cap : 0u, ok ? mine : 1u, tid);
@@ -1005,14 +1016,16 @@
     else
       fp_load<THREADS>(t, ok ? R + rb_ : dummy, ok ? nb_ : 1u, tid);
   };
-  auto load_probe = [&](Tup (&t)[FP_ROWS], bool ok, u32 pp, u32 sb_, u32 np_, u32 q1, u32 q2, u32 q3, u32 mine) {
-    if (PIECES)
-      fp_load_pieces<THREADS>(t, ok ? S + (u64)pp * SLAB_KB * a.s_cap : dummy, ok ? a.s_cap : 0u, ok ? mine : 1u, tid);
-    else if (SLAB)
-      fp_load_slab<THREADS>(t, ok ? S + (u64)pp * SLAB_KB * a.s_cap : dummy, ok ? a.s_cap : 0u, ok ? q1 : 1u, ok ? q2 : 1u,
-                            ok ? q3 : 1u, ok ? np_ : 1u, tid);
-    else
-      fp_load<THREADS>(t, ok ? S + sb_ : dummy, ok ? np_ : 1u, tid);
+  auto load_probe = [&](PRow (&t)[FP_ROWS], bool ok, u32 pp, u32 sb_, u32 np_, u32 q1, u32 q2, u32 q3, u32 mine) {
+    if constexpr (PIECES) {
+      fp_load_pieces<THREADS>(t, ok ? S + (u64)pp * SLAB_KB * a.s_cap : dummy_p, ok ? a.s_cap : 0u, ok ? mine : 1u, tid);
+    } else {
+      if (SLAB)
+        fp_load_slab<THREADS>(t, ok ? S + (u64)pp * SLAB_KB * a.s_cap : dummy, ok ? a.s_cap : 0u, ok ? q1 : 1u, ok ? q2 : 1u,
+                              ok ? q3 : 1u, ok ? np_ : 1u, tid);
+      else
+        fp_load<THREADS>(t, ok ? S + sb_ : dummy, ok ? np_ : 1u, tid);
+    }
   };
   const int tid_outer = tid;
   while (p < P) {
@@ -1051,10 +1064,12 @@
     if (OUT == 0) {
       load_probe(pq, regular2, pn, sb2, np2, s1n, s2n, s3n, smn);
     } else if (regular) {
-      if (SLAB)
-        fp_load_slab<THREADS>(pr, S + (u64)p * SLAB_KB * a.s_cap, a.s_cap, s1, s2, s3, np, tid);
-      else
-        fp_load<THREADS>(pr, S + sb, np, tid);
+      if constexpr (!KEYS) {
+        if (SLAB)
+          fp_load_slab<THREADS>(pr, S + (u64)p * SLAB_KB * a.s_cap, a.s_cap, s1, s2, s3, np, tid);
+        else
+          fp_load<THREADS>(pr, S + sb, np, tid);
+      }
     }
     if (regular) {
       lds_barrier();
@@ -1098,6 +1113,7 @@
       if (!HMJ_ABLATE(1u)) {
         u32 cur[FP_ROWS];
         u32 cnt[FP_ROWS], first[FP_ROWS];
+        u32 live = 0;
 #pragma unroll
         for (int k = 0; k < FP_ROWS; k++) {
           const u32 j = k * THREADS + tid;
@@ -1105,9 +1121,10 @@
           cnt[k] = 0;
           first[k] = OUT == 2 ? NIL : 0;
           if (PIECES ? ((u32)tid % QT + (u32)k * QT < sm_) : (j < np)) {
-            if (a.pfx_shift && (pr[k].key >> a.pfx_shift) != a.pfx_val) pfx_bad = true;
-            if (OUT >= 1 && (a.extra & 1u)) acc_p += pr[k].val;
-            const u32 hv = sm.head[fast_hash<LOG_NB>(pr[k].key)];
+            if (KEYS) live |= 1u << k;
+            if (a.pfx_shift && (fp_key(pr[k]) >> a.pfx_shift) != a.pfx_val) pfx_bad = true;
+            if (OUT >= 1 && (a.extra & 1u)) acc_p += fp_val(pr[k]);
+            const u32 hv = sm.head[fast_hash<LOG_NB>(fp_key(pr[k]))];
             cur[k] = ((hv >> 16) == epoch) ? (hv & 0xFFFFu) : NIL;
           }
         }
@@ -1122,19 +1139,20 @@
               const u32 i = cur[k];
               const u64 kk = sm.key[i], vv = sm.val[i];
               cur[k] = sm.next[i];
-              if (kk == pr[k].key) {
+              if (kk == fp_key(pr[k])) {
                 if (OUT == 2 && (a.extra & 2u)) {
                   first[k] = i < first[k] ? i : first[k];
                 } else {
                   acc_n++;
                   acc_r += vv;
-                  acc_s += pr[k].val;
+                  acc_s += fp_val(pr[k]);
                   if (OUT == 1) {
                     if (cnt[k] == 0) first[k] = i;
                     cnt[k]++;
                   }
+                  if (KEYS) cnt[k]++;
                   if (OUT >= 1 && (a.extra & 1u)) {
-                    const u64 m = tmix(kk, vv, pr[k].val);
+                    const u64 m = tmix(kk, vv, fp_val(pr[k]));
                     acc_x ^= m;
                     acc_m += m;
                   }
@@ -1143,6 +1161,10 @@
             }
           }
         }
+        if (KEYS) {
+#pragma unroll
+          for (int k = 0; k < FP_ROWS; k++) keys_bad |= ((live >> k) & 1u) && cnt[k] != 1u;
+        }
         if (OUT == 2 && (a.extra & 2u)) {
 #pragma unroll
           for (int k = 0; k < FP_ROWS; k++) {
@@ -1150,9 +1172,9 @@
               const u64 vv = sm.val[first[k]];
               acc_n++;
               acc_r += vv;
-              acc_s += pr[k].val;
+              acc_s += fp_val(pr[k]);
               if (a.extra & 1u) {
-                const u64 m = tmix(pr[k].key, vv, pr[k].val);
+                const u64 m = tmix(fp_key(pr[k]), vv, fp_val(pr[k]));
                 acc_x ^= m;
                 acc_m += m;
               }
@@ -1199,9 +1221,9 @@
             for (int k = 0; k < FP_ROWS; k++) {
               if (cnt[k]) {
                 const u64 d = o + ((ex >> (12 * k)) & 0xFFFu);
-                a.out_key[d] = pr[k].key;
+                a.out_key[d] = fp_key(pr[k]);
                 a.out_rval[d] = sm.val[first[k]];
-                a.out_sval[d] = pr[k].val;
+                a.out_sval[d] = fp_val(pr[k]);
               }
               const u32 tk = (u32)((tot >> (12 * k)) & 0xFFFu);
               o += tk;
@@ -1212,7 +1234,7 @@
         }
       } else {
 #pragma unroll
-        for (int k = 0; k < FP_ROWS; k++) acc_r += pr[k].key;
+        for (int k = 0; k < FP_ROWS; k++) acc_r += fp_key(pr[k]);
       }
       if (PCOUNT) {
         const u32 mine = (u32)(acc_n - n_before);
@@ -1224,7 +1246,9 @@
     } else {
       if ((PCOUNT || OUT == 1) && tid == 0 && !(nb && np)) a.part_count[p] = 0;
       if (OUT == 1 && nb && np) giveup = true;
-      if (OUT >= 1 && (a.extra & 1u) && !nb) {
+      if (KEYS && np && !nb) keys_bad = true;
+      if constexpr (KEYS) {
+      } else if (OUT >= 1 && (a.extra & 1u) && !nb) {
         if (SLAB) {
           const Tup* base = S + (u64)p * SLAB_KB * a.s_cap;
           for (u32 j = tid; j < np; j += THREADS) {
@@ -1250,6 +1274,7 @@
   if (SLAB && slab_bad && tid == 0) atomicOr(&a.accum[ACC_ERR], ERR_SLAB);
   if (OUT == 1 && __any(giveup) && (tid & 63) == 0) atomicOr(&a.accum[ACC_ERR], ERR_FASTPATH);
   if (__any(pfx_bad) && (tid & 63) == 0) atomicOr(&a.accum[ACC_ERR], ERR_PREFIX);
+  if (KEYS && __any(keys_bad) && (tid & 63) == 0) atomicOr(&a.accum[ACC_ERR], ERR_PROBE_KEYS);
   lds_barrier();
   if (PCOUNT && prev_p != 0xFFFFFFFFu && tid == 0) a.part_count[prev_p] = sm.itemcnt[parity ^ 1];
   if (tid < 8) sm.red[tid] = 0;
@@ -2410,15 +2435,15 @@
   return hipGetLastError();
 }
 
-template <int THREADS, int LOG_NB, bool PCOUNT, bool SLAB = false, int OUT = 0>
+template <int THREADS, int LOG_NB, bool PCOUNT, bool SLAB = false, int OUT = 0, bool KEYS = false>
 static hipError_t launch_fast_t(const ProbeArgs& a, u32* irregular, u32* n_irregular, int grid,
                                 hipStream_t st) {
   typedef FastSmem<THREADS, LOG_NB> Smem;
   static SmemAttrOnce attr_once;
-  if (hipError_t e = ensure_max_smem(attr_once, reinterpret_cast<const void*>(probe_count_fast_kernel<THREADS, LOG_NB, PCOUNT, SLAB, OUT>), (size_t)sizeof(Smem)); e != hipSuccess) return e;
+  if (hipError_t e = ensure_max_smem(attr_once, reinterpret_cast<const void*>(probe_count_fast_kernel<THREADS, LOG_NB, PCOUNT, SLAB, OUT, KEYS>), (size_t)sizeof(Smem)); e != hipSuccess) return e;
   if ((u32)grid > a.P) grid = (int)a.P;
   if (grid < 1) grid = 1;
-  hipLaunchKernelGGL((probe_count_fast_kernel<THREADS, LOG_NB, PCOUNT, SLAB, OUT>), dim3(grid), dim3(THREADS),
+  hipLaunchKernelGGL((probe_count_fast_kernel<THREADS, LOG_NB, PCOUNT, SLAB, OUT, KEYS>), dim3(grid), dim3(THREADS),
                      sizeof(Smem), st, a, irregular, n_irregular);
   return hipGetLastError();
 }
@@ -2520,8 +2545,9 @@
   return launch_fast_t<1024, BIG_LOG_NB, false, false, 2>(a, irregular, n_irregular, num_cus * 4, st);
 }
 
-hipError_t launch_probe_count_slab(const ProbeArgs& a, int num_cus, hipStream_t st) {
+hipError_t launch_probe_count_slab(const ProbeArgs& a, int num_cus, hipStream_t st, bool probe_keys) {
   if (!slab_operands_ok(a)) return hipErrorInvalidValue;
+  if (probe_keys) return launch_fast_t<1024, BIG_LOG_NB, false, true, 0, true>(a, nullptr, nullptr, num_cus * 4, st);
   return launch_fast_t<1024, BIG_LOG_NB, false, true>(a, nullptr, nullptr, num_cus * 4, st);
 }
 
diff --git a/hashmergejoin_amd/csrc/radix.hip b/hashmergejoin_amd/csrc/radix.hip
--- a/hashmergejoin_amd/csrc/radix.hip
+++ b/hashmergejoin_amd/csrc/radix.hip
@@ -233,6 +233,30 @@
 
 constexpr int WC_ITEMS = 4;
 constexpr int WC_LINE = 8;
+template <typename Row>
+struct WcRow;
+template <>
+struct WcRow<Tup> {
+  static constexpr int ITEMS = WC_ITEMS, LINE = WC_LINE, LINE_LOG2 = 3;
+  static __device__ __forceinline__ u64 key(const Tup& r) { return r.key; }
+  static __device__ __forceinline__ void split(const Tup& r, u64& k, u64& v) {
+    k = r.key;
+    v = r.val;
+  }
+  static __device__ __forceinline__ Tup join(u64 k, u64 v) {
+    Tup r;
+    r.key = k;
+    r.val = v;
+    return r;
+  }
+};
+template <>
+struct WcRow<u64> {
+  static constexpr int ITEMS = 8, LINE = 16, LINE_LOG2 = 4;
+  static __device__ __forceinline__ u64 key(u64 r) { return r; }
+  static __device__ __forceinline__ void split(u64 r, u64& k, u64&) { k = r; }
+  static __device__ __forceinline__ u64 join(u64 k, u64) { return k; }
+};
 
 #ifndef HMJ_WC_PLAN1
 #define HMJ_WC_PLAN1 0
@@ -274,19 +298,24 @@
 #define WC_VMWAIT()
 #endif
 
-template <int THREADS, int MAXD>
+template <int THREADS, int MAXD, typename Row = Tup>
 struct WcSmem {
-  static constexpr int TILE = THREADS * WC_ITEMS;
+  static constexpr int ITEMS = WcRow<Row>::ITEMS, LINE = WcRow<Row>::LINE;
+  static constexpr int TILE = THREADS * ITEMS;
   static constexpr int WAVES = THREADS / kWave;
-  static constexpr int ZROWS = WAVES * MAXD * 8 / 16;
-  static constexpr int MAXLINES = TILE / WC_LINE + 2 * MAXD;
+  static constexpr int ZROWS = WAVES * MAXD * 8 / (int)sizeof(Row);
+  static constexpr int MAXLINES = TILE / LINE + 2 * MAXD;
+  static_assert(LINE * sizeof(Row) == 128 && (1 << WcRow<Row>::LINE_LOG2) == LINE, "a line is 128 bytes");
   static_assert(ZROWS <= TILE && ZROWS % THREADS == 0, "lane masks must alias whole row slabs");
-  static_assert(MAXD <= THREADS && MAXD * WC_LINE == TILE, "one digit per thread; carry == tile slots");
+  static_assert(MAXD <= THREADS && MAXD * LINE == TILE, "one digit per thread; carry == tile slots");
+  static_assert(LINE <= 256 && TILE + LINE < (1 << 24) && TILE < (1 << 16) && MAXLINES < (1 << 16) && ITEMS * kWave < (1 << 16) &&
+                    MAXD <= (1 << 16),
+                "wc_tile's packed fields");
   union {
-    Tup stage[TILE];
+    Row stage[TILE];
     u64 lanemask[WAVES][MAXD];
   };
-  Tup carry[MAXD][WC_LINE];
+  Row carry[MAXD][LINE];
   u16 wcnt[WAVES][MAXD];
   u32 tile_off[MAXD];
   u32 cflush[MAXD];
@@ -303,13 +332,16 @@
 struct NoLimit {
   __device__ __forceinline__ u32 operator()(u32) const { return 0xFFFFFFFFu; }
 };
-template <int THREADS, int MAXD, bool HI, bool ALLVALID, bool LIMIT, typename Prefetch, typename Limit>
-__device__ __forceinline__ void wc_tile(WcSmem<THREADS, MAXD>& sm, Tup (&t)[WC_ITEMS], u32 tile_n,
-                                        Tup* __restrict__ out, int shift, u32 mask, u32 D,
+template <int THREADS, int MAXD, bool HI, bool ALLVALID, bool LIMIT, typename Row, typename Prefetch, typename Limit>
+__device__ __forceinline__ void wc_tile(WcSmem<THREADS, MAXD, Row>& sm, Row (&t)[WcRow<Row>::ITEMS], u32 tile_n,
+                                        Row* __restrict__ out, int shift, u32 mask, u32 D,
                                         Prefetch&& prefetch, const Limit& limit, bool* ovf WC_STAMP_ARG) {
-  typedef WcSmem<THREADS, MAXD> Smem;
+  typedef WcSmem<THREADS, MAXD, Row> Smem;
   constexpr int WAVES = Smem::WAVES;
-  const int tid = threadIdx.x, lane = tid & 63, w = tid >> 6;
+  constexpr int WC_ITEMS = Smem::ITEMS, WC_LINE = Smem::LINE, LINE_LOG2 = WcRow<Row>::LINE_LOG2;
+  int tid = threadIdx.x;
+  if constexpr (WC_ITEMS > 4) asm volatile("" : "+v"(tid));
+  const int lane = tid & 63, w = tid >> 6;
   u16* wc = &sm.wcnt[w][0];
   u64* lm = &sm.lanemask[w][0];
   const u64 lanebit = 1ull << lane;
@@ -326,7 +358,7 @@
   for (int r = 0; r < WC_ITEMS; r++) {
     u32 d = 0, rank = 0;
     if (ALLVALID || wbase + r * 64 < tile_n) {
-      d = digit_of<HI>(t[r].key, shift, mask);
+      d = digit_of<HI>(WcRow<Row>::key(t[r]), shift, mask);
       __hip_atomic_fetch_or(&lm[d], lanebit, __ATOMIC_RELAXED, __HIP_MEMORY_SCOPE_WORKGROUP);
       const u64 m = __hip_atomic_load(&lm[d], __ATOMIC_RELAXED, __HIP_MEMORY_SCOPE_WORKGROUP);
       const u32 old = __hip_atomic_load(&wc[d], __ATOMIC_RELAXED, __HIP_MEMORY_SCOPE_WORKGROUP);
@@ -373,7 +405,7 @@
         }
         const u32 tail = (cf[j] + avail) & (WC_LINE - 1);
         fl[j] = (tail >= avail) ? 0u : avail - tail;
-        nl[j] = fl[j] ? (((cf[j] & (WC_LINE - 1)) + fl[j] + WC_LINE - 1) >> 3) : 0u;
+        nl[j] = fl[j] ? (((cf[j] & (WC_LINE - 1)) + fl[j] + WC_LINE - 1) >> LINE_LOG2) : 0u;
         sm.pend[d] = avail - fl[j];
         sm.cflush[d] = cf[j] + fl[j];
       }
@@ -417,7 +449,7 @@
       }
       const u32 tail = (cf + avail) & (WC_LINE - 1);
       fl = (tail >= avail) ? 0u : avail - tail;
-      nl = fl ? (((cf & (WC_LINE - 1)) + fl + WC_LINE - 1) >> 3) : 0u;
+      nl = fl ? (((cf & (WC_LINE - 1)) + fl + WC_LINE - 1) >> LINE_LOG2) : 0u;
       sm.pend[tid] = avail - fl;
       sm.cflush[tid] = cf + fl;
     }
@@ -453,7 +485,7 @@
 
   {
     const u32 TL = sm.total_lines, k = (u32)tid & (WC_LINE - 1);
-    for (u32 L = (u32)tid >> 3; L < TL; L += THREADS / WC_LINE) {
+    for (u32 L = (u32)tid >> LINE_LOG2; L < TL; L += THREADS / WC_LINE) {
       const u32 d = sm.line_tab[L];
       const u32 pl = sm.plan[d], fl = pl >> 8, pd = pl & 0xFFu;
       u32 cfd;
@@ -468,7 +500,7 @@
   u32 has = 0;
 #pragma unroll
   for (int q = 0; q < WC_ITEMS; q++) {
-    const u32 s = q * THREADS + tid, d = s >> 3, k = s & (WC_LINE - 1);
+    const u32 s = q * THREADS + tid, d = s >> LINE_LOG2, k = s & (WC_LINE - 1);
     u32 idx = 0;
     if (d < D && k < sm.pend[d]) {
       const u32 pl = sm.plan[d], fl = pl >> 8, pd = pl & 0xFFu;
@@ -477,9 +509,8 @@
         has |= 1u << q;
       }
     }
-    const Tup kv = sm.stage[idx];
-    keep_k[q] = kv.key;
-    keep_v[q] = kv.val;
+    const Row kv = sm.stage[idx];
+    WcRow<Row>::split(kv, keep_k[q], keep_v[q]);
   }
   WC_MARK(7);
   lds_barrier();
@@ -488,18 +519,14 @@
   for (int q = 0; q < WC_ITEMS; q++) {
     const u32 s = q * THREADS + tid;
     if (has & (1u << q)) {
-      Tup kv;
-      kv.key = keep_k[q];
-      kv.val = keep_v[q];
-      sm.carry[s >> 3][s & (WC_LINE - 1)] = kv;
+      const Row kv = WcRow<Row>::join(keep_k[q], keep_v[q]);
+      sm.carry[s >> LINE_LOG2][s & (WC_LINE - 1)] = kv;
     }
   }
 #if HMJ_WC_NOBAR5
   {
-    constexpr int ZR = MAXD * 8 / 16;
-    Tup z;
-    z.key = 0;
-    z.val = 0;
+    constexpr int ZR = MAXD * 8 / (int)sizeof(Row);
+    const Row z = WcRow<Row>::join(0ull, 0ull);
 #pragma unroll
     for (int r = 0; r < ZR / kWave; r++) sm.stage[w * ZR + r * kWave + lane] = z;
     u32* wz = reinterpret_cast<u32*>(&sm.wcnt[w][0]);
@@ -511,12 +538,7 @@
 #else
 #pragma unroll
   for (int r = 0; r < WC_ITEMS; r++) {
-    if (r * THREADS < Smem::ZROWS) {
-      Tup z;
-      z.key = 0;
-      z.val = 0;
-      sm.stage[r * THREADS + tid] = z;
-    }
+    if (r * THREADS < Smem::ZROWS) sm.stage[r * THREADS + tid] = WcRow<Row>::join(0ull, 0ull);
   }
   for (int i = tid; i < WAVES * MAXD / 2; i += THREADS) reinterpret_cast<u32*>(&sm.wcnt[0][0])[i] = 0;
   WC_MARK(9);
@@ -525,20 +547,21 @@
 #endif
 }
 
-template <int THREADS, int MAXD>
-__device__ __forceinline__ void wc_flush_carry(WcSmem<THREADS, MAXD>& sm, Tup* __restrict__ out, u32 D) {
+template <int THREADS, int MAXD, typename Row>
+__device__ __forceinline__ void wc_flush_carry(WcSmem<THREADS, MAXD, Row>& sm, Row* __restrict__ out, u32 D) {
+  constexpr int WC_ITEMS = WcRow<Row>::ITEMS, WC_LINE = WcRow<Row>::LINE, LINE_LOG2 = WcRow<Row>::LINE_LOG2;
   const int tid = threadIdx.x;
   lds_barrier();
 #pragma unroll
   for (int q = 0; q < WC_ITEMS; q++) {
-    const u32 s = q * THREADS + tid, d = s >> 3, k = s & (WC_LINE - 1);
+    const u32 s = q * THREADS + tid, d = s >> LINE_LOG2, k = s & (WC_LINE - 1);
     if (d < D && k < sm.pend[d]) store_stream(&out[sm.cflush[d] + k], sm.carry[d][k]);
   }
 }
 
-template <int THREADS, int MAXD>
-__device__ __forceinline__ void wc_clear(WcSmem<THREADS, MAXD>& sm) {
-  constexpr int WAVES = WcSmem<THREADS, MAXD>::WAVES;
+template <int THREADS, int MAXD, typename Row>
+__device__ __forceinline__ void wc_clear(WcSmem<THREADS, MAXD, Row>& sm) {
+  constexpr int WAVES = WcSmem<THREADS, MAXD, Row>::WAVES;
   const int tid = threadIdx.x;
   for (int i = tid; i < WAVES * MAXD / 2; i += THREADS) reinterpret_cast<u32*>(&sm.wcnt[0][0])[i] = 0;
   for (int i = tid; i < WAVES * MAXD; i += THREADS) (&sm.lanemask[0][0])[i] = 0;
@@ -615,12 +638,23 @@
 struct NoXform {
   static constexpr bool kStrided = false;
 };
-template <int THREADS, int MAXD, bool HI, typename Xform>
+__device__ __forceinline__ unsigned long long& wc_paysum() {
+  __shared__ unsigned long long v;
+  return v;
+}
+template <int THREADS, int MAXD, bool HI, typename Xform, typename Row = Tup>
 __device__ __forceinline__ void slab_a_body(const Tup* __restrict__ in, u32 n, int shift, int bits, u32 rows_per_worker,
-                                            Tup* __restrict__ slab, u32 CA, u32 WA, u32* __restrict__ cnt_out,
+                                            Row* __restrict__ slab, u32 CA, u32 WA, u32* __restrict__ cnt_out,
                                             u64* __restrict__ accum, u32 worker_base, Xform& xf) {
-  typedef WcSmem<THREADS, MAXD> Smem;
+  typedef WcSmem<THREADS, MAXD, Row> Smem;
   constexpr int TILE = Smem::TILE;
+  constexpr int WC_ITEMS = Smem::ITEMS;
+  constexpr bool KEYS = std::is_same<Row, u64>::value;
+  static_assert(!KEYS || std::is_same<Xform, NoXform>::value, "bare keys: the join's plain pass A only");
+  u64 pay = 0;
+  if constexpr (KEYS) {
+    if (threadIdx.x == 0) wc_paysum() = 0;
+  }
   extern __shared__ __attribute__((aligned(16))) unsigned char smem_raw[];
   Smem& sm = *reinterpret_cast<Smem*>(smem_raw);
   const u32 D = 1u << bits, mask = D - 1;
@@ -641,7 +675,7 @@
 #ifdef HMJ_STAMPS
   WcStamps stamps = {};
 #endif
-  if constexpr (Xform::kStrided) {
+  if constexpr (Xform::kStrided && !KEYS) {
     constexpr u32 CH = RANK_PASS_CHUNK_ROWS, IPC = CH / 64, CPT = TILE / CH;
     static_assert(WC_ITEMS % IPC == 0 && IPC >= 1, "a wave's rows of a tile are whole chunks");
     const u64 n_chunks = ((u64)n + CH - 1) / CH, whole_chunks = n / CH;
@@ -678,6 +712,36 @@
       wc_flush_carry(sm, slab, D);
     }
   } else if (begin < end) {
+    if constexpr (KEYS) {
+      u64 t[WC_ITEMS], tv[WC_ITEMS];
+      auto load_tile = [&](const Tup* src, u32 tn) {
+#pragma unroll
+        for (int r = 0; r < WC_ITEMS; r++) {
+          const u32 q = wbase + r * 64;
+          const Tup x = load_stream(&src[q < tn ? q : tn - 1]);
+          t[r] = x.key;
+          tv[r] = x.val;
+        }
+      };
+      load_tile(in + begin, (u32)((end - begin < TILE) ? end - begin : TILE));
+      for (u64 tile = begin; tile < end; tile += TILE) {
+        const u32 tile_n = (u32)((end - tile < TILE) ? end - tile : TILE);
+        auto prefetch = [&]() {
+          if (tile + TILE < end) {
+            const u64 nt = tile + TILE;
+            load_tile(in + nt, (u32)((end - nt < TILE) ? end - nt : TILE));
+          }
+        };
+#pragma unroll
+        for (int r = 0; r < WC_ITEMS; r++)
+          pay += (wbase + (u32)r * 64 < tile_n) ? tv[r] : 0ull;
+        if (HMJ_WC_FULLTILE && tile_n == (u32)TILE)
+          wc_tile<THREADS, MAXD, HI, true, true>(sm, t, tile_n, slab, shift, mask, D, prefetch, limit, &ovf WC_STAMP_PASS);
+        else
+          wc_tile<THREADS, MAXD, HI, false, true>(sm, t, tile_n, slab, shift, mask, D, prefetch, limit, &ovf WC_STAMP_PASS);
+      }
+      wc_flush_carry(sm, slab, D);
+    } else {
     Tup t[WC_ITEMS];
     {
       const u32 tn = (u32)((end - begin < TILE) ? end - begin : TILE);
@@ -708,9 +772,16 @@
         wc_tile<THREADS, MAXD, HI, false, true>(sm, t, tile_n, slab, shift, mask, D, prefetch, limit, &ovf WC_STAMP_PASS);
     }
     wc_flush_carry(sm, slab, D);
+    }
   }
   if ((u32)tid < D) cnt_out[(u32)tid * WA + worker] = sm.cflush[tid] + sm.pend[tid] - ((u32)tid * WA + worker) * CA;
   if (ovf) atomicOr(&accum[ACC_ERR], ERR_SLAB);
+  if constexpr (KEYS) {
+    const u64 ws = wave_sum_u64(pay);
+    if (lane == 0 && ws) atomicAdd(&wc_paysum(), (unsigned long long)ws);
+    __syncthreads();
+    if (tid == 0 && wc_paysum()) atomicAdd(reinterpret_cast<unsigned long long*>(&accum[ACC_PAD]), wc_paysum());
+  }
 #ifdef HMJ_STAMPS
   stamps.flush();
 #endif
@@ -728,12 +799,14 @@
 #endif
 constexpr int SLAB_MAXSEG = 512;
 
-template <int THREADS, int MAXD, bool HI, int ADDR>
+template <int THREADS, int MAXD, bool HI, int ADDR, typename Row = Tup>
 __global__ __launch_bounds__(THREADS, (THREADS * (MAXD <= 256 ? 2 : 1)) / 256) void radix_slab_b_kernel(
-    const Tup* __restrict__ slab_a, const u32* __restrict__ cnt_a, u32 CA, u32 WA, int bits_a, int shift,
-    int bits, Tup* __restrict__ slab_b, u32 CB, u32* __restrict__ cnt_b, u64* __restrict__ accum, u32 KB) {
-  typedef WcSmem<THREADS, MAXD> Smem;
+    const Row* __restrict__ slab_a, const u32* __restrict__ cnt_a, u32 CA, u32 WA, int bits_a, int shift,
+    int bits, Row* __restrict__ slab_b, u32 CB, u32* __restrict__ cnt_b, u64* __restrict__ accum, u32 KB) {
+  typedef WcSmem<THREADS, MAXD, Row> Smem;
   constexpr int TILE = Smem::TILE;
+  constexpr int WC_ITEMS = Smem::ITEMS;
+  static_assert(ADDR == 2 || WC_ITEMS == 4, "the per-round lookup plans four rounds in lanes 0..3");
   static_assert(SLAB_MAXSEG <= THREADS, "one A-slab count per thread in the prologue scan");
   extern __shared__ __attribute__((aligned(16))) unsigned char smem_raw[];
   Smem& sm = *reinterpret_cast<Smem*>(smem_raw);
@@ -764,14 +837,14 @@
 #endif
   const u32 wbase = (u32)w * (WC_ITEMS * 64) + lane;
   (void)wbase;
-  const Tup* __restrict__ bucket = slab_a + (u64)(dA * WA + w0) * CA;
+  const Row* __restrict__ bucket = slab_a + (u64)(dA * WA + w0) * CA;
   bool ovf = false;
 #ifdef HMJ_STAMPS
   WcStamps stamps = {};
   stamps.base = 16;
 #endif
   if (total) {
-    Tup t[WC_ITEMS];
+    Row t[WC_ITEMS];
     if constexpr (ADDR != 0) {
     u32 d_s0 = 0, d_b0 = 0, d_b1 = 0, d_b2 = 0, d_b3 = 0;
     const float slabs_per_row = (float)ns / (float)total;
@@ -952,10 +1025,12 @@
         }
       };
 #ifdef HMJ_DEV
-      if (abl == 1 || abl == 4) {
-#pragma unroll
-        for (int r = 0; r < WC_ITEMS; r++)
-          if (t[r].key == 0) t[r].key = (u64)(tile + (u32)tid + r * THREADS + blockIdx.x * 7919u + 1) * 0x9E3779B97F4A7C15ull;
+      if constexpr (std::is_same<Row, Tup>::value) {
+        if (abl == 1 || abl == 4) {
+#pragma unroll
+          for (int r = 0; r < WC_ITEMS; r++)
+            if (t[r].key == 0) t[r].key = (u64)(tile + (u32)tid + r * THREADS + blockIdx.x * 7919u + 1) * 0x9E3779B97F4A7C15ull;
+        }
       }
 #endif
       if (HMJ_WC_FULLTILE && tile_n == (u32)TILE)
@@ -1120,12 +1195,12 @@
   }
 }
 
-template <int THREADS, int MAXD, bool HI>
+template <int THREADS, int MAXD, bool HI, typename Row = Tup>
 __global__ __launch_bounds__(THREADS, (THREADS * (MAXD <= 256 ? 2 : 1)) / 256) void radix_slab_a_kernel(
-    const Tup* __restrict__ in, u32 n, int shift, int bits, u32 rows_per_worker, Tup* __restrict__ slab,
+    const Tup* __restrict__ in, u32 n, int shift, int bits, u32 rows_per_worker, Row* __restrict__ slab,
     u32 CA, u32 WA, u32* __restrict__ cnt_out, u64* __restrict__ accum, u32 worker_base) {
   NoXform xf;
-  slab_a_body<THREADS, MAXD, HI, NoXform>(in, n, shift, bits, rows_per_worker, slab, CA, WA, cnt_out, accum, worker_base, xf);
+  slab_a_body<THREADS, MAXD, HI, NoXform, Row>(in, n, shift, bits, rows_per_worker, slab, CA, WA, cnt_out, accum, worker_base, xf);
 }
 
 template <bool CUT>
@@ -1202,28 +1277,36 @@
     if (rows) atomicAdd(reinterpret_cast<unsigned long long*>(&accum[ACC_N]), (unsigned long long)rows);
   }
 }
-template <int THREADS, int MAXD, bool HI>
+template <int THREADS, int MAXD, bool HI, typename Row = Tup>
 static hipError_t launch_slab_a_t(const void* in, u32 n, int shift, int bits, u32 rpw, void* slab, u32 CA,
                                   u32 WA, u32* cnt, u64* accum, hipStream_t st, u32 w_begin, u32 w_end) {
-  typedef WcSmem<THREADS, MAXD> Smem;
+  typedef WcSmem<THREADS, MAXD, Row> Smem;
   const size_t smem = sizeof(Smem);
   static_assert(sizeof(Smem) <= 160 * 1024, "slab pass A: LDS");
   static SmemAttrOnce attr_once;
-  if (hipError_t e = ensure_max_smem(attr_once, reinterpret_cast<const void*>(radix_slab_a_kernel<THREADS, MAXD, HI>), (size_t)smem); e != hipSuccess) return e;
+  if (hipError_t e = ensure_max_smem(attr_once, reinterpret_cast<const void*>(radix_slab_a_kernel<THREADS, MAXD, HI, Row>), (size_t)smem); e != hipSuccess) return e;
   if (w_end > WA) w_end = WA;
   if (w_begin >= w_end) return hipSuccess;
-  hipLaunchKernelGGL((radix_slab_a_kernel<THREADS, MAXD, HI>), dim3(w_end - w_begin), dim3(THREADS), smem, st,
-                     static_cast<const Tup*>(in), n, shift, bits, rpw, static_cast<Tup*>(slab), CA, WA, cnt,
+  hipLaunchKernelGGL((radix_slab_a_kernel<THREADS, MAXD, HI, Row>), dim3(w_end - w_begin), dim3(THREADS), smem, st,
+                     static_cast<const Tup*>(in), n, shift, bits, rpw, static_cast<Row*>(slab), CA, WA, cnt,
                      accum, w_begin);
   return hipGetLastError();
 }
 
-template <int THREADS, int MAXD, bool HI>
+template <int THREADS, int MAXD, bool HI, typename Row = Tup>
 static hipError_t launch_slab_b_t(const void* slab_a, const u32* cnt_a, u32 CA, u32 WA, int bits_a, int shift,
                                   int bits, void* slab_b, u32 CB, u32* cnt_b, u64* accum, hipStream_t st, u32 KB) {
-  typedef WcSmem<THREADS, MAXD> Smem;
+  typedef WcSmem<THREADS, MAXD, Row> Smem;
   const size_t smem = sizeof(Smem) + (SLAB_MAXSEG + 1) * sizeof(u32);
   static_assert(sizeof(Smem) + (SLAB_MAXSEG + 1) * sizeof(u32) <= 160 * 1024, "slab pass B: LDS");
+  if constexpr (!std::is_same<Row, Tup>::value) {
+    static SmemAttrOnce attr_keys;
+    if (hipError_t e = ensure_max_smem(attr_keys, reinterpret_cast<const void*>(radix_slab_b_kernel<THREADS, MAXD, HI, 2, Row>), (size_t)smem); e != hipSuccess) return e;
+    hipLaunchKernelGGL((radix_slab_b_kernel<THREADS, MAXD, HI, 2, Row>), dim3((1u << bits_a) * KB), dim3(THREADS), smem, st,
+                       static_cast<const Row*>(slab_a), cnt_a, CA, WA, bits_a, shift, bits,
+                       static_cast<Row*>(slab_b), CB, cnt_b, accum, KB);
+    return hipGetLastError();
+  } else {
 #ifdef HMJ_DEV
   if (g_b_addr_alt) {
     constexpr int ALT = HMJ_B_ADDR == 2 ? 1 : 2;
@@ -1241,6 +1324,7 @@
                      static_cast<const Tup*>(slab_a), cnt_a, CA, WA, bits_a, shift, bits,
                      static_cast<Tup*>(slab_b), CB, cnt_b, accum, KB);
   return hipGetLastError();
+  }
 }
 
 static u32 slab_cap(double mean, double fan) {
@@ -1248,9 +1332,10 @@
   return ((u32)c + 8) & ~7u;
 }
 u32 slab_capacity(double mean, double fan) { return slab_cap(mean, fan < 1.0 ? 1.0 : fan); }
-bool slab_geometry(u32 n, int bits_a, int bits_b, SlabGeom* g, u32 kb, double fan, double density) {
+bool slab_geometry(u32 n, int bits_a, int bits_b, SlabGeom* g, u32 kb, double fan, double density, u32 row_bytes) {
   if (bits_a < 1 || bits_a > SLAB_MAX_BITS || bits_b < 1 || bits_b > SLAB_MAX_BITS) return false;
-  const u32 tile = bits_a > 8 ? 4096 : 2048;
+  if (row_bytes != 16 && (row_bytes != 8 || bits_a > 8 || bits_b > 8)) return false;
+  const u32 tile = (bits_a > 8 ? 4096u : 2048u) * (16u / row_bytes);
   u64 tiles = ((u64)n + tile - 1) / tile;
   u64 max_workers = 2048;
 #ifdef HMJ_DEV
@@ -1268,6 +1353,10 @@
   const double fan_a = 1.0 + 4.0 * (double)g->rpw * fan / (double)(n ? n : 1);
   g->CA = slab_cap(density * (double)g->rpw / (double)(1u << bits_a), fan_a < fan ? fan_a : fan);
   g->CB = slab_cap(density * (double)n / (double)(1u << bits_a) / (double)kb / (double)(1u << bits_b), fan);
+  if (row_bytes == 8) {
+    g->CA = (g->CA + 15u) & ~15u;
+    g->CB = (g->CB + 15u) & ~15u;
+  }
   const u64 rows_a = (u64)(1u << bits_a) * g->WA * g->CA;
   const u64 rows_b = (u64)(1u << (bits_a + bits_b)) * kb * g->CB;
   g->rows_a = rows_a;
@@ -1295,11 +1384,17 @@
 }
 
 hipError_t launch_slab_a(const void* in, u32 n, int shift, int bits, const SlabGeom& g, void* slab_a, u64 slab_a_rows,
-                         u32* cnt_a, u64 cnt_a_n, u64* accum, hipStream_t st, u32 w_begin, u32 w_end) {
+                         u32* cnt_a, u64 cnt_a_n, u64* accum, hipStream_t st, u32 w_begin, u32 w_end, u32 row_bytes) {
   if (bits < 1 || bits > SLAB_MAX_BITS || g.WA == 0 || g.CA == 0 || (u64)g.WA * g.rpw < n) return hipErrorInvalidValue;
   if (slab_a_rows < ((u64)g.WA << bits) * g.CA || cnt_a_n < ((u64)g.WA << bits)) return hipErrorInvalidValue;
   if (((u64)g.WA << bits) * g.CA >= 0xFFFFFFF0ull) return hipErrorInvalidValue;
   const bool hi = shift >= 32;
+  if (row_bytes == 8) {
+    if (bits > 8 || (g.CA & 15u) || (g.rpw & 4095u)) return hipErrorInvalidValue;
+    return hi ? launch_slab_a_t<512, 256, true, u64>(in, n, shift, bits, g.rpw, slab_a, g.CA, g.WA, cnt_a, accum, st, w_begin, w_end)
+              : launch_slab_a_t<512, 256, false, u64>(in, n, shift, bits, g.rpw, slab_a, g.CA, g.WA, cnt_a, accum, st, w_begin, w_end);
+  }
+  if (row_bytes != 16) return hipErrorInvalidValue;
 #define HMJ_SLAB_A(T, M, H) launch_slab_a_t<T, M, H>(in, n, shift, bits, g.rpw, slab_a, g.CA, g.WA, cnt_a, accum, st, w_begin, w_end)
   if (bits > 8) return hi ? HMJ_SLAB_A(1024, 512, true) : HMJ_SLAB_A(1024, 512, false);
   return hi ? HMJ_SLAB_A(512, 256, true) : HMJ_SLAB_A(512, 256, false);
@@ -1348,13 +1443,20 @@
 }
 
 hipError_t launch_slab_b(const void* slab_a, const u32* cnt_a, int bits_a, int shift, int bits,
-                         const SlabGeom& g, void* slab_b, u64 slab_b_rows, u32* cnt_b, u64 cnt_b_n, u64* accum, hipStream_t st) {
+                         const SlabGeom& g, void* slab_b, u64 slab_b_rows, u32* cnt_b, u64 cnt_b_n, u64* accum, hipStream_t st,
+                         u32 row_bytes) {
   if (bits < 1 || bits > SLAB_MAX_BITS || bits_a < 1 || bits_a > SLAB_MAX_BITS || g.KB == 0 || g.WA < g.KB ||
       (g.WA + g.KB - 1) / g.KB > (u32)SLAB_MAXSEG)
     return hipErrorInvalidValue;
   const u64 pieces = ((u64)g.KB << (bits_a + bits));
   if (slab_b_rows < pieces * g.CB || cnt_b_n < pieces || pieces * g.CB >= 0xFFFFFFF0ull) return hipErrorInvalidValue;
   const bool hi = shift >= 32;
+  if (row_bytes == 8) {
+    if (bits > 8 || bits_a > 8 || (g.CA & 15u) || (g.CB & 15u)) return hipErrorInvalidValue;
+    return hi ? launch_slab_b_t<512, 256, true, u64>(slab_a, cnt_a, g.CA, g.WA, bits_a, shift, bits, slab_b, g.CB, cnt_b, accum, st, g.KB)
+              : launch_slab_b_t<512, 256, false, u64>(slab_a, cnt_a, g.CA, g.WA, bits_a, shift, bits, slab_b, g.CB, cnt_b, accum, st, g.KB);
+  }
+  if (row_bytes != 16) return hipErrorInvalidValue;
 #define HMJ_SLAB_B(T, M, H) launch_slab_b_t<T, M, H>(slab_a, cnt_a, g.CA, g.WA, bits_a, shift, bits, slab_b, g.CB, cnt_b, accum, st, g.KB)
   if (bits > 8) return hi ? HMJ_SLAB_B(1024, 512, true) : HMJ_SLAB_B(1024, 512, false);
   return hi ? HMJ_SLAB_B(512, 256, true) : HMJ_SLAB_B(512, 256, false);
diff --git a/include/hmj.h b/include/hmj.h
--- a/include/hmj.h
+++ b/include/hmj.h
@@ -92,6 +92,7 @@
 #define HMJ_PATH_ORDERED_EXPANSION 0x400000u
 #define HMJ_PATH_LDS_TABLE 0x800000u
 #define HMJ_PATH_GLOBAL_TABLE 0x100000u
+#define HMJ_PATH_PROBE_KEYS 0x10000000u
 #define HMJ_PATH_HOST_PIPELINE 0x4000u
 
 typedef struct {
@@ -136,6 +137,7 @@
 #define HMJ_COOL_EXACT_PREFIX 0x800u
 #define HMJ_COOL_RANK_RUNS 0x1000u
 #define HMJ_COOL_SORT_MSD 0x2000u
+#define HMJ_COOL_PROBE_KEYS 0x4000u
 
 int hmj_create(hmj_ctx** out, int device_id);
 void hmj_destroy(hmj_ctx* ctx);
```

After: 34.28 billion. Within noise of the previous version (-0.1%).
